# czi-ai/variantformer

Measured on AMD Instinct MI355X. Metric: genes/sec/node (54-tissue expr) at 1 Mb cis-window, higher is better.
Workload: dtype bf16; 1 GPU; BASELINE configs[1]: full 1.2B-architecture network (25 modulator layers, width 1536, 32 heads; seq2reg width 512, 8 heads, 6 layers, assumed), random-init weights, 1 Mb cis-window, 54 tissues, 1 donor; one step = 32 such genes per GPU; n_cre_windows=1024, gene_chunks=200, tissues=54, parallelism=gene-shard x1, streams=CRE layers on a side stream (default)

## Files before the change

variantformer_amd/_lib.py:

```python
from __future__ import annotations

import ctypes as C
import os

_HERE = os.path.dirname(os.path.abspath(__file__))
LIB_PATH = os.path.join(_HERE, "csrc", "libvf_hip.so")

VF_F32, VF_BF16, VF_F16 = 0, 1, 2
EPI_BF16, EPI_F32, EPI_RES_F32, EPI_GEGLU_BF16, EPI_GELU_F32, EPI_GELU_BF16 = 0, 1, 2, 3, 4, 5
ABI_VERSION = 13

_p, _i, _l, _f = C.c_void_p, C.c_int, C.c_int64, C.c_float

SIGNATURES = {
    "vf_version": [],
    "vf_last_error": [],
    "vf_last_kernel": [_i],
    "vf_gemm_bf16": [_p, _l, _p, _p, _p, _l, _p, _l, _i, _i, _i, _i, _p],
    "vf_gemm_bf16_ex": [_p, _l, _p, _p, _p, _l, _p, _l, _i, _i, _i, _i, _i, _p],
    "vf_gemm_f16": [_p, _l, _p, _p, _p, _l, _p, _l, _i, _i, _i, _i, _p],
    "vf_gemm_f16_ex": [_p, _l, _p, _p, _p, _l, _p, _l, _i, _i, _i, _i, _i, _p],
    "vf_gemm_ln_bf16": [_p, _l, _p, _p, _p, _l, _p, _l, _i, _i, _i, _i, _p, _p, _p, _l, _p, _p],
    "vf_gemm_ln_t16": [_p, _l, _p, _p, _p, _l, _f, _p, _l, _i, _i, _i, _i, _p, _l, _p, _f, _p, _l, _f, _p],
    "vf_gemm_ln": [_p, _l, _p, _p, _p, _l, _i, _p, _l, _i, _i, _i, _i, _i, _p, _p, _p, _l, _p, _f, _f, _p],
    "vf_ln_finalize": [_p, _l, _i, _i, _f, _p, _p],
    "vf_ln_finalize2": [_p, _l, _i, _i, _f, _f, _f, _f, _p, _p, _p],
    "vf_row_stats_cast2": [_p, _l, _i, _f, _p, _i, _f, _f, _f, _p, _p, _p],
    "vf_row_stats_cast": [_p, _l, _i, _f, _p, _i, _p, _p],
    "vf_pack_geglu_rows": [_p, _p, _p, _p, _i, _i, _p],
    "vf_attn_varlen_fwd": [_p, _p, _p, _p, _l, _l, _l, _l, _p, _p, _i, _i, _i, _i, _i, _p, _f, _p],
    "vf_attn_varlen_fwd_qstart": [_p, _p, _p, _p, _l, _l, _l, _l, _p, _p, _i, _i, _i, _i, _i, _p, _f, _p],
    "vf_attn_varlen_fwd_f16": [_p, _p, _p, _p, _l, _l, _l, _l, _p, _p, _i, _i, _i, _i, _i, _p, _f, _p],
    "vf_attn_varlen_fwd_qstart_f16": [_p, _p, _p, _p, _l, _l, _l, _l, _p, _p, _i, _i, _i, _i, _i, _p, _f, _p],
    "vf_attn_varlen_fwd_v2": [_p, _p, _p, _p, _l, _l, _l, _l, _p, _p, _i, _i, _i, _i, _i, _p, _f, _i, _i, _p],
    "vf_attn_varlen_fwd_v3": [_p, _p, _p, _p, _l, _l, _l, _l, _p, _p, _i, _i, _i, _i, _i, _p, _f, _i, _i, _p],
    "vf_attn_rows_supported": [_i, _i, _i, _i, _i, _i, _i],
    "vf_attn_counted_keys": [_p, _l, _p, _l, _p, _p, _i, _i, _i, _i, _i, _p, _l, _i, _p],
    "vf_attn_probs": [_p, _l, _p, _l, _p, _p, _p, _i, _i, _i, _i, _i, _f, _i, _i, _i, _p, _p, _l, _p],
    "vf_attn_probs_v2": [_p, _l, _p, _l, _p, _p, _p, _i, _i, _i, _i, _i, _f, _i, _i, _i, _p, _p, _l, _p, _p, _p, _p],
    "vf_softmax_counted": [_p, _l, _p, _p, _i, _i, _i, _i, _i, _p, _l, _i, _p],
    "vf_attn_varlen_fwd_rows": [_p, _p, _p, _p, _l, _l, _l, _l, _p, _p, _i, _i, _i, _i, _i, _p, _f, _i, _i, _p, _p, _p],
    "vf_layernorm": [_p, _p, _p, _p, _l, _i, _f, _i, _i, _p],
    "vf_embed_stream": [_p, _p, _p, _p, _p, _p, _p, _i, _f, _p, _f, _p, _f, _f, _f, _p, _i, _i, _i, _i, _p],
    "vf_embed_pack": [_p, _p, _p, _p, _p, _p, _i, _i, _i, _i, _p],
    "vf_mask_to_cu_seqlens": [_p, _p, _i, _i, _p],
    "vf_segment_mean": [_p, _p, _p, _i, _i, _i, _p],
    "vf_segment_mean16": [_p, _l, _i, _p, _f, _p, _p, _i, _i, _p],
    "vf_token_keys": [_p, _p, _p, _p, _i, _i, _i, _i, _p],
    "vf_gather_rows_f32": [_p, _p, _p, _p, _l, _i, _i, _p],
    "vf_gather_rows_bf16": [_p, _l, _p, _p, _l, _l, _i, _p],
    "vf_rowdot_softplus": [_p, _p, _p, _p, _l, _i, _i, _p],
    "vf_cast_f32_bf16": [_p, _p, _l, _p],
    "vf_cast_f32_f16": [_p, _p, _l, _p],
    "vf_segment_max": [_p, _p, _p, _i, _i, _p],
    "vf_segment_linear": [_p, _p, _p, _p, _p, _p, _i, _i, _i, _i, _p],
    "vf_affine_rows_f32": [_p, _p, _p, _p, _p, _l, _i, _p],
    "vf_add_rows_f32": [_p, _p, _p, _p, _p, _l, _i, _p],
    "vf_bpe_create": [_p, _i, _p, _i],
    "vf_bpe_destroy": [_p],
    "vf_bpe_encode": [_p, C.c_char_p, _l, _p, _p, _l],
    "vf_bpe_encode_prefix": [_p, C.c_char_p, _l, _l, _p, _p, _l],
    "vf_vcf_open": [C.c_char_p, C.c_char_p],
    "vf_vcf_close": [_p],
    "vf_vcf_num_records": [_p, C.c_char_p],
    "vf_vcf_consensus": [_p, C.c_char_p, _l, C.c_char_p, _l, _i, _i, _p, _l, _p],
    "vf_build_windows": [_p, _p, C.c_char_p, _l, C.c_char_p, _l, _l, _p, _p, _i, _i, _i, _i, _l, _p, _p, _p],
    "vf_narrow_ids": [_p, _l, _p, _l, _l],
}
NEXT_SIGNATURES = {
    "vf_attn_contrib": [_p, _l, _p, _p, _l, _p, _p, _i, _i, _i, _i, _i, _i, _i, _p, _p, _l, _p],
}
_RESTYPES = {"vf_last_error": C.c_char_p, "vf_last_kernel": C.c_char_p, "vf_bpe_create": C.c_void_p, "vf_bpe_destroy": None, "vf_bpe_encode": C.c_int64, "vf_bpe_encode_prefix": C.c_int64,
             "vf_vcf_open": C.c_void_p, "vf_vcf_close": None, "vf_vcf_num_records": C.c_int64,
             "vf_vcf_consensus": C.c_int64, "vf_build_windows": C.c_int64}

_lib = None


class VFError(RuntimeError):
    pass


def load(path: str | None = None):
    global _lib
    if _lib is not None and path is None:
        return _lib
    path = path or LIB_PATH
    import torch
    if not os.path.exists(path):
        raise VFError(
            f"{path} not found: the HIP extension has not been built "
            "(run `python -m variantformer_amd.csrc.build` or __graft_entry__.build()). "
            "There is no CPU fallback for the product path.")
    lib = C.CDLL(path)
    for name, argtypes in list(SIGNATURES.items()) + list(NEXT_SIGNATURES.items()):
        try:
            fn = getattr(lib, name)
        except AttributeError as e:
            raise VFError(f"libvf_hip.so does not export {name}") from e
        fn.argtypes = argtypes
        fn.restype = _RESTYPES.get(name, C.c_int)
    v = lib.vf_version()
    if v != ABI_VERSION:
        raise VFError(f"libvf_hip.so ABI version {v} != expected {ABI_VERSION}")
    _lib = lib
    return lib


def check(rc: int, what: str):
    if rc != 0:
        msg = load().vf_last_error()
        raise VFError(f"{what} failed (code {rc}): {msg.decode() if msg else ''}")
```

variantformer_amd/csrc/build.py:

```python
from __future__ import annotations

import os
import shutil
import subprocess
import sys

HERE = os.path.dirname(os.path.abspath(__file__))
SOURCES = ["vf_gemm.hip", "vf_attn.hip", "vf_misc.hip", "vf_bpe.cpp", "vf_vcf.cpp", "vf_host.cpp"]
HEADERS = ["vf_common.h", os.path.join("..", "..", "include", "vf_hip.h"), os.path.join("..", "..", "include", "vf_hip_next.h")]
LIB = os.path.join(HERE, "libvf_hip.so")
ARCH = "gfx950"
EXTRA_FLAGS = {"vf_attn.hip": ["-fno-honor-nans"]}
NO_PACKED_FP32 = ["-Xclang", "-target-feature", "-Xclang", "-packed-fp32-ops"]


def _stale() -> bool:
    if not os.path.exists(LIB):
        return True
    t = os.path.getmtime(LIB)
    return any(os.path.getmtime(os.path.join(HERE, f)) > t for f in SOURCES + HEADERS + [os.path.basename(__file__)])


def build_lib(force: bool = False, verbose: bool = False) -> str:
    if not force and not _stale():
        return LIB
    hipcc = shutil.which("hipcc") or "/opt/rocm/bin/hipcc"
    if not os.path.exists(hipcc):
        raise RuntimeError("hipcc not found: cannot build libvf_hip.so")
    objs = []
    procs = []
    for src in SOURCES:
        obj = os.path.join(HERE, os.path.splitext(src)[0] + ".o")
        cmd = [hipcc, f"--offload-arch={ARCH}", "-O3", "-std=c++17", "-fPIC", "-Wno-unused-result",
               "-mllvm", "-amdgpu-mfma-vgpr-form=1"] + (NO_PACKED_FP32 if src.endswith(".hip") else []) + \
              EXTRA_FLAGS.get(src, []) + \
              ["-c", os.path.join(HERE, src), "-o", obj]
        if verbose:
            cmd.insert(1, "-Rpass-analysis=kernel-resource-usage")
        procs.append((src, subprocess.Popen(cmd, stdout=subprocess.PIPE, stderr=subprocess.STDOUT, text=True)))
        objs.append(obj)
    for src, p in procs:
        out, _ = p.communicate()
        if p.returncode != 0:
            raise RuntimeError(f"hipcc failed on {src}:\n{out}")
        if verbose and out:
            print(out)
    cmd = [hipcc, f"--offload-arch={ARCH}", "-shared", "-fPIC", "-o", LIB + ".tmp"] + objs + ["-lz"]
    r = subprocess.run(cmd, stdout=subprocess.PIPE, stderr=subprocess.STDOUT, text=True)
    if r.returncode != 0:
        raise RuntimeError(f"link failed:\n{r.stdout}")
    os.replace(LIB + ".tmp", LIB)
    return LIB


if __name__ == "__main__":
    print(build_lib(force="--force" in sys.argv, verbose="-v" in sys.argv))
```

variantformer_amd/csrc/vf_common.h:

```cpp
#pragma once
#include <hip/hip_runtime.h>
#include <stdint.h>
#include <stdio.h>
#include "../../include/vf_hip.h"
#include "../../include/vf_hip_next.h"

typedef __attribute__((ext_vector_type(8))) __bf16 bf16x8_t;
typedef __attribute__((ext_vector_type(4))) short s16x4_t;
typedef __attribute__((ext_vector_type(4))) float f32x4_t;
typedef __attribute__((ext_vector_type(16))) float f32x16_t;
typedef __attribute__((ext_vector_type(4))) unsigned int u32x4_t;
typedef __attribute__((ext_vector_type(2))) unsigned int u32x2_t;

#define VF_WAVE 64

void vf_set_error(const char* fmt, ...);
void vf_note_kernel(int which, const char* name);

#define VF_MAX_DEVICES 64
static inline int vf_current_device() {
    int d = -1;
    if (hipGetDevice(&d) != hipSuccess) { (void)hipGetLastError(); return -1; }
    return (d >= 0 && d < VF_MAX_DEVICES) ? d : -1;
}

#define VF_REQUIRE(cond, ...)                        \
    do {                                             \
        if (!(cond)) {                               \
            vf_set_error(__VA_ARGS__);               \
            return VF_ERR_INVALID_ARG;               \
        }                                            \
    } while (0)

#define VF_CHECK_LAUNCH(name)                                                          \
    do {                                                                               \
        hipError_t e_ = hipGetLastError();                                             \
        if (e_ != hipSuccess) {                                                        \
            vf_set_error("%s: launch failed: %s", name, hipGetErrorString(e_));        \
            return VF_ERR_LAUNCH;                                                      \
        }                                                                              \
    } while (0)

__device__ __forceinline__ unsigned short f2bf(float x) {
    __bf16 b = (__bf16)x;
    return *reinterpret_cast<unsigned short*>(&b);
}
typedef __attribute__((ext_vector_type(2))) float f32x2_t;
typedef __attribute__((ext_vector_type(2))) __bf16 bf16x2_t;
__device__ __forceinline__ unsigned int pack2bf(float lo, float hi) {
    const f32x2_t v = {lo, hi};
    const bf16x2_t b = __builtin_convertvector(v, bf16x2_t);
    return __builtin_bit_cast(unsigned int, b);
}
__device__ __forceinline__ float bf2f(unsigned short b) {
    return __uint_as_float(((unsigned int)b) << 16);
}
typedef __attribute__((ext_vector_type(8))) _Float16 f16x8_t;
typedef __attribute__((ext_vector_type(2))) _Float16 f16x2_t;
__device__ __forceinline__ unsigned int pack2h(float lo, float hi) {
    const f32x2_t v = {lo, hi};
    const f16x2_t h = __builtin_convertvector(v, f16x2_t);
    return __builtin_bit_cast(unsigned int, h);
}
__device__ __forceinline__ float h2f(unsigned short b) {
    return (float)__builtin_bit_cast(_Float16, b);
}

template <int DT> struct Op16;
template <> struct Op16<VF_BF16> {
    using frag = bf16x8_t;
    static __device__ __forceinline__ f32x4_t mfma(frag a, frag b, f32x4_t c) {
        return __builtin_amdgcn_mfma_f32_16x16x32_bf16(a, b, c, 0, 0, 0);
    }
    static __device__ __forceinline__ f32x16_t mfma32(frag a, frag b, f32x16_t c) {
        return __builtin_amdgcn_mfma_f32_32x32x16_bf16(a, b, c, 0, 0, 0);
    }
    static __device__ __forceinline__ unsigned int pack2(float lo, float hi) { return pack2bf(lo, hi); }
    static __device__ __forceinline__ float to_f32(unsigned short b) { return bf2f(b); }
    static constexpr unsigned int ONE = 0x3F80u, NEG_BIG = 0xC700u;
};
template <> struct Op16<VF_F16> {
    using frag = f16x8_t;
    static __device__ __forceinline__ f32x4_t mfma(frag a, frag b, f32x4_t c) {
        return __builtin_amdgcn_mfma_f32_16x16x32_f16(a, b, c, 0, 0, 0);
    }
    static __device__ __forceinline__ f32x16_t mfma32(frag a, frag b, f32x16_t c) {
        return __builtin_amdgcn_mfma_f32_32x32x16_f16(a, b, c, 0, 0, 0);
    }
    static __device__ __forceinline__ unsigned int pack2(float lo, float hi) { return pack2h(lo, hi); }
    static __device__ __forceinline__ float to_f32(unsigned short b) { return h2f(b); }
    static constexpr unsigned int ONE = 0x3C00u, NEG_BIG = 0xF800u;
};

__device__ __forceinline__ f32x4_t gelu_erf4(f32x4_t x) {
    f32x4_t ax, t, e;
#pragma unroll
    for (int i = 0; i < 4; ++i) ax[i] = __builtin_fabsf(x[i]);
    const f32x4_t d = ax * 0.23164190f + 1.0f;
#pragma unroll
    for (int i = 0; i < 4; ++i) t[i] = __builtin_amdgcn_rcpf(d[i]);
    f32x4_t p = t * 1.061405429f + -1.453152027f;
    p = p * t + 1.421413741f;
    p = p * t + -0.284496736f;
    p = p * t + 0.254829592f;
    const f32x4_t w = x * x * -0.72134752044448170368f;
#pragma unroll
    for (int i = 0; i < 4; ++i) e[i] = __builtin_amdgcn_exp2f(w[i]);
    const f32x4_t hq = p * t * e * 0.5f;
    f32x4_t r;
#pragma unroll
    for (int i = 0; i < 4; ++i) r[i] = x[i] * (x[i] >= 0.f ? 1.0f - hq[i] : hq[i]);
    return r;
}
__device__ __forceinline__ float gelu_erf(float x) {
    return gelu_erf4((f32x4_t){x, x, x, x})[0];
}
__device__ __forceinline__ float wave_sum(float v) {
#pragma unroll
    for (int o = 32; o > 0; o >>= 1) v += __shfl_xor(v, o);
    return v;
}
```

variantformer_amd/csrc/vf_gemm.hip:

```cpp
#include <type_traits>
#include "vf_common.h"

namespace {

template <int BK>
__device__ __forceinline__ int swz(int row) {
    if (BK == 64) return (row >> 1) & 7;
    return (0x78 >> (((row >> 2) & 3) * 2)) & 3;
}

__device__ __forceinline__ void glds16(const void* g, void* lds) {
    __builtin_amdgcn_global_load_lds((__attribute__((address_space(1))) void*)g,
                                     (__attribute__((address_space(3))) void*)lds, 16, 0, 0);
}

template <int N>
__device__ __forceinline__ void wait_vmcnt() {
    asm volatile("s_waitcnt vmcnt(%0)" ::"n"(N) : "memory");
}

struct LnArgs {
    const float* row_stats;
    const float* colsum;
    void* out16;
    float* part_stats;
    int64_t ld16;
    int64_t rows;
    float x16_scale;
    float res16_scale;
    const unsigned short* res16;
    int64_t ldr16;
    unsigned short* t16_out;
    int64_t ldt16;
    float t16_scale;
};
enum { VF_LN_NONE = 0, VF_LN_CONSUMER = 1, VF_LN_PRODUCER = 2, VF_LN_PRODUCER_R16 = 3, VF_LN_PRODUCER_T16 = 4 };
constexpr bool ln_is_producer(int ln) { return ln == VF_LN_PRODUCER || ln == VF_LN_PRODUCER_R16 || ln == VF_LN_PRODUCER_T16; }
constexpr bool ln_res_is_16(int ln) { return ln == VF_LN_PRODUCER_R16 || ln == VF_LN_PRODUCER_T16; }

template <int DT>
__device__ __forceinline__ f32x4_t cvt4_16(u32x2_t v) {
    if (DT == VF_BF16)
        return (f32x4_t){__uint_as_float(v[0] << 16), __uint_as_float(v[0] & 0xFFFF0000u), __uint_as_float(v[1] << 16),
                         __uint_as_float(v[1] & 0xFFFF0000u)};
    return (f32x4_t){Op16<DT>::to_f32((unsigned short)(v[0] & 0xFFFFu)), Op16<DT>::to_f32((unsigned short)(v[0] >> 16)),
                     Op16<DT>::to_f32((unsigned short)(v[1] & 0xFFFFu)), Op16<DT>::to_f32((unsigned short)(v[1] >> 16))};
}

template <int CTRL>
__device__ __forceinline__ float dpp_f32(float v) {
    return __builtin_bit_cast(float, __builtin_amdgcn_update_dpp(0, __builtin_bit_cast(int, v), CTRL, 0xF, 0xF, true));
}

template <int DT>
__device__ __forceinline__ void ln_emit(f32x4_t f, bool valid, unsigned short* p16, float* ppart, int lane,
                                        float x16_scale = 1.0f, unsigned short* pt16 = nullptr, float t16_scale = 1.0f) {
    float s1 = (f[0] + f[1]) + (f[2] + f[3]);
    s1 += dpp_f32<0xB1>(s1);
    s1 += dpp_f32<0x4E>(s1);
    s1 += dpp_f32<0x141>(s1);
    const float mp = s1 * (1.0f / 32.0f);
    const float d0 = f[0] - mp, d1 = f[1] - mp, d2 = f[2] - mp, d3 = f[3] - mp;
    float s2 = __builtin_fmaf(d3, d3, __builtin_fmaf(d2, d2, __builtin_fmaf(d1, d1, d0 * d0)));
    s2 += dpp_f32<0xB1>(s2);
    s2 += dpp_f32<0x4E>(s2);
    s2 += dpp_f32<0x141>(s2);
    if (valid) {
        u32x2_t pk;
        if (pt16) {
            const f32x4_t t = f * t16_scale;
            pk[0] = pack2h(t[0], t[1]);
            pk[1] = pack2h(t[2], t[3]);
            *reinterpret_cast<u32x2_t*>(pt16) = pk;
        }
        if (DT == VF_F16) f *= x16_scale;
        pk[0] = Op16<DT>::pack2(f[0], f[1]);
        pk[1] = Op16<DT>::pack2(f[2], f[3]);
        *reinterpret_cast<u32x2_t*>(p16) = pk;
        if ((lane & 7) == 0) *reinterpret_cast<f32x2_t*>(ppart) = (f32x2_t){s1, s2};
    }
}

template <int DT>
__device__ __forceinline__ void ln_emit8(f32x4_t fa, f32x4_t fb, bool valid, unsigned short* p16, float* ppart, int lane,
                                         float x16_scale, unsigned short* pt16, float t16_scale) {
    float s1 = ((fa[0] + fa[1]) + (fa[2] + fa[3])) + ((fb[0] + fb[1]) + (fb[2] + fb[3]));
    s1 += dpp_f32<0xB1>(s1);
    s1 += dpp_f32<0x4E>(s1);
    const float mp = s1 * (1.0f / 32.0f);
    const float a0 = fa[0] - mp, a1 = fa[1] - mp, a2 = fa[2] - mp, a3 = fa[3] - mp;
    const float b0 = fb[0] - mp, b1 = fb[1] - mp, b2 = fb[2] - mp, b3 = fb[3] - mp;
    float s2 = __builtin_fmaf(a3, a3, __builtin_fmaf(a2, a2, __builtin_fmaf(a1, a1, a0 * a0))) +
               __builtin_fmaf(b3, b3, __builtin_fmaf(b2, b2, __builtin_fmaf(b1, b1, b0 * b0)));
    s2 += dpp_f32<0xB1>(s2);
    s2 += dpp_f32<0x4E>(s2);
    if (valid) {
        u32x4_t pk;
        if (pt16) {
            const f32x4_t ta = fa * t16_scale, tb = fb * t16_scale;
            pk = (u32x4_t){pack2h(ta[0], ta[1]), pack2h(ta[2], ta[3]), pack2h(tb[0], tb[1]), pack2h(tb[2], tb[3])};
            *reinterpret_cast<u32x4_t*>(pt16) = pk;
        }
        if (DT == VF_F16) { fa *= x16_scale; fb *= x16_scale; }
        pk = (u32x4_t){Op16<DT>::pack2(fa[0], fa[1]), Op16<DT>::pack2(fa[2], fa[3]), Op16<DT>::pack2(fb[0], fb[1]),
                       Op16<DT>::pack2(fb[2], fb[3])};
        *reinterpret_cast<u32x4_t*>(p16) = pk;
        if ((lane & 3) == 0) *reinterpret_cast<f32x2_t*>(ppart) = (f32x2_t){s1, s2};
        else asm volatile("" :: "v"(s1), "v"(s2));
    }
}

template <int DT, int LN, class V>
__device__ __forceinline__ f32x4_t res_value(V v, const LnArgs& ln) {
    if constexpr (LN == VF_LN_PRODUCER_T16) return cvt4_16<VF_F16>(v) * ln.res16_scale;
    else if constexpr (ln_res_is_16(LN)) {
        if constexpr (DT == VF_F16) return cvt4_16<DT>(v) * ln.res16_scale;
        else return cvt4_16<DT>(v);
    }
    else return v;
}

template <int DT, int LN, int REGION>
__device__ __forceinline__ void producer16_epilogue_wide(f32x4_t (&acc)[4][8], char* region, const char* side, int side_n,
                                                         int64_t mw0, int nw0, bool has_bias, void* out, int64_t ldo, int M,
                                                         int N, const LnArgs& ln) {
    constexpr int TM = 8, TN = 4, WT_M = 128, PITCH = 64 * 4 + 16, RP = 32, IMP = RP / 16, NPASS = TM / IMP;
    constexpr int RI = 8, NI = RP / RI;
    constexpr bool T16 = LN == VF_LN_PRODUCER_T16;
    static_assert(REGION >= RP * PITCH, "wide producer epilogue: staging region too small");
    int lane_e;
    asm volatile("v_mbcnt_lo_u32_b32 %0, -1, 0\n\tv_mbcnt_hi_u32_b32 %0, -1, %0" : "=v"(lane_e));
    const int lane = lane_e, r = lane & 15, g = lane >> 4;
    const int ep_row = lane >> 3, ep_col = nw0 + (lane & 7) * 8;
    const int rows_left = (int)(M - mw0) - ep_row;
    const int64_t row0 = mw0 + ep_row;
    const int colc = ep_col < N ? ep_col : N - 8;
    const char* res_run = reinterpret_cast<const char*>(ln.res16) + (row0 * ln.ldr16 + colc) * 2;
    const char* const res_last = reinterpret_cast<const char*>(ln.res16) + ((int64_t)(M - 1) * ln.ldr16 + colc) * 2;
    const int64_t res_step = (int64_t)RI * ln.ldr16 * 2;
    char* out_run = reinterpret_cast<char*>(out) + (row0 * ldo + ep_col) * 4;
    const int64_t out_step = (int64_t)RI * ldo * 4;
    unsigned short* o16_run = reinterpret_cast<unsigned short*>(ln.out16) + row0 * ln.ld16 + ep_col;
    const int64_t o16_step = (int64_t)RI * ln.ld16;
    float* part_run = ln.part_stats + ((int64_t)(ep_col >> 5) * ln.rows + row0) * 2;
    unsigned short* t16_run = T16 ? ln.t16_out + row0 * ln.ldt16 + ep_col : nullptr;
    const int64_t t16_step = (int64_t)RI * ln.ldt16;
    u32x4_t rbuf[2][NI];
    auto load_res_pass = [&](int ps, u32x4_t (&dst)[NI]) {
#pragma unroll
        for (int k = 0; k < NI; ++k) {
            const int j = ps * NI + k;
            const char* rp = (j * RI < rows_left) ? res_run : res_last;
            res_run += res_step;
            dst[k] = *reinterpret_cast<const u32x4_t*>(rp);
        }
    };
    load_res_pass(0, rbuf[0]);
    f32x4_t bvec[TN];
#pragma unroll
    for (int in = 0; in < TN; ++in)
        bvec[in] = has_bias ? *reinterpret_cast<const f32x4_t*>(side + (side_n + in * 16 + 4 * g) * 4) : (f32x4_t){0.f, 0.f, 0.f, 0.f};
#pragma unroll
    for (int ps = 0; ps < NPASS; ++ps) {
        if (ps + 1 < NPASS) load_res_pass(ps + 1, rbuf[(ps + 1) & 1]);
#pragma unroll
        for (int iml = 0; iml < IMP; ++iml) {
            const int im = ps * IMP + iml;
            char* rowp = region + (iml * 16 + r) * PITCH;
#pragma unroll
            for (int in = 0; in < TN; ++in) *reinterpret_cast<f32x4_t*>(rowp + (in * 16 + 4 * g) * 4) = acc[in][im] + bvec[in];
        }
        u32x4_t da[NI], db[NI];
#pragma unroll
        for (int k = 0; k < NI; ++k) {
            const char* p = region + (k * RI + ep_row) * PITCH + (lane & 7) * 32;
            da[k] = *reinterpret_cast<const u32x4_t*>(p);
            db[k] = *reinterpret_cast<const u32x4_t*>(p + 16);
        }
#pragma unroll
        for (int k = 0; k < NI; ++k) {
            const int j = ps * NI + k;
            const u32x4_t rv = rbuf[ps & 1][k];
            const f32x4_t fa = __builtin_bit_cast(f32x4_t, da[k]) + res_value<DT, LN>((u32x2_t){rv[0], rv[1]}, ln);
            const f32x4_t fb = __builtin_bit_cast(f32x4_t, db[k]) + res_value<DT, LN>((u32x2_t){rv[2], rv[3]}, ln);
            const bool ok = j * RI + ep_row < WT_M && j * RI < rows_left && ep_col < N;
            ln_emit8<DT>(fa, fb, ok, o16_run, part_run, lane, ln.x16_scale, (T16 && ln.t16_out) ? t16_run : nullptr, ln.t16_scale);
            o16_run += o16_step;
            part_run += RI * 2;
            if (T16) t16_run += t16_step;
            if (ok && out != nullptr) {
                *reinterpret_cast<f32x4_t*>(out_run) = fa;
                *reinterpret_cast<f32x4_t*>(out_run + 16) = fb;
            }
            out_run += out_step;
        }
    }
}

template <int EPI, int DT = VF_BF16>
__device__ __forceinline__ void epilogue_store(f32x4_t v, f32x4_t gate, int64_t m, int n_bias, int n_bias_gate,
                                               int n_out, const float* __restrict__ bias,
                                               const float* __restrict__ res, int64_t ldr, void* out, int64_t ldo,
                                               const f32x4_t* res_pre = nullptr) {
    if (bias) {
        const f32x4_t b = *reinterpret_cast<const f32x4_t*>(bias + n_bias);
        v += b;
        if (EPI == VF_EPI_GEGLU_BF16) gate += *reinterpret_cast<const f32x4_t*>(bias + n_bias_gate);
    }
    if (EPI == VF_EPI_RES_F32) v += res_pre ? *res_pre : *reinterpret_cast<const f32x4_t*>(res + m * ldr + n_out);
    if (EPI == VF_EPI_GEGLU_BF16) {
        v = v * gelu_erf4(gate);
    }
    if (EPI == VF_EPI_GELU_F32 || EPI == VF_EPI_GELU_BF16) {
        v = gelu_erf4(v);
    }
    if (EPI == VF_EPI_F32 || EPI == VF_EPI_RES_F32 || EPI == VF_EPI_GELU_F32) {
        *reinterpret_cast<f32x4_t*>(reinterpret_cast<float*>(out) + m * ldo + n_out) = v;
    } else {
        u32x2_t p;
        p[0] = Op16<DT>::pack2(v[0], v[1]);
        p[1] = Op16<DT>::pack2(v[2], v[3]);
        *reinterpret_cast<u32x2_t*>(reinterpret_cast<unsigned short*>(out) + m * ldo + n_out) = p;
    }
}

template <int BM_, int BN_, int WM_, int WN_, int STAGES_, int BK_ = 64>
struct Cfg {
    static constexpr int BM = BM_, BN = BN_, WM = WM_, WN = WN_, STAGES = STAGES_, BK = BK_;
    static constexpr int NW = WM * WN, THREADS = NW * 64;
    static constexpr int TM = BM / WM / 16, TN = BN / WN / 16;
    static constexpr int ROW_BYTES = BK * 2, CPR = BK / 8, KS = BK / 32;
    static constexpr int ROWS_PER_PIECE = 1024 / ROW_BYTES;
    static constexpr int A_BYTES = BM * ROW_BYTES, W_BYTES = BN * ROW_BYTES, STAGE_BYTES = A_BYTES + W_BYTES;
    static constexpr int LDS_BYTES = STAGES * STAGE_BYTES;
    static constexpr int PA = A_BYTES / 1024 / NW, PW = W_BYTES / 1024 / NW;
    static constexpr int LPT = PA + PW;
    static_assert(BK == 64 || BK == 32, "BK");
    static_assert(A_BYTES % (1024 * NW) == 0 && W_BYTES % (1024 * NW) == 0, "pieces must divide over the waves");
    static_assert(STAGES >= 2 && STAGES <= 5 && (STAGES - 2) * LPT <= 48, "vmcnt range");
};

__device__ __forceinline__ void tile_origin(int t, int n_tiles, int tiles_n, int GROUP_M, int BM, int BN, int& m0, int& n0) {
    const int q8 = n_tiles >> 3, r8 = n_tiles & 7, xcd = t & 7, loc = t >> 3;
    const int wg = (xcd < r8 ? xcd * (q8 + 1) : r8 * (q8 + 1) + (xcd - r8) * q8) + loc;
    const int tiles_m = n_tiles / tiles_n;
    const int per_group = GROUP_M * tiles_n;
    const int grp = wg / per_group, in_grp = wg - grp * per_group;
    const int first_m = grp * GROUP_M;
    const int gsz = (tiles_m - first_m) < GROUP_M ? (tiles_m - first_m) : GROUP_M;
    m0 = (first_m + in_grp % gsz) * BM;
    n0 = (in_grp / gsz) * BN;
}

template <class C, int EPI, int DT = VF_BF16, int LN = VF_LN_NONE>
__global__ __launch_bounds__(C::THREADS, 2) void gemm_mfma_kernel(const unsigned short* __restrict__ A, int64_t lda,
                                                              const unsigned short* __restrict__ W,
                                                              const float* __restrict__ bias,
                                                              const float* __restrict__ res, int64_t ldr, void* out,
                                                              int64_t ldo, int M, int N, int K, int tiles_n, int n_blocks,
                                                              int GROUP_M, LnArgs ln) {
    extern __shared__ __attribute__((aligned(16))) char smem[];
    using frag_t = typename Op16<DT>::frag;
    constexpr int BM = C::BM, BN = C::BN, TM = C::TM, TN = C::TN, STAGES = C::STAGES, LPT = C::LPT;
    constexpr int BK = C::BK, ROW_BYTES = C::ROW_BYTES, CPR = C::CPR, RPP = C::ROWS_PER_PIECE;

    int m0, n0;
    tile_origin(blockIdx.x, n_blocks, tiles_n, GROUP_M, BM, BN, m0, n0);

    const int tid = threadIdx.x, lane = tid & 63;
    const int wave = __builtin_amdgcn_readfirstlane(tid >> 6);
    const int wm = wave / C::WN, wn = wave % C::WN;
    const int r = lane & 15, g = lane >> 4;

    const unsigned short* srcA[C::PA];
    const unsigned short* srcW[C::PW];
#pragma unroll
    for (int i = 0; i < C::PA; ++i) {
        const int row = RPP * (wave * C::PA + i) + lane / CPR;
        const int c = (lane % CPR) ^ swz<BK>(row);
        int gm = m0 + row; gm = gm < M ? gm : M - 1;
        srcA[i] = A + (int64_t)gm * lda + c * 8;
    }
#pragma unroll
    for (int i = 0; i < C::PW; ++i) {
        const int row = RPP * (wave * C::PW + i) + lane / CPR;
        const int c = (lane % CPR) ^ swz<BK>(row);
        int gn = n0 + row; gn = gn < N ? gn : N - 1;
        srcW[i] = W + (int64_t)gn * K + c * 8;
    }
    char* const ldsA_piece = smem + wave * C::PA * 1024;
    char* const ldsW_piece = smem + C::A_BYTES + wave * C::PW * 1024;

    auto issue = [&](int kt, int stage) {
#pragma unroll
        for (int i = 0; i < C::PA; ++i) glds16(srcA[i] + kt * BK, ldsA_piece + stage * C::STAGE_BYTES + i * 1024);
#pragma unroll
        for (int i = 0; i < C::PW; ++i) glds16(srcW[i] + kt * BK, ldsW_piece + stage * C::STAGE_BYTES + i * 1024);
    };

    f32x4_t acc[TN][TM];
#pragma unroll
    for (int i = 0; i < TN; ++i)
#pragma unroll
        for (int j = 0; j < TM; ++j) acc[i][j] = (f32x4_t){0.f, 0.f, 0.f, 0.f};

    const int sw = swz<BK>(r);
    const int offW = C::A_BYTES + (wn * (BN / C::WN) + r) * ROW_BYTES;
    const int offA = (wm * (BM / C::WM) + r) * ROW_BYTES;

    auto read_frags = [&](int stage, int ks, frag_t(&wf)[TN], frag_t(&af)[TM]) {
        const char* base = smem + stage * C::STAGE_BYTES + (((4 * ks + g) ^ sw) << 4);
#pragma unroll
        for (int i = 0; i < TN; ++i) wf[i] = *reinterpret_cast<const frag_t*>(base + offW + i * 16 * ROW_BYTES);
#pragma unroll
        for (int i = 0; i < TM; ++i) af[i] = *reinterpret_cast<const frag_t*>(base + offA + i * 16 * ROW_BYTES);
    };
    auto issue_piece = [&](int kt, int stage, int i) {
        if (i < C::PA) glds16(srcA[i] + kt * BK, ldsA_piece + stage * C::STAGE_BYTES + i * 1024);
        else glds16(srcW[i - C::PA] + kt * BK, ldsW_piece + stage * C::STAGE_BYTES + (i - C::PA) * 1024);
    };
    auto mma_spread = [&](const frag_t(&wf)[TN], const frag_t(&af)[TM], int kt_issue, int stage_issue, bool do_issue) {
        constexpr int EVERY = 3;
#pragma unroll
        for (int in = 0; in < TN; ++in)
#pragma unroll
            for (int im = 0; im < TM; ++im) {
                acc[in][im] = Op16<DT>::mfma(wf[in], af[im], acc[in][im]);
                const int idx = in * TM + im;
                if (idx % EVERY == EVERY - 1 && idx / EVERY < LPT) {
                    if (do_issue) issue_piece(kt_issue, stage_issue, idx / EVERY);
                    __builtin_amdgcn_sched_barrier(0);
                }
            }
    };
    auto mma = [&](const frag_t(&wf)[TN], const frag_t(&af)[TM]) {
#pragma unroll
        for (int in = 0; in < TN; ++in)
#pragma unroll
            for (int im = 0; im < TM; ++im)
                acc[in][im] = Op16<DT>::mfma(wf[in], af[im], acc[in][im]);
    };
    auto wait_tiles = [&](int ahead) {
        if (STAGES >= 5 && ahead >= 3) wait_vmcnt<3 * LPT>();
        else if (STAGES >= 4 && ahead == 2) wait_vmcnt<2 * LPT>();
        else if (STAGES >= 3 && ahead == 1) wait_vmcnt<LPT>();
        else wait_vmcnt<0>();
    };

    const int nkt = K / BK;
#pragma unroll
    for (int p = 0; p < STAGES; ++p)
        if (p < nkt) issue(p, p);
    wait_tiles((nkt - 1) < (STAGES - 1) ? (nkt - 1) : (STAGES - 1));
    __builtin_amdgcn_s_barrier();
    asm volatile("" ::: "memory");

    frag_t wf0[TN], af0[TM], wf1[TN], af1[TM];
    read_frags(0, 0, wf0, af0);
    int stage = 0;
    auto boundary = [&](int t) {
        asm volatile("s_waitcnt lgkmcnt(0)" ::: "memory");
        wait_tiles((nkt - 2 - t) < (STAGES - 2) ? (nkt - 2 - t) : (STAGES - 2));
        __builtin_amdgcn_s_barrier();
        asm volatile("" ::: "memory");
        if (t + STAGES < nkt) issue(t + STAGES, stage);
        stage = stage + 1 == STAGES ? 0 : stage + 1;
    };
    constexpr bool OUT_F32 = (EPI == VF_EPI_F32 || EPI == VF_EPI_RES_F32 || EPI == VF_EPI_GELU_F32);
    constexpr int ES = OUT_F32 ? 4 : 2;
    constexpr int WT_M = BM / C::WM, WT_N = BN / C::WN;
    constexpr int WT_NO = (EPI == VF_EPI_GEGLU_BF16) ? WT_N / 2 : WT_N;
    constexpr int PITCH = WT_NO * ES + 16;
    constexpr int REGION = C::LDS_BYTES / C::NW;
    constexpr int RP = (((REGION / PITCH) < WT_M ? (REGION / PITCH) : WT_M) / 16) * 16;
    constexpr int IMP = RP / 16, NPASS = (TM + IMP - 1) / IMP;
    constexpr int CR = WT_NO * ES / 16, RI = 64 / CR, NI = RP / RI;
    static_assert(RP >= 16 && CR >= 1 && CR <= 64 && 64 % CR == 0, "epilogue geometry");
    const int n_out_total = (EPI == VF_EPI_GEGLU_BF16) ? N / 2 : N;
    const int64_t mw0 = m0 + wm * WT_M;
    const int no0 = (EPI == VF_EPI_GEGLU_BF16) ? (n0 + wn * WT_N) / 2 : (n0 + wn * WT_N);
    const int ep_row = lane / CR, ep_col = no0 + (lane % CR) * (16 / ES);
    constexpr bool RES_PRE = (EPI == VF_EPI_RES_F32) && (TN * TM <= 16);
    constexpr bool R16 = ln_res_is_16(LN), T16 = LN == VF_LN_PRODUCER_T16;
    using res_t = typename std::conditional<R16, u32x2_t, f32x4_t>::type;
    auto res_load = [&](int64_t m, int col) -> res_t {
        if constexpr (R16) return *reinterpret_cast<const u32x2_t*>(ln.res16 + m * ln.ldr16 + col);
        else return *reinterpret_cast<const f32x4_t*>(res + m * ldr + col);
    };
    res_t resv[RES_PRE ? NPASS : 1][RES_PRE ? NI : 1];
    auto prefetch_residual = [&]() {
        if (RES_PRE) {
#pragma unroll
            for (int ps = 0; ps < NPASS; ++ps)
#pragma unroll
                for (int k = 0; k < NI; ++k) {
                    int64_t m = mw0 + ps * RP + k * RI + ep_row;
                    m = m < M ? m : M - 1;
                    const int col = ep_col < N ? ep_col : N - 4;
                    resv[RES_PRE ? ps : 0][RES_PRE ? k : 0] = res_load(m, col);
                }
        }
    };
    constexpr bool RES_PIPE = (EPI == VF_EPI_RES_F32) && !RES_PRE;
    res_t rbuf[2][RES_PIPE ? NI : 1];
    auto load_res_pass = [&](int ps, res_t (&dst)[RES_PIPE ? NI : 1]) {
        if (RES_PIPE) {
#pragma unroll
            for (int k = 0; k < NI; ++k) {
                int64_t m = mw0 + ps * RP + k * RI + ep_row;
                m = m < M ? m : M - 1;
                const int col = ep_col < N ? ep_col : N - 4;
                dst[RES_PIPE ? k : 0] = res_load(m, col);
            }
        }
    };
    constexpr bool SPREAD = C::KS == 2 && C::NW == 8 && STAGES == 2 && (TN * TM) >= 3 * LPT;
    if (SPREAD) {
        for (int kt = 0; kt < nkt; ++kt) {
            read_frags(stage, 1, wf1, af1);
            if (kt + 1 == nkt) prefetch_residual();
            mma(wf0, af0);
            int freed = stage;
            const bool more = kt + 1 < nkt;
            if (more) {
                asm volatile("s_waitcnt lgkmcnt(0)" ::: "memory");
                wait_tiles((nkt - 2 - kt) < (STAGES - 2) ? (nkt - 2 - kt) : (STAGES - 2));
                __builtin_amdgcn_s_barrier();
                asm volatile("" ::: "memory");
                stage = stage + 1 == STAGES ? 0 : stage + 1;
                read_frags(stage, 0, wf0, af0);
            }
            mma_spread(wf1, af1, kt + STAGES, freed, more && kt + STAGES < nkt);
        }
    } else if (C::KS == 2) {
        for (int kt = 0; kt < nkt; ++kt) {
            read_frags(stage, 1, wf1, af1);
            if (kt + 1 == nkt) prefetch_residual();
            mma(wf0, af0);
            if (kt + 1 < nkt) {
                boundary(kt);
                read_frags(stage, 0, wf0, af0);
            }
            mma(wf1, af1);
        }
    } else {
        for (int kt = 0; kt < nkt; kt += 2) {
            boundary(kt);
            read_frags(stage, 0, wf1, af1);
            mma(wf0, af0);
            if (kt + 2 < nkt) {
                boundary(kt + 1);
                read_frags(stage, 0, wf0, af0);
            } else {
                prefetch_residual();
            }
            mma(wf1, af1);
        }
    }

    const int nw0 = n0 + wn * WT_N;
    load_res_pass(0, rbuf[0]);
    __syncthreads();
    f32x4_t bvec[TN];
    if (bias) {
#pragma unroll
        for (int in = 0; in < TN; ++in) {
            int nb = (EPI == VF_EPI_GEGLU_BF16) ? nw0 + (in >> 1) * 32 + (in & 1) * 16 + 4 * g : nw0 + in * 16 + 4 * g;
            nb = nb < N ? nb : 0;
            bvec[in] = *reinterpret_cast<const f32x4_t*>(bias + nb);
        }
    } else {
#pragma unroll
        for (int in = 0; in < TN; ++in) bvec[in] = (f32x4_t){0.f, 0.f, 0.f, 0.f};
    }
    f32x4_t svec[LN == VF_LN_CONSUMER ? TN : 1];
    float ln_mu[LN == VF_LN_CONSUMER ? TM : 1], ln_rs[LN == VF_LN_CONSUMER ? TM : 1];
    if (LN == VF_LN_CONSUMER) {
#pragma unroll
        for (int in = 0; in < TN; ++in) {
            int nb = (EPI == VF_EPI_GEGLU_BF16) ? nw0 + (in >> 1) * 32 + (in & 1) * 16 + 4 * g : nw0 + in * 16 + 4 * g;
            nb = nb < N ? nb : 0;
            svec[LN == VF_LN_CONSUMER ? in : 0] = *reinterpret_cast<const f32x4_t*>(ln.colsum + nb);
        }
#pragma unroll
        for (int im = 0; im < TM; ++im) {
            int64_t m = mw0 + im * 16 + r;
            m = m < M ? m : M - 1;
            const f32x2_t st = *reinterpret_cast<const f32x2_t*>(ln.row_stats + 2 * m);
            ln_mu[LN == VF_LN_CONSUMER ? im : 0] = -st[0] * st[1];
            ln_rs[LN == VF_LN_CONSUMER ? im : 0] = st[1];
        }
    }
    auto lnv = [&](int in, int im) -> f32x4_t {
        if (LN == VF_LN_CONSUMER)
            return acc[in][im] * ln_rs[LN == VF_LN_CONSUMER ? im : 0] +
                   (ln_mu[LN == VF_LN_CONSUMER ? im : 0] * svec[LN == VF_LN_CONSUMER ? in : 0] + bvec[in]);
        return acc[in][im] + bvec[in];
    };
    char* const region = smem + wave * REGION;
#pragma unroll
    for (int ps = 0; ps < NPASS; ++ps) {
        if (ps + 1 < NPASS) load_res_pass(ps + 1, rbuf[(ps + 1) & 1]);
#pragma unroll
        for (int iml = 0; iml < IMP; ++iml) {
            const int im = ps * IMP + iml;
            if (im < TM) {
                char* rowp = region + (iml * 16 + r) * PITCH;
                if (EPI == VF_EPI_GEGLU_BF16) {
#pragma unroll
                    for (int ip = 0; ip < TN / 2; ++ip) {
                        const f32x4_t v = lnv(2 * ip, im), gt = lnv(2 * ip + 1, im);
                        u32x2_t pk;
                        const f32x4_t y = v * gelu_erf4(gt);
                        pk[0] = Op16<DT>::pack2(y[0], y[1]);
                        pk[1] = Op16<DT>::pack2(y[2], y[3]);
                        *reinterpret_cast<u32x2_t*>(rowp + (ip * 16 + 4 * g) * 2) = pk;
                    }
                } else {
#pragma unroll
                    for (int in = 0; in < TN; ++in) {
                        f32x4_t v = lnv(in, im);
                        if (EPI == VF_EPI_GELU_F32 || EPI == VF_EPI_GELU_BF16) {
                            v = gelu_erf4(v);
                        }
                        if (OUT_F32) {
                            *reinterpret_cast<f32x4_t*>(rowp + (in * 16 + 4 * g) * 4) = v;
                        } else {
                            u32x2_t pk;
                            pk[0] = Op16<DT>::pack2(v[0], v[1]);
                            pk[1] = Op16<DT>::pack2(v[2], v[3]);
                            *reinterpret_cast<u32x2_t*>(rowp + (in * 16 + 4 * g) * 2) = pk;
                        }
                    }
                }
            }
        }
        constexpr int KB = (EPI == VF_EPI_RES_F32) ? 4 : NI;
#pragma unroll
        for (int k0 = 0; k0 < NI; k0 += KB) {
            u32x4_t dd[KB];
#pragma unroll
            for (int k = 0; k < KB; ++k)
                if (k0 + k < NI)
                    dd[k] = *reinterpret_cast<const u32x4_t*>(region + ((k0 + k) * RI + ep_row) * PITCH + (lane % CR) * 16);
#pragma unroll
            for (int k = 0; k < KB; ++k) {
                if (k0 + k >= NI) continue;
                const int row = (k0 + k) * RI + ep_row;
                const int64_t m = mw0 + ps * RP + row;
                u32x4_t d = dd[k];
                if (EPI == VF_EPI_RES_F32) {
                    f32x4_t f = __builtin_bit_cast(f32x4_t, d);
                    f += res_value<DT, LN>(RES_PRE ? resv[RES_PRE ? ps : 0][RES_PRE ? k0 + k : 0] : rbuf[ps & 1][RES_PIPE ? k0 + k : 0], ln);
                    d = __builtin_bit_cast(u32x4_t, f);
                }
                const bool ok = ps * RP + row < WT_M && m < M && ep_col < n_out_total;
                if (ln_is_producer(LN) && OUT_F32)
                    ln_emit<DT>(__builtin_bit_cast(f32x4_t, d), ok,
                                reinterpret_cast<unsigned short*>(ln.out16) + m * ln.ld16 + ep_col,
// ... 43 lines not shown
                        Op16<DT>::mfma(WF[i][ks], af[j][ks], acc[IN0 + i][IM0 + j]); \
    } while (0)

template <int EPI, int DT = VF_BF16, int LN = VF_LN_NONE>
__global__ __launch_bounds__(512, 2) void gemm8_kernel(const unsigned short* __restrict__ A, int64_t lda,
                                                       const unsigned short* __restrict__ W,
                                                       const float* __restrict__ bias, const float* __restrict__ res,
                                                       int64_t ldr, void* out, int64_t ldo, int M, int N, int K,
                                                       int tiles_n, int n_blocks, int GROUP_M, LnArgs ln) {
    extern __shared__ __attribute__((aligned(16))) char smem[];
    using frag_t = typename Op16<DT>::frag;
    using C = Cfg8;
    constexpr int BM = C::BM, BN = C::BN, TM = C::TM, TN = C::TN, BK = C::BK;

    int m0, n0;
    tile_origin(blockIdx.x, n_blocks, tiles_n, GROUP_M, BM, BN, m0, n0);

    const int tid = threadIdx.x, lane = tid & 63;
    const int wave = __builtin_amdgcn_readfirstlane(tid >> 6);
    const int wm = wave >> 2, wn = wave & 3;
    const int r = lane & 15, g = lane >> 4;

    const unsigned short* src[4][2];
#pragma unroll
    for (int pi = 0; pi < 2; ++pi) {
        const int i = 16 * wave + 8 * pi + (lane >> 3);
        const int c = (lane & 7) ^ ((i >> 1) & 7);
        const int am = m0 + (i >> 6) * 128 + (i & 63);
        const int wn_row = n0 + (i >> 5) * 64 + (i & 31);
        int v;
        v = am;           v = v < M ? v : M - 1;  src[C::AL][pi] = A + (int64_t)v * lda + c * 8;
        v = am + 64;      v = v < M ? v : M - 1;  src[C::AH][pi] = A + (int64_t)v * lda + c * 8;
        v = wn_row;       v = v < N ? v : N - 1;  src[C::WL][pi] = W + (int64_t)v * K + c * 8;
        v = wn_row + 32;  v = v < N ? v : N - 1;  src[C::WH][pi] = W + (int64_t)v * K + c * 8;
    }
    char* const lds_piece = smem + wave * 2048;
    auto issue = [&](int kt, int type) {
        char* dst = lds_piece + (kt & 1) * C::TILE_BYTES + type * C::HALF_BYTES;
        glds16(src[type][0] + kt * BK, dst);
        glds16(src[type][1] + kt * BK, dst + 1024);
    };

    f32x4_t acc[TN][TM];
#pragma unroll
    for (int i = 0; i < TN; ++i)
#pragma unroll
        for (int j = 0; j < TM; ++j) acc[i][j] = (f32x4_t){0.f, 0.f, 0.f, 0.f};

    const int sw = (r >> 1) & 7;
    const int ck0 = ((g) ^ sw) << 4, ck1 = ((4 + g) ^ sw) << 4;
    const int offW = (wn * 32 + r) * 128;
    const int offA = (wm * 64 + r) * 128;
    frag_t wlo[2][2], whi[2][2], af[4][2];
    auto read_w = [&](const char* buf, int type, frag_t (&f)[2][2]) {
        const char* b = buf + type * C::HALF_BYTES + offW;
#pragma unroll
        for (int i = 0; i < 2; ++i) {
            f[i][0] = *reinterpret_cast<const frag_t*>(b + i * 2048 + ck0);
            f[i][1] = *reinterpret_cast<const frag_t*>(b + i * 2048 + ck1);
        }
    };
    auto read_a = [&](const char* buf, int type) {
        const char* b = buf + type * C::HALF_BYTES + offA;
#pragma unroll
        for (int i = 0; i < 4; ++i) {
            af[i][0] = *reinterpret_cast<const frag_t*>(b + i * 2048 + ck0);
            af[i][1] = *reinterpret_cast<const frag_t*>(b + i * 2048 + ck1);
        }
    };
    char* const side = smem + C::LDS_BYTES;
    if (bias && wave == 0) {
        int n = n0 + 4 * lane;
        n = n < N ? n : N - 4;
        glds16(bias + n, side);
    }
    if (LN == VF_LN_CONSUMER) {
        if (wave == 1) {
            int n = n0 + 4 * lane;
            n = n < N ? n : N - 4;
            glds16(ln.colsum + n, side + 1024);
        }
        int64_t m = m0 + 32 * wave + (lane >> 1);
        m = m < M ? m : M - 1;
        __builtin_amdgcn_global_load_lds((__attribute__((address_space(1))) void*)(ln.row_stats + 2 * m + (lane & 1)),
                                         (__attribute__((address_space(3))) void*)(side + 2048 + wave * 256), 4, 0, 0);
    }

    const int nkt = K / BK;
    issue(0, C::WL); issue(0, C::AL); issue(0, C::WH); issue(0, C::AH);
    if (nkt > 1) {
        issue(1, C::WL); issue(1, C::AL); issue(1, C::WH);
        wait_vmcnt<6>();
    } else {
        wait_vmcnt<0>();
    }
    __builtin_amdgcn_s_barrier();
    asm volatile("" ::: "memory");
    if (wm == 1) __builtin_amdgcn_s_barrier();

    for (int t = 0; t < nkt; ++t) {
        const char* buf = smem + (t & 1) * C::TILE_BYTES;
        const bool pre1 = t + 1 < nkt, pre2 = t + 2 < nkt;
        read_w(buf, C::WL, wlo);
        __builtin_amdgcn_sched_barrier(0);
        read_a(buf, C::AL);
        if (pre1) issue(t + 1, C::AH);
        asm volatile("s_waitcnt lgkmcnt(8)" ::: "memory");
        VF_G8_SYNC_IN();
        VF_G8_MMA(wlo, 0, 0);
        VF_G8_SYNC_OUT();
        read_w(buf, C::WH, whi);
        if (pre2) issue(t + 2, C::WL);
        VF_G8_SYNC_IN();
        VF_G8_MMA(whi, 2, 0);
        VF_G8_SYNC_OUT();
        read_a(buf, C::AH);
        if (pre2) issue(t + 2, C::AL);
        VF_G8_SYNC_IN();
        VF_G8_MMA(whi, 2, 4);
        VF_G8_SYNC_OUT();
        if (pre2) {
            issue(t + 2, C::WH);
            wait_vmcnt<6>();
        } else {
            wait_vmcnt<0>();
        }
        VF_G8_SYNC_IN();
        VF_G8_MMA(wlo, 0, 4);
        VF_G8_SYNC_OUT();
    }
    if (wm == 0) __builtin_amdgcn_s_barrier();
    asm volatile("" ::: "memory");

    constexpr bool OUT_F32 = (EPI == VF_EPI_F32 || EPI == VF_EPI_RES_F32 || EPI == VF_EPI_GELU_F32);
    constexpr int ES = OUT_F32 ? 4 : 2;
    constexpr int WT_M = 128, WT_N = 64;
    constexpr int WT_NO = (EPI == VF_EPI_GEGLU_BF16) ? WT_N / 2 : WT_N;
    constexpr int PITCH = WT_NO * ES + 16;
    constexpr int REGION = C::LDS_BYTES / C::NW;
    constexpr int RP_FIT = (((REGION / PITCH) < WT_M ? (REGION / PITCH) : WT_M) / 16) * 16;
    constexpr int RP = (ln_is_producer(LN) && EPI == VF_EPI_RES_F32 && RP_FIT > 32) ? 32 : RP_FIT;
    constexpr int IMP = RP / 16, NPASS = (TM + IMP - 1) / IMP;
    constexpr int CR = WT_NO * ES / 16, RI = 64 / CR, NI = RP / RI;
    static_assert(RP >= 16 && CR >= 1 && CR <= 64 && 64 % CR == 0, "epilogue geometry");
    constexpr bool RES = (EPI == VF_EPI_RES_F32);
    const int n_out_total = (EPI == VF_EPI_GEGLU_BF16) ? N / 2 : N;
    const int64_t mw0 = m0 + wm * WT_M;
    const int nw0 = n0 + wn * WT_N;
    const int no0 = (EPI == VF_EPI_GEGLU_BF16) ? nw0 / 2 : nw0;
    const int ep_row = lane / CR, ep_col = no0 + (lane % CR) * (16 / ES);
    const int rows_left = (int)(M - mw0) - ep_row;
    const int64_t row0 = mw0 + ep_row;
    const int colc = ep_col < N ? ep_col : N - 4;
    constexpr bool R16 = ln_res_is_16(LN), T16 = LN == VF_LN_PRODUCER_T16;
    using res_t = typename std::conditional<R16, u32x2_t, f32x4_t>::type;
    const char* const res_base = R16 ? reinterpret_cast<const char*>(ln.res16) : reinterpret_cast<const char*>(res);
    const int64_t res_ld = R16 ? ln.ldr16 : ldr;
    constexpr int RES_ES = R16 ? 2 : 4;
    const char* const res_p = RES ? res_base + (row0 * res_ld + colc) * RES_ES : nullptr;
    const char* const res_last = RES ? res_base + ((int64_t)(M - 1) * res_ld + colc) * RES_ES : nullptr;
    const int64_t res_step = (int64_t)RI * res_ld * RES_ES;
    char* const out_p = reinterpret_cast<char*>(out) + (row0 * ldo + ep_col) * ES;
    const int64_t out_step = (int64_t)RI * ldo * ES;
    unsigned short* const o16_p = ln_is_producer(LN) ? reinterpret_cast<unsigned short*>(ln.out16) + row0 * ln.ld16 + ep_col : nullptr;
    const int64_t o16_step = (int64_t)RI * ln.ld16;
    float* const part_p = ln_is_producer(LN) ? ln.part_stats + ((int64_t)(ep_col >> 5) * ln.rows + row0) * 2 : nullptr;
    const char* res_run = res_p;
    char* out_run = out_p;
    unsigned short* o16_run = o16_p;
    float* part_run = part_p;
    unsigned short* t16_run = T16 ? ln.t16_out + row0 * ln.ldt16 + ep_col : nullptr;
    const int64_t t16_step = (int64_t)RI * ln.ldt16;
    res_t rbuf[2][RES ? NI : 1];
    auto load_res_pass = [&](int ps, res_t (&dst)[RES ? NI : 1]) {
        if (RES) {
#pragma unroll
            for (int k = 0; k < NI; ++k) {
                const int j = ps * NI + k;
                const char* rp = (j * RI < rows_left) ? res_run : res_last;
                res_run += res_step;
                dst[RES ? k : 0] = *reinterpret_cast<const res_t*>(rp);
            }
        }
    };
    load_res_pass(0, rbuf[0]);
    f32x4_t bvec[TN];
    if (bias) {
#pragma unroll
        for (int in = 0; in < TN; ++in) {
            const int nl = wn * WT_N + ((EPI == VF_EPI_GEGLU_BF16) ? (in >> 1) * 32 + (in & 1) * 16 + 4 * g : in * 16 + 4 * g);
            bvec[in] = *reinterpret_cast<const f32x4_t*>(side + nl * 4);
        }
    } else {
#pragma unroll
        for (int in = 0; in < TN; ++in) bvec[in] = (f32x4_t){0.f, 0.f, 0.f, 0.f};
    }
    f32x4_t svec[LN == VF_LN_CONSUMER ? TN : 1];
    float ln_mu[LN == VF_LN_CONSUMER ? TM : 1], ln_rs[LN == VF_LN_CONSUMER ? TM : 1];
    if (LN == VF_LN_CONSUMER) {
#pragma unroll
        for (int in = 0; in < TN; ++in) {
            const int nl = wn * WT_N + ((EPI == VF_EPI_GEGLU_BF16) ? (in >> 1) * 32 + (in & 1) * 16 + 4 * g : in * 16 + 4 * g);
            svec[LN == VF_LN_CONSUMER ? in : 0] = *reinterpret_cast<const f32x4_t*>(side + 1024 + nl * 4);
        }
#pragma unroll
        for (int im = 0; im < TM; ++im) {
            const f32x2_t st = *reinterpret_cast<const f32x2_t*>(side + 2048 + (wm * WT_M + im * 16 + r) * 8);
            ln_mu[LN == VF_LN_CONSUMER ? im : 0] = -st[0] * st[1];
            ln_rs[LN == VF_LN_CONSUMER ? im : 0] = st[1];
        }
    }
    auto lnv = [&](int in, int im) -> f32x4_t {
        if (LN == VF_LN_CONSUMER)
            return acc[in][im] * ln_rs[LN == VF_LN_CONSUMER ? im : 0] +
                   (ln_mu[LN == VF_LN_CONSUMER ? im : 0] * svec[LN == VF_LN_CONSUMER ? in : 0] + bvec[in]);
        return acc[in][im] + bvec[in];
    };
    char* const region = smem + wave * REGION;
#pragma unroll
    for (int ps = 0; ps < NPASS; ++ps) {
        if (ps + 1 < NPASS) load_res_pass(ps + 1, rbuf[(ps + 1) & 1]);
#pragma unroll
        for (int iml = 0; iml < IMP; ++iml) {
            const int im = ps * IMP + iml;
            if (im < TM) {
                char* rowp = region + (iml * 16 + r) * PITCH;
                if (EPI == VF_EPI_GEGLU_BF16) {
#pragma unroll
                    for (int ip = 0; ip < TN / 2; ++ip) {
                        const f32x4_t v = lnv(2 * ip, im), gt = lnv(2 * ip + 1, im);
                        u32x2_t pk;
                        const f32x4_t y = v * gelu_erf4(gt);
                        pk[0] = Op16<DT>::pack2(y[0], y[1]);
                        pk[1] = Op16<DT>::pack2(y[2], y[3]);
                        *reinterpret_cast<u32x2_t*>(rowp + (ip * 16 + 4 * g) * 2) = pk;
                    }
                } else {
#pragma unroll
                    for (int in = 0; in < TN; ++in) {
                        f32x4_t v = lnv(in, im);
                        if (EPI == VF_EPI_GELU_F32 || EPI == VF_EPI_GELU_BF16) {
                            v = gelu_erf4(v);
                        }
                        if (OUT_F32) {
                            *reinterpret_cast<f32x4_t*>(rowp + (in * 16 + 4 * g) * 4) = v;
                        } else {
                            u32x2_t pk;
                            pk[0] = Op16<DT>::pack2(v[0], v[1]);
                            pk[1] = Op16<DT>::pack2(v[2], v[3]);
                            *reinterpret_cast<u32x2_t*>(rowp + (in * 16 + 4 * g) * 2) = pk;
                        }
                    }
                }
            }
        }
        constexpr int KB = RES ? 4 : NI;
#pragma unroll
        for (int k0 = 0; k0 < NI; k0 += KB) {
            u32x4_t dd[KB];
#pragma unroll
            for (int k = 0; k < KB; ++k)
                if (k0 + k < NI)
                    dd[k] = *reinterpret_cast<const u32x4_t*>(region + ((k0 + k) * RI + ep_row) * PITCH + (lane % CR) * 16);
#pragma unroll
            for (int k = 0; k < KB; ++k) {
                if (k0 + k >= NI) continue;
                const int j = ps * NI + k0 + k;
                u32x4_t d = dd[k];
                if (RES) {
                    f32x4_t f = __builtin_bit_cast(f32x4_t, d);
                    f += res_value<DT, LN>(rbuf[ps & 1][RES ? k0 + k : 0], ln);
                    d = __builtin_bit_cast(u32x4_t, f);
                }
                const bool ok = j * RI + ep_row < WT_M && j * RI < rows_left && ep_col < n_out_total;
                if (ln_is_producer(LN) && OUT_F32) {
                    ln_emit<DT>(__builtin_bit_cast(f32x4_t, d), ok, o16_run, part_run, lane, ln.x16_scale,
                                (T16 && ln.t16_out) ? t16_run : nullptr, ln.t16_scale);
                    o16_run += o16_step;
                    part_run += RI * 2;
                    if (T16) t16_run += t16_step;
                }
                if (ok && (!ln_is_producer(LN) || out != nullptr)) *reinterpret_cast<u32x4_t*>(out_run) = d;
                out_run += out_step;
            }
        }
    }
}

template <int EPI, int DT = VF_BF16, int LN = VF_LN_NONE>
__global__ __launch_bounds__(512, 2) void gemm8x_kernel(const unsigned short* __restrict__ A, int64_t lda,
                                                       const unsigned short* __restrict__ W,
                                                       const float* __restrict__ bias, const float* __restrict__ res,
                                                       int64_t ldr, void* out, int64_t ldo, int M, int N, int K,
                                                       int tiles_n, int n_tiles, int GROUP_M, LnArgs ln) {
    extern __shared__ __attribute__((aligned(16))) char smem[];
    using frag_t = typename Op16<DT>::frag;
    using C = Cfg8;
    constexpr int BM = C::BM, BN = C::BN, TM = C::TM, TN = C::TN, BK = C::BK;

    const int bid = blockIdx.x;
    const int grid = gridDim.x;
    const int my_tiles = (n_tiles - bid + grid - 1) / grid;
    auto origin = [&](int t, int& m0, int& n0) { tile_origin(t, n_tiles, tiles_n, GROUP_M, BM, BN, m0, n0); };

    const int tid = threadIdx.x, lane = tid & 63;
    const int wave = __builtin_amdgcn_readfirstlane(tid >> 6);
    const int wm = wave >> 2, wn = wave & 3;
    const int r = lane & 15, g = lane >> 4;

    const unsigned short* src[4][2];
    auto set_src = [&](int m0, int n0) {
#pragma unroll
        for (int pi = 0; pi < 2; ++pi) {
            const int i = 16 * wave + 8 * pi + (lane >> 3);
            const int c = (lane & 7) ^ ((i >> 1) & 7);
            const int am = m0 + (i >> 6) * 128 + (i & 63);
            const int wn_row = n0 + (i >> 5) * 64 + (i & 31);
            int v;
            v = am;           v = v < M ? v : M - 1;  src[C::AL][pi] = A + (int64_t)v * lda + c * 8;
            v = am + 64;      v = v < M ? v : M - 1;  src[C::AH][pi] = A + (int64_t)v * lda + c * 8;
            v = wn_row;       v = v < N ? v : N - 1;  src[C::WL][pi] = W + (int64_t)v * K + c * 8;
            v = wn_row + 32;  v = v < N ? v : N - 1;  src[C::WH][pi] = W + (int64_t)v * K + c * 8;
        }
    };
    char* const lds_piece = smem + wave * 2048;
    auto issue = [&](int gk, int kt, int type) {
        char* dst = lds_piece + (gk & 1) * C::TILE_BYTES + type * C::HALF_BYTES;
        glds16(src[type][0] + kt * BK, dst);
        glds16(src[type][1] + kt * BK, dst + 1024);
    };
    auto issue_side = [&](int m0, int n0, int seq) {
        char* const sd = smem + C::LDS_BYTES + C::SPARE_BYTES + (seq & 1) * C::SIDE_BYTES;
        int lane;
        asm volatile("v_mbcnt_lo_u32_b32 %0, -1, 0\n\tv_mbcnt_hi_u32_b32 %0, -1, %0" : "=v"(lane));
        if (bias && wave == 0) {
            int n = n0 + 4 * lane;
            n = n < N ? n : N - 4;
            glds16(bias + n, sd);
        }
        if (LN == VF_LN_CONSUMER) {
            if (wave == 1) {
                int n = n0 + 4 * lane;
                n = n < N ? n : N - 4;
                glds16(ln.colsum + n, sd + 1024);
            }
            int64_t m = m0 + 32 * wave + (lane >> 1);
            m = m < M ? m : M - 1;
            __builtin_amdgcn_global_load_lds((__attribute__((address_space(1))) void*)(ln.row_stats + 2 * m + (lane & 1)),
                                             (__attribute__((address_space(3))) void*)(sd + 2048 + wave * 256), 4, 0, 0);
        }
    };

    f32x4_t acc[TN][TM];

    const int sw = (r >> 1) & 7;
    const int ck0 = ((g) ^ sw) << 4, ck1 = ((4 + g) ^ sw) << 4;
    const int offW = (wn * 32 + r) * 128;
    const int offA = (wm * 64 + r) * 128;
    frag_t wlo[2][2], whi[2][2], af[4][2];
    auto read_w = [&](const char* buf, int type, frag_t (&f)[2][2]) {
        const char* b = buf + type * C::HALF_BYTES + offW;
#pragma unroll
        for (int i = 0; i < 2; ++i) {
            f[i][0] = *reinterpret_cast<const frag_t*>(b + i * 2048 + ck0);
            f[i][1] = *reinterpret_cast<const frag_t*>(b + i * 2048 + ck1);
        }
    };
    auto read_a = [&](const char* buf, int type) {
        const char* b = buf + type * C::HALF_BYTES + offA;
#pragma unroll
        for (int i = 0; i < 4; ++i) {
            af[i][0] = *reinterpret_cast<const frag_t*>(b + i * 2048 + ck0);
            af[i][1] = *reinterpret_cast<const frag_t*>(b + i * 2048 + ck1);
        }
    };
    const int nkt = K / BK;
    int m0, n0;
    origin(bid, m0, n0);
    set_src(m0, n0);
    issue_side(m0, n0, 0);
    issue(0, 0, C::WL); issue(0, 0, C::AL); issue(0, 0, C::WH); issue(0, 0, C::AH);

    int g0 = 0;
    for (int ti = 0; ti < my_tiles; ++ti) {
        const bool has_next = ti + 1 < my_tiles;
        origin(bid + ti * grid, m0, n0);
#pragma unroll
        for (int i = 0; i < TN; ++i)
#pragma unroll
            for (int j = 0; j < TM; ++j) acc[i][j] = (f32x4_t){0.f, 0.f, 0.f, 0.f};
        issue(g0 + 1, 1, C::WL); issue(g0 + 1, 1, C::AL); issue(g0 + 1, 1, C::WH);
        if (ti == 0) wait_vmcnt<6>();
        __builtin_amdgcn_s_barrier();
        asm volatile("" ::: "memory");
        if (wm == 1) __builtin_amdgcn_s_barrier();

        for (int t = 0; t < nkt; ++t) {
            const char* buf = smem + ((g0 + t) & 1) * C::TILE_BYTES;
            const bool pre1 = t + 1 < nkt || has_next;
            const bool pre2 = t + 2 < nkt || (t + 2 == nkt && has_next);
            const bool into_next = t + 2 >= nkt;
            read_w(buf, C::WL, wlo);
            __builtin_amdgcn_sched_barrier(0);
            read_a(buf, C::AL);
            if (pre1) issue(g0 + t + 1, t + 1 < nkt ? t + 1 : 0, C::AH);
            asm volatile("s_waitcnt lgkmcnt(8)" ::: "memory");
            VF_G8_SYNC_IN();
            VF_G8_MMA(wlo, 0, 0);
            VF_G8_SYNC_OUT();
            if (t + 2 == nkt && has_next) {
                int m1, n1;
                origin(bid + (ti + 1) * grid, m1, n1);
                set_src(m1, n1);
                issue_side(m1, n1, ti + 1);
            }
            read_w(buf, C::WH, whi);
            if (pre2) issue(g0 + t + 2, into_next ? 0 : t + 2, C::WL);
            VF_G8_SYNC_IN();
            VF_G8_MMA(whi, 2, 0);
            VF_G8_SYNC_OUT();
            read_a(buf, C::AH);
            if (pre2) issue(g0 + t + 2, into_next ? 0 : t + 2, C::AL);
            VF_G8_SYNC_IN();
            VF_G8_MMA(whi, 2, 4);
            VF_G8_SYNC_OUT();
            if (pre2) {
                issue(g0 + t + 2, into_next ? 0 : t + 2, C::WH);
                wait_vmcnt<6>();
            } else {
                wait_vmcnt<0>();
            }
            VF_G8_SYNC_IN();
            VF_G8_MMA(wlo, 0, 4);
            VF_G8_SYNC_OUT();
        }
        if (wm == 0) __builtin_amdgcn_s_barrier();
        asm volatile("" ::: "memory");
        char* const side = smem + C::LDS_BYTES + C::SPARE_BYTES + (ti & 1) * C::SIDE_BYTES;
        char* const stage_buf = smem + C::TILE_BYTES;
        int lane_e;
        asm volatile("v_mbcnt_lo_u32_b32 %0, -1, 0\n\tv_mbcnt_hi_u32_b32 %0, -1, %0" : "=v"(lane_e));
        const int lane = lane_e, r = lane & 15, g = lane >> 4;

        constexpr bool WIDE = ln_res_is_16(LN) && EPI == VF_EPI_RES_F32;
        if constexpr (WIDE) {
            producer16_epilogue_wide<DT, LN, (C::TILE_BYTES + C::SPARE_BYTES) / C::NW>(
                acc, stage_buf + wave * ((C::TILE_BYTES + C::SPARE_BYTES) / C::NW), side, wn * 64, (int64_t)m0 + wm * 128,
                n0 + wn * 64, bias != nullptr, out, ldo, M, N, ln);
        } else {
        constexpr bool OUT_F32 = (EPI == VF_EPI_F32 || EPI == VF_EPI_RES_F32 || EPI == VF_EPI_GELU_F32);
        constexpr int ES = OUT_F32 ? 4 : 2;
        constexpr int WT_M = 128, WT_N = 64;
        constexpr int WT_NO = (EPI == VF_EPI_GEGLU_BF16) ? WT_N / 2 : WT_N;
        constexpr int PITCH = WT_NO * ES + 16;
        constexpr int REGION = (C::TILE_BYTES + C::SPARE_BYTES) / C::NW;
        constexpr int RP_FIT = (((REGION / PITCH) < WT_M ? (REGION / PITCH) : WT_M) / 16) * 16;
        constexpr bool R16 = ln_res_is_16(LN), T16 = LN == VF_LN_PRODUCER_T16;
        constexpr int RP = (EPI == VF_EPI_RES_F32 && !R16 && RP_FIT > 16) ? 16 : RP_FIT;
        constexpr int IMP = RP / 16, NPASS = (TM + IMP - 1) / IMP;
        constexpr int CR = WT_NO * ES / 16, RI = 64 / CR, NI = RP / RI;
        static_assert(RP >= 16 && CR >= 1 && CR <= 64 && 64 % CR == 0, "epilogue geometry");
        constexpr bool RES = (EPI == VF_EPI_RES_F32);
        const int n_out_total = (EPI == VF_EPI_GEGLU_BF16) ? N / 2 : N;
        const int64_t mw0 = m0 + wm * WT_M;
        const int nw0 = n0 + wn * WT_N;
        const int no0 = (EPI == VF_EPI_GEGLU_BF16) ? nw0 / 2 : nw0;
        const int ep_row = lane / CR, ep_col = no0 + (lane % CR) * (16 / ES);
        const int rows_left = (int)(M - mw0) - ep_row;
        const int64_t row0 = mw0 + ep_row;
        const int colc = ep_col < N ? ep_col : N - 4;
        using res_t = typename std::conditional<R16, u32x2_t, f32x4_t>::type;
        const char* const res_base = R16 ? reinterpret_cast<const char*>(ln.res16) : reinterpret_cast<const char*>(res);
        const int64_t res_ld = R16 ? ln.ldr16 : ldr;
        constexpr int RES_ES = R16 ? 2 : 4;
        const char* const res_p = RES ? res_base + (row0 * res_ld + colc) * RES_ES : nullptr;
        const char* const res_last = RES ? res_base + ((int64_t)(M - 1) * res_ld + colc) * RES_ES : nullptr;
        const int64_t res_step = (int64_t)RI * res_ld * RES_ES;
        char* const out_p = reinterpret_cast<char*>(out) + (row0 * ldo + ep_col) * ES;
        const int64_t out_step = (int64_t)RI * ldo * ES;
        unsigned short* const o16_p = ln_is_producer(LN) ? reinterpret_cast<unsigned short*>(ln.out16) + row0 * ln.ld16 + ep_col : nullptr;
        const int64_t o16_step = (int64_t)RI * ln.ld16;
        float* const part_p = ln_is_producer(LN) ? ln.part_stats + ((int64_t)(ep_col >> 5) * ln.rows + row0) * 2 : nullptr;
        const char* res_run = res_p;
        char* out_run = out_p;
        unsigned short* o16_run = o16_p;
        float* part_run = part_p;
        unsigned short* t16_run = T16 ? ln.t16_out + row0 * ln.ldt16 + ep_col : nullptr;
        const int64_t t16_step = (int64_t)RI * ln.ldt16;
        res_t rbuf[2][RES ? NI : 1];
        auto load_res_pass = [&](int ps, res_t (&dst)[RES ? NI : 1]) {
            if (RES) {
#pragma unroll
                for (int k = 0; k < NI; ++k) {
                    const int j = ps * NI + k;
                    const char* rp = (j * RI < rows_left) ? res_run : res_last;
                    res_run += res_step;
                    dst[RES ? k : 0] = *reinterpret_cast<const res_t*>(rp);
                }
            }
        };
        load_res_pass(0, rbuf[0]);
        f32x4_t bvec[TN];
        if (bias) {
#pragma unroll
            for (int in = 0; in < TN; ++in) {
                const int nl = wn * WT_N + ((EPI == VF_EPI_GEGLU_BF16) ? (in >> 1) * 32 + (in & 1) * 16 + 4 * g : in * 16 + 4 * g);
                bvec[in] = *reinterpret_cast<const f32x4_t*>(side + nl * 4);
            }
        } else {
#pragma unroll
            for (int in = 0; in < TN; ++in) bvec[in] = (f32x4_t){0.f, 0.f, 0.f, 0.f};
        }
        f32x4_t svec[LN == VF_LN_CONSUMER ? TN : 1];
        if (LN == VF_LN_CONSUMER) {
#pragma unroll
            for (int in = 0; in < TN; ++in) {
                const int nl = wn * WT_N + ((EPI == VF_EPI_GEGLU_BF16) ? (in >> 1) * 32 + (in & 1) * 16 + 4 * g : in * 16 + 4 * g);
                svec[LN == VF_LN_CONSUMER ? in : 0] = *reinterpret_cast<const f32x4_t*>(side + 1024 + nl * 4);
            }
        }
        auto lnv = [&](int in, int im, f32x2_t st) -> f32x4_t {
            if (LN == VF_LN_CONSUMER) return acc[in][im] * st[1] + (st[0] * svec[LN == VF_LN_CONSUMER ? in : 0] + bvec[in]);
            return acc[in][im] + bvec[in];
        };
        char* const region = stage_buf + wave * REGION;
#pragma unroll
        for (int ps = 0; ps < NPASS; ++ps) {
            if (ps + 1 < NPASS) load_res_pass(ps + 1, rbuf[(ps + 1) & 1]);
#pragma unroll
            for (int iml = 0; iml < IMP; ++iml) {
                const int im = ps * IMP + iml;
                if (im < TM) {
                    char* rowp = region + (iml * 16 + r) * PITCH;
                    f32x2_t st = {0.f, 1.f};
                    if (LN == VF_LN_CONSUMER) {
                        st = *reinterpret_cast<const f32x2_t*>(side + 2048 + (wm * WT_M + im * 16 + r) * 8);
                        st[0] = -st[0] * st[1];
                    }
                    if (EPI == VF_EPI_GEGLU_BF16) {
#pragma unroll
                        for (int ip = 0; ip < TN / 2; ++ip) {
                            const f32x4_t v = lnv(2 * ip, im, st), gt = lnv(2 * ip + 1, im, st);
                            u32x2_t pk;
                            const f32x4_t y = v * gelu_erf4(gt);
                            pk[0] = Op16<DT>::pack2(y[0], y[1]);
                            pk[1] = Op16<DT>::pack2(y[2], y[3]);
                            *reinterpret_cast<u32x2_t*>(rowp + (ip * 16 + 4 * g) * 2) = pk;
                        }
                    } else {
#pragma unroll
                        for (int in = 0; in < TN; ++in) {
                            f32x4_t v = lnv(in, im, st);
                            if (EPI == VF_EPI_GELU_F32 || EPI == VF_EPI_GELU_BF16) {
                                v = gelu_erf4(v);
                            }
                            if (OUT_F32) {
                                *reinterpret_cast<f32x4_t*>(rowp + (in * 16 + 4 * g) * 4) = v;
                            } else {
                                u32x2_t pk;
                                pk[0] = Op16<DT>::pack2(v[0], v[1]);
                                pk[1] = Op16<DT>::pack2(v[2], v[3]);
                                *reinterpret_cast<u32x2_t*>(rowp + (in * 16 + 4 * g) * 2) = pk;
                            }
                        }
                    }
                }
            }
            constexpr int KB = RES ? 4 : NI;
#pragma unroll
            for (int k0 = 0; k0 < NI; k0 += KB) {
                u32x4_t dd[KB];
#pragma unroll
                for (int k = 0; k < KB; ++k)
                    if (k0 + k < NI)
                        dd[k] = *reinterpret_cast<const u32x4_t*>(region + ((k0 + k) * RI + ep_row) * PITCH + (lane % CR) * 16);
#pragma unroll
                for (int k = 0; k < KB; ++k) {
                    if (k0 + k >= NI) continue;
                    const int j = ps * NI + k0 + k;
                    u32x4_t d = dd[k];
                    if (RES) {
                        f32x4_t f = __builtin_bit_cast(f32x4_t, d);
                        f += res_value<DT, LN>(rbuf[ps & 1][RES ? k0 + k : 0], ln);
                        d = __builtin_bit_cast(u32x4_t, f);
                    }
                    const bool ok = j * RI + ep_row < WT_M && j * RI < rows_left && ep_col < n_out_total;
                    if (ln_is_producer(LN) && OUT_F32) {
                        ln_emit<DT>(__builtin_bit_cast(f32x4_t, d), ok, o16_run, part_run, lane, ln.x16_scale,
                                    (T16 && ln.t16_out) ? t16_run : nullptr, ln.t16_scale);
                        o16_run += o16_step;
                        part_run += RI * 2;
                        if (T16) t16_run += t16_step;
                    }
                    if (ok && (!ln_is_producer(LN) || out != nullptr)) *reinterpret_cast<u32x4_t*>(out_run) = d;
                    out_run += out_step;
                }
            }
        }

        }

        __builtin_amdgcn_s_barrier();
        asm volatile("" ::: "memory");
        g0 += nkt;
    }
#undef VF_G8_SYNC_IN
#undef VF_G8_SYNC_OUT
#undef VF_G8_MMA
}

// ... 64 lines not shown
        }
        if (dev >= 0) attr_set[dev] = true;
    }
    vf_note_kernel(0, name);
    hipLaunchKernelGGL(KERN, dim3(grid), dim3(threads), LDS, st, args...);
    VF_CHECK_LAUNCH("vf_gemm_bf16");
    return VF_OK;
}

template <class C, int EPI, int DT = VF_BF16, int LN = VF_LN_NONE>
int launch_cfg(const void* A, int64_t lda, const void* W, const float* bias, const float* res, int64_t ldr, void* out,
               int64_t ldo, int M, int N, int K, hipStream_t st, LnArgs ln = LnArgs{}) {
    const int tiles_m = (M + C::BM - 1) / C::BM, tiles_n = (N + C::BN - 1) / C::BN;
    const int n_blocks = tiles_m * tiles_n;
    const int group_m = 8;
    return launch_with_lds<gemm_mfma_kernel<C, EPI, DT, LN>, C::LDS_BYTES>(
        vf_current_device(), C::BM == 128 ? "gemm_mfma_kernel<128x128>" : C::BM == 64 ? "gemm_mfma_kernel<64x64>" : "gemm_mfma_kernel<other>",
        n_blocks, C::THREADS, st, (const unsigned short*)A, lda, (const unsigned short*)W, bias, res, ldr, out, ldo, M, N, K,
        tiles_n, n_blocks, group_m, ln);
}

template <int EPI, int DT = VF_BF16, int LN = VF_LN_NONE>
int launch_gemm8(const void* A, int64_t lda, const void* W, const float* bias, const float* res, int64_t ldr, void* out,
                 int64_t ldo, int M, int N, int K, hipStream_t st, LnArgs ln = LnArgs{}) {
    const int tiles_m = (M + 255) / 256, tiles_n = (N + 255) / 256;
    const int n_blocks = tiles_m * tiles_n;
    const int group_m = 8;
    return launch_with_lds<gemm8_kernel<EPI, DT, LN>, Cfg8::LDS_BYTES + Cfg8::SIDE_BYTES>(
        vf_current_device(), "gemm8_kernel", n_blocks, 512, st, (const unsigned short*)A, lda, (const unsigned short*)W, bias, res,
        ldr, out, ldo, M, N, K, tiles_n, n_blocks, group_m, ln);
}

template <int EPI, int DT = VF_BF16, int LN = VF_LN_NONE>
int launch_gemm8x(const void* A, int64_t lda, const void* W, const float* bias, const float* res, int64_t ldr, void* out,
                  int64_t ldo, int M, int N, int K, hipStream_t st, LnArgs ln = LnArgs{}) {
    constexpr int LDS = Cfg8::LDS_BYTES + Cfg8::SPARE_BYTES + 2 * Cfg8::SIDE_BYTES;
    static int n_cu[VF_MAX_DEVICES] = {};
    const int dev = vf_current_device();
    int cus = 256;
    if (dev >= 0) {
        if (n_cu[dev] == 0) {
            int v = 0;
            if (hipDeviceGetAttribute(&v, hipDeviceAttributeMultiprocessorCount, dev) != hipSuccess || v <= 0) v = 256;
            n_cu[dev] = v;
        }
        cus = n_cu[dev];
    }
    const int tiles_m = (M + 255) / 256, tiles_n = (N + 255) / 256;
    const int n_tiles = tiles_m * tiles_n;
    const int grid = n_tiles < cus ? n_tiles : cus;
    const int group_m = 8;
    return launch_with_lds<gemm8x_kernel<EPI, DT, LN>, LDS>(dev, "gemm8x_kernel", grid, 512, st, (const unsigned short*)A, lda,
                                                            (const unsigned short*)W, bias, res, ldr, out, ldo, M, N, K, tiles_n,
                                                            n_tiles, group_m, ln);
}

int pick_variant(int M, int N, int K, int epilogue) {
    const long t128 = (long)((M + 127) / 128) * ((N + 127) / 128);
    const long t256 = (long)((M + 255) / 256) * ((N + 255) / 256);
    if (t128 < 256) return 5;
    (void)K;
    const long waves_small = (t128 + 511) / 512, waves_big = (t256 + 255) / 256;
    const double gain = epilogue == VF_EPI_RES_F32 ? 1.14 : 1.2;
    if (!((double)waves_big * 2.0 / gain < (double)waves_small)) return 1;
    const bool out16 = epilogue == VF_EPI_BF16 || epilogue == VF_EPI_GEGLU_BF16 || epilogue == VF_EPI_GELU_BF16;
    return (out16 && K % 128 == 0) ? 22 : 20;
}

template <int EPI, int DT>
int launch_gemm(const void* A, int64_t lda, const void* W, const float* bias, const float* res, int64_t ldr, void* out,
                int64_t ldo, int M, int N, int K, int variant, hipStream_t st) {
    if (K % 64 != 0) {
        static int max_grid_y[VF_MAX_DEVICES] = {};
        const int dev = vf_current_device();
        int limit = 65535;
        if (dev >= 0) {
            if (max_grid_y[dev] == 0) {
                int v = 0;
                if (hipDeviceGetAttribute(&v, hipDeviceAttributeMaxGridDimY, dev) != hipSuccess || v <= 0) {
                    (void)hipGetLastError();
                    v = 65535;
                }
                max_grid_y[dev] = v;
            }
            limit = max_grid_y[dev];
        }
        VF_REQUIRE(((long)M + 63) / 64 <= limit,
                   "vf_gemm: K=%d is not a multiple of 64, and the generic kernel puts ceil(M / 64) = %d row blocks on "
                   "grid.y, above the device's limit of %d (hipDeviceAttributeMaxGridDimY): split M", K, (int)(((long)M + 63) / 64), limit);
        dim3 grid((N + 63) / 64, (M + 63) / 64);
        vf_note_kernel(0, "gemm_generic_kernel");
        hipLaunchKernelGGL((gemm_generic_kernel<EPI, DT>), grid, dim3(256), 0, st, (const unsigned short*)A, lda,
                           (const unsigned short*)W, bias, res, ldr, out, ldo, M, N, K);
        VF_CHECK_LAUNCH("vf_gemm_bf16");
        return VF_OK;
    }
    if (variant == 0) variant = pick_variant(M, N, K, EPI);
    switch (variant) {
        case 1: return launch_cfg<CfgA, EPI, DT>(A, lda, W, bias, res, ldr, out, ldo, M, N, K, st);
        case 5: return launch_cfg<CfgE, EPI, DT>(A, lda, W, bias, res, ldr, out, ldo, M, N, K, st);
        case 20: return launch_gemm8<EPI, DT>(A, lda, W, bias, res, ldr, out, ldo, M, N, K, st);
        case 22: if (K % 128 == 0) return launch_gemm8x<EPI, DT>(A, lda, W, bias, res, ldr, out, ldo, M, N, K, st);
                 return launch_gemm8<EPI, DT>(A, lda, W, bias, res, ldr, out, ldo, M, N, K, st);
        default: break;
    }
    vf_set_error("vf_gemm_bf16_ex: unknown variant %d", variant);
    return VF_ERR_INVALID_ARG;
}

__global__ void pack_geglu_rows_kernel(const unsigned short* __restrict__ W, const float* __restrict__ bias,
                                       unsigned short* __restrict__ Wo, float* __restrict__ bo, int two_f, int K) {
    const int row_out = blockIdx.x;
    const int F = two_f / 2;
    const int b = row_out >> 5, t = row_out & 31;
    const int row_in = t < 16 ? 16 * b + t : F + 16 * b + (t - 16);
    for (int k = threadIdx.x; k < K; k += blockDim.x) Wo[(int64_t)row_out * K + k] = W[(int64_t)row_in * K + k];
    if (bias && threadIdx.x == 0) bo[row_out] = bias[row_in];
}

}

template <int DT>
static int gemm_dispatch(const void* A, int64_t lda, const void* W, const float* bias, const float* residual,
                         int64_t ldr, void* out, int64_t ldo, int M, int N, int K, int epilogue, int variant, void* stream) {
    VF_REQUIRE(A && W && out, "vf_gemm: null pointer");
    VF_REQUIRE(M >= 0 && N > 0 && K > 0, "vf_gemm: bad shape M=%d N=%d K=%d", M, N, K);
    VF_REQUIRE(K % 8 == 0 && N % 8 == 0, "vf_gemm: K and N must be multiples of 8 (K=%d N=%d)", K, N);
    VF_REQUIRE(lda % 8 == 0 && lda >= K, "vf_gemm: lda=%lld must be >= K and a multiple of 8", (long long)lda);
    VF_REQUIRE(ldo % 8 == 0 || (ldo % 4 == 0 && (epilogue == VF_EPI_F32 || epilogue == VF_EPI_RES_F32 || epilogue == VF_EPI_GELU_F32)),
               "vf_gemm: ldo=%lld must keep rows 16-byte aligned (multiple of 8 for 16-bit, 4 for fp32 outputs)", (long long)ldo);
    VF_REQUIRE(((uintptr_t)A % 16 == 0) && ((uintptr_t)W % 16 == 0) && ((uintptr_t)out % 16 == 0),
               "vf_gemm: pointers must be 16-byte aligned");
    VF_REQUIRE(variant >= 0 && variant <= 999, "vf_gemm_ex: variant %d out of range", variant);
    if (M == 0) return VF_OK;
    hipStream_t st = (hipStream_t)stream;
    switch (epilogue) {
        case VF_EPI_BF16: return launch_gemm<VF_EPI_BF16, DT>(A, lda, W, bias, residual, ldr, out, ldo, M, N, K, variant, st);
        case VF_EPI_F32: return launch_gemm<VF_EPI_F32, DT>(A, lda, W, bias, residual, ldr, out, ldo, M, N, K, variant, st);
        case VF_EPI_RES_F32:
            VF_REQUIRE(residual && ldr % 4 == 0 && ((uintptr_t)residual % 16 == 0), "vf_gemm: residual epilogue needs an aligned residual");
            return launch_gemm<VF_EPI_RES_F32, DT>(A, lda, W, bias, residual, ldr, out, ldo, M, N, K, variant, st);
        case VF_EPI_GEGLU_BF16:
            VF_REQUIRE(N % 32 == 0, "vf_gemm: GEGLU epilogue needs N %% 32 == 0 (N=%d)", N);
            return launch_gemm<VF_EPI_GEGLU_BF16, DT>(A, lda, W, bias, residual, ldr, out, ldo, M, N, K, variant, st);
        case VF_EPI_GELU_F32: return launch_gemm<VF_EPI_GELU_F32, DT>(A, lda, W, bias, residual, ldr, out, ldo, M, N, K, variant, st);
        case VF_EPI_GELU_BF16: return launch_gemm<VF_EPI_GELU_BF16, DT>(A, lda, W, bias, residual, ldr, out, ldo, M, N, K, variant, st);
        default: VF_REQUIRE(false, "vf_gemm: unknown epilogue %d", epilogue);
    }
    return VF_OK;
}

template <int EPI, int DT, int LN>
static int launch_gemm_ln(const void* A, int64_t lda, const void* W, const float* bias, const float* residual, int64_t ldr,
                          void* out, int64_t ldo, int M, int N, int K, const LnArgs& ln, hipStream_t st) {
    int variant = pick_variant(M, N, K, EPI);
    if constexpr (ln_res_is_16(LN)) {
        if (variant == 20 && K % 128 == 0 && out == nullptr) variant = 22;
    }
    switch (variant) {
        case 1: return launch_cfg<CfgA, EPI, DT, LN>(A, lda, W, bias, residual, ldr, out, ldo, M, N, K, st, ln);
        case 5: return launch_cfg<CfgE, EPI, DT, LN>(A, lda, W, bias, residual, ldr, out, ldo, M, N, K, st, ln);
        case 22: return launch_gemm8x<EPI, DT, LN>(A, lda, W, bias, residual, ldr, out, ldo, M, N, K, st, ln);
        default: return launch_gemm8<EPI, DT, LN>(A, lda, W, bias, residual, ldr, out, ldo, M, N, K, st, ln);
    }
}

template <int DT>
static int gemm_ln_dispatch(const void* A, int64_t lda, const void* W, const float* bias, const void* residual, int64_t ldr,
                            int residual_dtype, void* out, int64_t ldo, int M, int N, int K, int epilogue,
                            const float* row_stats, const float* colsum, void* out16, int64_t ld16, float* part_stats,
                            float x16_scale, float res16_scale, void* stream, bool trunk = false, void* t16_out = nullptr,
                            int64_t ldt16 = 0, float t16_scale = 1.0f) {
    VF_REQUIRE(A && W && (out || (out16 && part_stats)), "vf_gemm_ln: null pointer");
    VF_REQUIRE(M >= 0 && N > 0 && K > 0 && K % 64 == 0 && N % 8 == 0, "vf_gemm_ln: needs K %% 64 == 0, N %% 8 == 0 (N=%d K=%d)", N, K);
    VF_REQUIRE(lda % 8 == 0 && lda >= K, "vf_gemm_ln: lda=%lld must be >= K and a multiple of 8", (long long)lda);
    VF_REQUIRE(((uintptr_t)A % 16 == 0) && ((uintptr_t)W % 16 == 0) && ((uintptr_t)out % 16 == 0),
               "vf_gemm_ln: pointers must be 16-byte aligned");
    const bool consumer = row_stats && colsum, producer = out16 && part_stats;
    VF_REQUIRE(consumer != producer, "vf_gemm_ln: give (row_stats, colsum) OR (out16, part_stats)");
    if (M == 0) return VF_OK;
    LnArgs ln{};
    ln.x16_scale = 1.0f;
    ln.res16_scale = 1.0f;
    hipStream_t st = (hipStream_t)stream;
    if (consumer) {
        VF_REQUIRE(out, "vf_gemm_ln: the consumer needs an output");
        VF_REQUIRE(((uintptr_t)row_stats % 8 == 0) && ((uintptr_t)colsum % 16 == 0), "vf_gemm_ln: misaligned statistics");
        VF_REQUIRE(ldo % 8 == 0, "vf_gemm_ln: ldo=%lld must be a multiple of 8", (long long)ldo);
        ln.row_stats = row_stats;
        ln.colsum = colsum;
        if (epilogue == VF_EPI_BF16)
            return launch_gemm_ln<VF_EPI_BF16, DT, VF_LN_CONSUMER>(A, lda, W, bias, nullptr, 0, out, ldo, M, N, K, ln, st);
        if (epilogue == VF_EPI_F32)
            return launch_gemm_ln<VF_EPI_F32, DT, VF_LN_CONSUMER>(A, lda, W, bias, nullptr, 0, out, ldo, M, N, K, ln, st);
        VF_REQUIRE(epilogue == VF_EPI_GEGLU_BF16 && N % 32 == 0, "vf_gemm_ln: consumer epilogues are BF16, F32 and GEGLU_BF16");
        return launch_gemm_ln<VF_EPI_GEGLU_BF16, DT, VF_LN_CONSUMER>(A, lda, W, bias, nullptr, 0, out, ldo, M, N, K, ln, st);
    }
    VF_REQUIRE(ld16 % 4 == 0 && ld16 >= N && ((uintptr_t)out16 % 8 == 0) && ((uintptr_t)part_stats % 8 == 0) && ldo % 4 == 0,
               "vf_gemm_ln: producer outputs must keep 8-byte alignment (ld16=%lld)", (long long)ld16);
    VF_REQUIRE(N % 32 == 0, "vf_gemm_ln: a producer needs N %% 32 == 0 (whole 32-column parts; N=%d)", N);
    VF_REQUIRE(x16_scale > 0.f && (DT == VF_F16 || x16_scale == 1.0f), "vf_gemm_ln: x16_scale must be > 0 (and 1 for bf16 streams)");
    ln.out16 = out16;
    ln.part_stats = part_stats;
    ln.ld16 = ld16;
    ln.rows = M;
    ln.x16_scale = x16_scale;
    if (epilogue == VF_EPI_F32)
        return launch_gemm_ln<VF_EPI_F32, DT, VF_LN_PRODUCER>(A, lda, W, bias, nullptr, 0, out, ldo, M, N, K, ln, st);
    VF_REQUIRE(epilogue == VF_EPI_RES_F32 && residual, "vf_gemm_ln: producer epilogues are F32 and RES_F32 (with a residual)");
    if (residual_dtype == VF_F32) {
        VF_REQUIRE(ldr % 4 == 0 && ((uintptr_t)residual % 16 == 0), "vf_gemm_ln: misaligned fp32 residual");
        return launch_gemm_ln<VF_EPI_RES_F32, DT, VF_LN_PRODUCER>(A, lda, W, bias, (const float*)residual, ldr, out, ldo, M, N, K, ln, st);
    }
    if (trunk) {
        VF_REQUIRE(residual_dtype == VF_F16, "vf_gemm_ln_t16: the trunk residual is fp16");
        VF_REQUIRE(ldr % 4 == 0 && ((uintptr_t)residual % 8 == 0) && res16_scale > 0.f, "vf_gemm_ln_t16: misaligned fp16 residual");
        VF_REQUIRE(!t16_out || (ldt16 % 4 == 0 && ldt16 >= N && ((uintptr_t)t16_out % 8 == 0) && t16_scale > 0.f),
                   "vf_gemm_ln_t16: the fp16 trunk output must keep 8-byte alignment (ldt16=%lld)", (long long)ldt16);
        ln.res16 = (const unsigned short*)residual;
        ln.ldr16 = ldr;
        ln.res16_scale = res16_scale;
        ln.t16_out = (unsigned short*)t16_out;
        ln.ldt16 = ldt16;
        ln.t16_scale = t16_scale;
        return launch_gemm_ln<VF_EPI_RES_F32, DT, VF_LN_PRODUCER_T16>(A, lda, W, bias, (const float*)residual, ldr, out, ldo, M, N, K, ln, st);
    }
    VF_REQUIRE(residual_dtype == DT, "vf_gemm_ln: a 16-bit residual must have the operand type");
    VF_REQUIRE(ldr % 4 == 0 && ((uintptr_t)residual % 8 == 0) && res16_scale > 0.f, "vf_gemm_ln: misaligned 16-bit residual");
    VF_REQUIRE(DT == VF_F16 || res16_scale == 1.0f, "vf_gemm_ln: res16_scale must be 1 for bf16 streams");
    ln.res16 = (const unsigned short*)residual;
    ln.ldr16 = ldr;
    ln.res16_scale = res16_scale;
    return launch_gemm_ln<VF_EPI_RES_F32, DT, VF_LN_PRODUCER_R16>(A, lda, W, bias, (const float*)residual, ldr, out, ldo, M, N, K, ln, st);
}

extern "C" int vf_gemm_ln(const void* A, int64_t lda, const void* W, const float* bias, const void* residual, int64_t ldr,
                          int residual_dtype, void* out, int64_t ldo, int M, int N, int K, int epilogue, int operand_dtype,
                          const float* row_stats, const float* colsum, void* out16, int64_t ld16, float* part_stats,
                          float x16_scale, float res16_scale, void* stream) {
    if (operand_dtype == VF_BF16)
        return gemm_ln_dispatch<VF_BF16>(A, lda, W, bias, residual, ldr, residual_dtype, out, ldo, M, N, K, epilogue, row_stats,
                                         colsum, out16, ld16, part_stats, x16_scale, res16_scale, stream);
    VF_REQUIRE(operand_dtype == VF_F16, "vf_gemm_ln: operand_dtype must be VF_BF16 or VF_F16");
    return gemm_ln_dispatch<VF_F16>(A, lda, W, bias, residual, ldr, residual_dtype, out, ldo, M, N, K, epilogue, row_stats,
                                    colsum, out16, ld16, part_stats, x16_scale, res16_scale, stream);
}

extern "C" int vf_gemm_ln_t16(const void* A, int64_t lda, const void* W, const float* bias, const void* residual_f16,
                              int64_t ldr, float res_scale, void* out, int64_t ldo, int M, int N, int K, int operand_dtype,
                              void* out16, int64_t ld16, float* part_stats, float x16_scale, void* t16_out, int64_t ldt16,
                              float t16_scale, void* stream) {
    VF_REQUIRE(residual_f16, "vf_gemm_ln_t16: null residual");
    if (operand_dtype == VF_BF16)
        return gemm_ln_dispatch<VF_BF16>(A, lda, W, bias, residual_f16, ldr, VF_F16, out, ldo, M, N, K, VF_EPI_RES_F32, nullptr,
                                         nullptr, out16, ld16, part_stats, x16_scale, res_scale, stream, true, t16_out, ldt16,
                                         t16_scale);
    VF_REQUIRE(operand_dtype == VF_F16, "vf_gemm_ln_t16: operand_dtype must be VF_BF16 or VF_F16");
    return gemm_ln_dispatch<VF_F16>(A, lda, W, bias, residual_f16, ldr, VF_F16, out, ldo, M, N, K, VF_EPI_RES_F32, nullptr, nullptr,
                                    out16, ld16, part_stats, x16_scale, res_scale, stream, true, t16_out, ldt16, t16_scale);
}

extern "C" int vf_gemm_ln_bf16(const void* A, int64_t lda, const void* W, const float* bias, const float* residual,
                               int64_t ldr, void* out, int64_t ldo, int M, int N, int K, int epilogue,
                               const float* row_stats, const float* colsum, void* out16, int64_t ld16,
                               float* part_stats, void* stream) {
    return gemm_ln_dispatch<VF_BF16>(A, lda, W, bias, residual, ldr, VF_F32, out, ldo, M, N, K, epilogue, row_stats, colsum,
                                     out16, ld16, part_stats, 1.0f, 1.0f, stream);
}

extern "C" int vf_gemm_bf16(const void* A, int64_t lda, const void* W, const float* bias, const float* residual,
                            int64_t ldr, void* out, int64_t ldo, int M, int N, int K, int epilogue, void* stream) {
    return gemm_dispatch<VF_BF16>(A, lda, W, bias, residual, ldr, out, ldo, M, N, K, epilogue, 0, stream);
}

extern "C" int vf_gemm_bf16_ex(const void* A, int64_t lda, const void* W, const float* bias, const float* residual,
                               int64_t ldr, void* out, int64_t ldo, int M, int N, int K, int epilogue, int variant,
                               void* stream) {
    return gemm_dispatch<VF_BF16>(A, lda, W, bias, residual, ldr, out, ldo, M, N, K, epilogue, variant, stream);
}

extern "C" int vf_gemm_f16(const void* A, int64_t lda, const void* W, const float* bias, const float* residual,
                           int64_t ldr, void* out, int64_t ldo, int M, int N, int K, int epilogue, void* stream) {
    return gemm_dispatch<VF_F16>(A, lda, W, bias, residual, ldr, out, ldo, M, N, K, epilogue, 0, stream);
}

extern "C" int vf_gemm_f16_ex(const void* A, int64_t lda, const void* W, const float* bias, const float* residual,
                              int64_t ldr, void* out, int64_t ldo, int M, int N, int K, int epilogue, int variant,
                              void* stream) {
    return gemm_dispatch<VF_F16>(A, lda, W, bias, residual, ldr, out, ldo, M, N, K, epilogue, variant, stream);
}

extern "C" int vf_pack_geglu_rows(const void* W, const float* bias, void* W_out, float* bias_out, int two_f, int K,
                                  void* stream) {
    VF_REQUIRE(W && W_out && two_f > 0 && two_f % 32 == 0 && K > 0, "vf_pack_geglu_rows: need 2F %% 32 == 0 (2F=%d)", two_f);
    VF_REQUIRE(!bias || bias_out, "vf_pack_geglu_rows: bias given without bias_out");
    hipLaunchKernelGGL(pack_geglu_rows_kernel, dim3(two_f), dim3(256), 0, (hipStream_t)stream, (const unsigned short*)W,
                       bias, (unsigned short*)W_out, bias_out, two_f, K);
    VF_CHECK_LAUNCH("vf_pack_geglu_rows");
    return VF_OK;
}
```

variantformer_amd/ops.py:

```python
from __future__ import annotations

import contextlib
import contextvars
import math

import torch

from . import _lib, runtime
from ._lib import (EPI_BF16, EPI_F32, EPI_GEGLU_BF16, EPI_GELU_BF16, EPI_GELU_F32, EPI_RES_F32, VF_BF16,
                   VF_F16, VF_F32, check)

_CDT: contextvars.ContextVar = contextvars.ContextVar("vf_compute_dtype", default=torch.bfloat16)


@contextlib.contextmanager
def compute_dtype(dtype):
    assert dtype in (torch.bfloat16, torch.float16), dtype
    token = _CDT.set(dtype)
    try:
        yield
    finally:
        _CDT.reset(token)


def cdt():
    return _CDT.get()


def _is16(dtype) -> bool:
    return dtype in (torch.bfloat16, torch.float16)


def _stream() -> int:
    return torch.cuda.current_stream().cuda_stream


class KernelTimer:

    def __init__(self, detail: bool = False):
        self.records = {}
        self.detail = detail
        self.order = []

    def time(self, name: str, flops, nbytes: float, launch, geometry: str = "", family: str = ""):
        a, b = torch.cuda.Event(enable_timing=True), torch.cuda.Event(enable_timing=True)
        a.record()
        out = launch()
        b.record()
        rec = [a, b, flops, nbytes]
        self.records.setdefault(name, []).append(rec)
        if self.detail:
            self.order.append((name, geometry, family, None if callable(flops) else float(flops), float(nbytes)))
        if family:
            self.records.setdefault(f"{name}:{family}", []).append(rec)
        if self.detail and geometry:
            self.records.setdefault(f"{name}[{geometry}]", []).append(rec)
        return out

    def summary(self) -> dict:
        torch.cuda.synchronize()
        out = {}
        for name, recs in self.records.items():
            for r in recs:
                if callable(r[2]):
                    r[2] = float(r[2]())
            ms = sum(a.elapsed_time(b) for a, b, _, _ in recs)
            out[name] = {"launches": len(recs), "total_ms": ms, "flops": sum(r[2] for r in recs),
                         "bytes": sum(r[3] for r in recs)}
        return out


TIMER: KernelTimer | None = None
_SCOPE = ""


class scope:

    def __init__(self, name: str):
        self.name = name

    def __enter__(self):
        global _SCOPE
        self.prev, _SCOPE = _SCOPE, self.name

    def __exit__(self, *exc):
        global _SCOPE
        _SCOPE = self.prev
        return False


def _run(launch, record) -> None:
    if TIMER is not None:
        name, flops, nbytes, geometry, family = record()
        TIMER.time(name, flops, nbytes, launch, geometry, family)
    else:
        launch()


def _dev(*ts):
    cur = None
    for t in ts:
        if t is None:
            continue
        if not t.is_cuda:
            raise _lib.VFError("variantformer_amd ops need tensors on the GPU (no CPU fallback)")
        if cur is None:
            cur = torch.cuda.current_device()
        if t.device.index != cur:
            raise _lib.VFError(f"tensor on cuda:{t.device.index} but the current device is cuda:{cur}: "
                               "libvf_hip launches on the current device's stream (wrap the call in torch.cuda.device)")


def _ptr(t):
    return 0 if t is None else t.data_ptr()


def _dt(dtype) -> int:
    if dtype == torch.float32:
        return VF_F32
    if dtype == torch.bfloat16:
        return VF_BF16
    if dtype == torch.float16:
        return VF_F16
    raise _lib.VFError(f"unsupported dtype {dtype}")


def gemm(a: torch.Tensor, w: torch.Tensor, bias: torch.Tensor | None, epilogue: int,
         residual: torch.Tensor | None = None, out: torch.Tensor | None = None, variant: int = 0,
         family: str = "") -> torch.Tensor:
    _dev(a, w, bias, residual, out)
    assert _is16(a.dtype) and w.dtype == a.dtype and a.dim() == 2 and w.dim() == 2
    assert a.stride(1) == 1 and w.is_contiguous() and a.shape[1] == w.shape[1]
    M, K = a.shape
    N = w.shape[0]
    n_out = N // 2 if epilogue == EPI_GEGLU_BF16 else N
    odt = torch.float32 if epilogue in (EPI_F32, EPI_RES_F32, EPI_GELU_F32) else a.dtype
    if out is None:
        out = torch.empty((M, n_out), dtype=odt, device=a.device)
    assert out.dtype == odt and out.shape == (M, n_out) and out.stride(1) == 1
    ldr = 0
    if residual is not None:
        assert residual.dtype == torch.float32 and residual.shape == (M, N) and residual.stride(1) == 1
        ldr = residual.stride(0)
    if bias is not None:
        assert bias.dtype == torch.float32 and bias.numel() == N and bias.is_contiguous()
    lib = _lib.load()

    def launch():
        lda = a.stride(0) if M > 1 else max(a.stride(0), K)
        ldo = out.stride(0) if M > 1 else max(out.stride(0), n_out)
        f16 = a.dtype == torch.float16
        if variant:
            fn = lib.vf_gemm_f16_ex if f16 else lib.vf_gemm_bf16_ex
            check(fn(a.data_ptr(), lda, w.data_ptr(), _ptr(bias), _ptr(residual), ldr, out.data_ptr(),
                     ldo, M, N, K, epilogue, variant, _stream()), "vf_gemm_ex")
        else:
            fn = lib.vf_gemm_f16 if f16 else lib.vf_gemm_bf16
            check(fn(a.data_ptr(), lda, w.data_ptr(), _ptr(bias), _ptr(residual), ldr, out.data_ptr(),
                     ldo, M, N, K, epilogue, _stream()), "vf_gemm")
    _run(launch, lambda: ("gemm", 2.0 * M * N * K,
                          2.0 * (M * K + N * K) + out.numel() * out.element_size() + (0 if residual is None else 4.0 * M * N),
                          f"M={M} N={N} K={K} epi={epilogue}", family or _SCOPE))
    return out


class LnStream:
    __slots__ = ("x", "x16", "stats", "scale", "t16")

    def __init__(self, x, x16, stats, scale: float = 1.0, t16=None):
        self.x, self.x16, self.stats, self.scale = x, x16, stats, float(scale)
        self.t16 = t16

    def operand16(self):
        return self.x16 if self.scale == 1.0 else cast16(self.x, self.x16.dtype)


def x16_scale_for(dtype) -> float:
    return 1.0 if dtype != torch.float16 else 2.0 ** -4


LN_FOLD_RATIO_LIMIT = 8.0
_ALERT: dict = {}


def _alert_flag(device) -> torch.Tensor:
    sid = torch.cuda.current_stream(device).cuda_stream if device.type == "cuda" else 0
    key = (device.type, device.index, sid)
    if key not in _ALERT:
        _ALERT[key] = torch.zeros(1, dtype=torch.int32, device=device)
    return _ALERT[key]


def ln_fold_alert_clear(device) -> None:
    if device.type == "cuda":
        _alert_flag(device).zero_()


def ln_fold_alert_take(device):
    if device.type != "cuda":
        return None
    flag = _alert_flag(device)
    bits = flag.clone()
    flag.zero_()
    return bits


def ln_fold_abs_limit() -> float:
    scales = []
    if cdt() == torch.float16:
        scales.append(x16_scale_for(torch.float16))
    if runtime.env().trunk16 == "f16":
        scales.append(T16_SCALE)
    return 60000.0 / max(scales) if scales else 0.0


def ln_fold_alert(device, reset: bool = True) -> int:
    if device.type != "cuda":
        return 0
    sid = torch.cuda.current_stream(device).cuda_stream
    key = (device.type, device.index, sid)
    if key not in _ALERT:
        return 0
    hit = int(_ALERT[key].item())
    if hit and reset:
        _ALERT[key].zero_()
    return hit


def ln_stream(x: torch.Tensor, eps: float = 1e-5, raise_alert: bool = True) -> LnStream:
    _dev(x)
    assert x.dtype == torch.float32 and x.is_contiguous() and x.dim() == 2
    M, D = x.shape
    x16 = torch.empty((M, D), dtype=cdt(), device=x.device)
    stats = torch.empty((M, 2), dtype=torch.float32, device=x.device)
    scale = x16_scale_for(x16.dtype)
    alert_ptr = _alert_flag(x.device).data_ptr() if raise_alert else 0

    def launch():
        check(_lib.load().vf_row_stats_cast2(x.data_ptr(), M, D, eps, x16.data_ptr(), _dt(x16.dtype), scale, LN_FOLD_RATIO_LIMIT,
                                             ln_fold_abs_limit(), alert_ptr, stats.data_ptr(), _stream()),
              "vf_row_stats_cast")
    _run(launch, lambda: ("layernorm", 0.0, float(M) * D * 6, f"stats_cast D={D}", _SCOPE))
    return LnStream(x, x16, stats, scale)


def ln_stream_rows(s: LnStream, rows: torch.Tensor) -> LnStream:
    return LnStream(None if s.x is None else gather_rows_f32(s.x, None, rows), gather_rows_bf16(s.x16, rows),
                    gather_rows_f32(s.stats, None, rows), s.scale,
                    None if s.t16 is None else gather_rows_bf16(s.t16, rows))


T16_SCALE = 2.0 ** -4


def trunk16_of(x: torch.Tensor, raise_alert: bool = True) -> torch.Tensor:
    _dev(x)
    assert x.dtype == torch.float32 and x.is_contiguous() and x.dim() == 2
    M, D = x.shape
    t16 = torch.empty((M, D), dtype=torch.float16, device=x.device)
    stats = torch.empty((M, 2), dtype=torch.float32, device=x.device)

    alert_ptr = _alert_flag(x.device).data_ptr() if raise_alert else 0

    def launch():
        check(_lib.load().vf_row_stats_cast2(x.data_ptr(), M, D, 1e-5, t16.data_ptr(), VF_F16, T16_SCALE, 1e30,
                                             60000.0 / T16_SCALE, alert_ptr, stats.data_ptr(), _stream()),
              "vf_row_stats_cast")
    _run(launch, lambda: ("layernorm", 0.0, float(M) * D * 6, f"trunk16_of D={D}", _SCOPE))
    return t16


def gemm_ln_consumer(s: LnStream, w: torch.Tensor, bias: torch.Tensor, colsum: torch.Tensor, epilogue: int,
                     family: str = "") -> torch.Tensor:
    a = s.x16
    _dev(a, w, bias, colsum, s.stats)
    assert _is16(a.dtype) and w.dtype == a.dtype and a.shape[1] == w.shape[1] and a.stride(1) == 1
    assert epilogue in (EPI_BF16, EPI_GEGLU_BF16, EPI_F32)
    M, K = a.shape
    N = w.shape[0]
    n_out = N // 2 if epilogue == EPI_GEGLU_BF16 else N
    out = torch.empty((M, n_out), dtype=torch.float32 if epilogue == EPI_F32 else a.dtype, device=a.device)
    lib = _lib.load()

    def launch():
        check(lib.vf_gemm_ln(a.data_ptr(), a.stride(0) if M > 1 else max(a.stride(0), K), w.data_ptr(), bias.data_ptr(),
                             0, 0, VF_F32, out.data_ptr(), n_out, M, N, K, epilogue, _dt(a.dtype), s.stats.data_ptr(),
                             colsum.data_ptr(), 0, 0, 0, 1.0, 1.0, _stream()), "vf_gemm_ln")
    _run(launch, lambda: ("gemm", 2.0 * M * N * K, 2.0 * (M * K + N * K) + out.numel() * out.element_size() + 8.0 * M,
                          f"M={M} N={N} K={K} epi={epilogue} ln=consumer", family or _SCOPE))
    return out


def gemm_ln_producer(a: torch.Tensor, w: torch.Tensor, bias: torch.Tensor | None, residual,
                     eps: float = 1e-5, family: str = "", need_x: bool = True, trunk16: torch.Tensor | None = None,
                     need_t16: bool = False) -> LnStream:
    assert residual is None if trunk16 is not None else not need_t16
    res16 = residual if isinstance(residual, LnStream) else None
    res32 = None if res16 is not None else residual
    _dev(a, w, bias, res32, None if res16 is None else res16.x16, trunk16)
    assert _is16(a.dtype) and w.dtype == a.dtype and a.shape[1] == w.shape[1] and a.stride(1) == 1
    M, K = a.shape
    N = w.shape[0]
    out = torch.empty((M, N), dtype=torch.float32, device=a.device) if need_x else None
    t_out = torch.empty((M, N), dtype=torch.float16, device=a.device) if need_t16 else None
    x16 = torch.empty((M, N), dtype=a.dtype, device=a.device)
    n_parts = (N + 31) // 32
    part = torch.empty((n_parts, M, 2), dtype=torch.float32, device=a.device)
    stats = torch.empty((M, 2), dtype=torch.float32, device=a.device)
    scale = x16_scale_for(a.dtype)
    alert = _alert_flag(a.device)
    lib = _lib.load()
    lda = a.stride(0) if M > 1 else max(a.stride(0), K)
    if trunk16 is not None:
        assert trunk16.dtype == torch.float16 and trunk16.shape == (M, N) and trunk16.stride(1) == 1
        epi, res_bytes = EPI_RES_F32, (2.0 + (2.0 if need_t16 else 0.0)) * M * N
        tag = "-t16" + ("" if need_t16 else "-in")

        def launch():
            check(lib.vf_gemm_ln_t16(a.data_ptr(), lda, w.data_ptr(), _ptr(bias), trunk16.data_ptr(), trunk16.stride(0),
                                     1.0 / T16_SCALE, _ptr(out), N, M, N, K, _dt(a.dtype), x16.data_ptr(), N, part.data_ptr(),
                                     scale, _ptr(t_out), N, T16_SCALE, _stream()), "vf_gemm_ln_t16")
    else:
        epi = EPI_F32 if residual is None else EPI_RES_F32
        if res32 is not None:
            assert res32.dtype == torch.float32 and res32.shape == (M, N) and res32.stride(1) == 1
            r_ptr, r_ld, r_dt, r_scale, res_bytes, tag = res32.data_ptr(), res32.stride(0), VF_F32, 1.0, 4.0 * M * N, ""
        elif res16 is not None:
            r = res16.x16
            assert r.dtype == a.dtype and r.shape == (M, N) and r.stride(1) == 1
            r_ptr, r_ld, r_dt, r_scale, res_bytes, tag = r.data_ptr(), r.stride(0), _dt(r.dtype), 1.0 / res16.scale, 2.0 * M * N, "-r16"
        else:
            r_ptr, r_ld, r_dt, r_scale, res_bytes, tag = 0, 0, VF_F32, 1.0, 0.0, ""

        def launch():
            check(lib.vf_gemm_ln(a.data_ptr(), lda, w.data_ptr(), _ptr(bias), r_ptr, r_ld, r_dt, _ptr(out), N, M, N, K, epi,
                                 _dt(a.dtype), 0, 0, x16.data_ptr(), N, part.data_ptr(), scale, r_scale, _stream()), "vf_gemm_ln")

    def finalize():
        check(lib.vf_ln_finalize2(part.data_ptr(), M, n_parts, N, eps, scale, LN_FOLD_RATIO_LIMIT, ln_fold_abs_limit(),
                                  alert.data_ptr(), stats.data_ptr(), _stream()), "vf_ln_finalize")
    _run(launch, lambda: ("gemm", 2.0 * M * N * K,
                          2.0 * (M * K + N * K) + M * N * ((4.0 if need_x else 0.0) + 2.0) + res_bytes + 8.0 * M * n_parts,
                          f"M={M} N={N} K={K} epi={epi} ln=producer{'' if need_x else '-nox'}{tag}", family or _SCOPE))
    _run(finalize, lambda: ("layernorm", 0.0, 8.0 * M * (n_parts + 1), f"finalize D={N}", _SCOPE))
    return LnStream(out, x16, stats, scale, t_out)


def pack_geglu_rows(w: torch.Tensor, bias: torch.Tensor | None):
    _dev(w, bias)
    assert _is16(w.dtype) and w.is_contiguous()
    wo = torch.empty_like(w)
    bo = torch.empty_like(bias) if bias is not None else None
    check(_lib.load().vf_pack_geglu_rows(w.data_ptr(), _ptr(bias), wo.data_ptr(), _ptr(bo), w.shape[0], w.shape[1],
                                         _stream()), "vf_pack_geglu_rows")
    return wo, bo


ATTN_Q_AT_START, ATTN_Q_LOG2 = 1, 2


def attn_counted_keys(q: torch.Tensor, kv_table: torch.Tensor, log2_count: torch.Tensor, cu_q: torch.Tensor, max_q: int,
                      n_heads: int, head_dim: int, family: str = "") -> torch.Tensor:
    _dev(q, kv_table, log2_count, cu_q)
    assert _is16(q.dtype) and kv_table.dtype == q.dtype and q.stride(1) == 1 and kv_table.stride(1) == 1
    assert log2_count.dtype == torch.float32 and log2_count.is_contiguous() and cu_q.dtype == torch.int32
    D = n_heads * head_dim
    n_seq, C = cu_q.numel() - 1, kv_table.shape[0]
    assert log2_count.shape == (n_seq, C) and kv_table.shape[1] >= 2 * D
    out = torch.empty((q.shape[0], D), dtype=q.dtype, device=q.device)

    def launch():
        check(_lib.load().vf_attn_counted_keys(q.data_ptr(), q.stride(0), kv_table.data_ptr(), kv_table.stride(0),
                                               log2_count.data_ptr(), cu_q.data_ptr(), n_seq, int(max_q), C, n_heads, head_dim,
                                               out.data_ptr(), out.stride(0), _dt(q.dtype), _stream()), "vf_attn_counted_keys")
    _run(launch, lambda: ("attn", 4.0 * q.shape[0] * C * D, 2.0 * D * 2 * q.shape[0],
                          f"H={n_heads} dh={head_dim} max_q={int(max_q)} counted_keys={C}", family or _SCOPE))
    return out


def softmax_counted(scores: torch.Tensor, log2_count: torch.Tensor, cu_q: torch.Tensor, max_q: int, n_heads: int, slots: int,
                    out_dtype=None, family: str = "") -> torch.Tensor:
    _dev(scores, log2_count, cu_q)
    assert scores.dtype == torch.float32 and scores.stride(1) == 1 and log2_count.dtype == torch.float32 and log2_count.is_contiguous()
    T, n_seq, C = scores.shape[0], cu_q.numel() - 1, log2_count.shape[1]
    assert scores.shape[1] >= n_heads * slots and log2_count.shape[0] == n_seq
    dt = cdt() if out_dtype is None else out_dtype
    out = torch.empty((T, n_heads * slots), dtype=dt, device=scores.device)

    def launch():
        check(_lib.load().vf_softmax_counted(scores.data_ptr(), scores.stride(0), log2_count.data_ptr(), cu_q.data_ptr(), n_seq,
                                             int(max_q), n_heads, slots, C, out.data_ptr(), out.stride(0), _dt(dt), _stream()),
              "vf_softmax_counted")
    _run(launch, lambda: ("attn", 0.0, float(T) * n_heads * slots * 6, f"softmax_counted H={n_heads} C={C}", family or _SCOPE))
    return out


def attn_rows_supported(head_dim: int, alibi: bool, n_seq: int, n_heads: int, max_q: int, max_k: int, q_log2: bool) -> bool:
    return bool(_lib.load().vf_attn_rows_supported(int(head_dim), int(bool(alibi)), int(n_seq), int(n_heads), int(max_q),
                                                   int(max_k), ATTN_Q_LOG2 if q_log2 else 0))


ATTN_CLASS_DIMS = (32, 48, 64, 96, 128)


def attn_varlen(q: torch.Tensor, k: torch.Tensor, v: torch.Tensor, cu_q: torch.Tensor, cu_k: torch.Tensor | None,
                max_q: int, max_k: int, n_heads: int, head_dim: int, slopes: torch.Tensor | None = None,
                scale: float | None = None, out: torch.Tensor | None = None, q_at_start: bool = False,
                family: str = "", q_log2: bool = False, rows: torch.Tensor | None = None) -> torch.Tensor:
    _dev(q, k, v, cu_q, cu_k, slopes, out, rows)
    for t in (q, k, v):
        assert _is16(t.dtype) and t.dtype == q.dtype and t.dim() == 2 and t.stride(1) == 1
    assert cu_q.dtype == torch.int32 and (cu_k is None or cu_k.dtype == torch.int32)
    D = n_heads * head_dim
    tq = q.shape[0] if rows is None else rows.numel()
    tk = k.shape[0] if rows is None else rows.numel()
    if rows is not None:
        assert rows.dtype == torch.int64 and rows.is_contiguous() and cu_k is None
    if out is None:
        out = torch.empty((tq, D), dtype=q.dtype, device=q.device)
    if scale is None:
        scale = 1.0 / math.sqrt(head_dim)
    if slopes is not None:
        assert slopes.dtype == torch.float32 and slopes.numel() == n_heads
    def launch():
        lib = _lib.load()
        flags = (ATTN_Q_AT_START if q_at_start else 0) | (ATTN_Q_LOG2 if q_log2 else 0)
        if rows is not None:
            check(lib.vf_attn_varlen_fwd_rows(q.data_ptr(), k.data_ptr(), v.data_ptr(), out.data_ptr(), q.stride(0), k.stride(0),
                                              v.stride(0), out.stride(0), cu_q.data_ptr(), None, cu_q.numel() - 1, int(max_q),
                                              int(max_k), n_heads, head_dim, _ptr(slopes), float(scale), _dt(q.dtype), flags,
                                              rows.data_ptr(), rows.data_ptr(), _stream()), "vf_attn_varlen_fwd_rows")
            return
        fwd = lib.vf_attn_varlen_fwd_v2 if head_dim in ATTN_CLASS_DIMS else lib.vf_attn_varlen_fwd_v3
        check(fwd(q.data_ptr(), k.data_ptr(), v.data_ptr(), out.data_ptr(), q.stride(0), k.stride(0),
                  v.stride(0), out.stride(0), cu_q.data_ptr(), _ptr(cu_k), cu_q.numel() - 1, int(max_q),
                  int(max_k), n_heads, head_dim, _ptr(slopes), float(scale), _dt(q.dtype), flags,
                  _stream()), "vf_attn_varlen_fwd")

    def flops():
        lq = (cu_q[1:] - cu_q[:-1]).double()
        lk = lq if cu_k is None else (cu_k[1:] - cu_k[:-1]).double()
        return 4.0 * float((lq * lk).sum().item()) * D
    _run(launch, lambda: ("attn", flops, 2.0 * D * (2 * tq + 2 * tk),
                          f"H={n_heads} dh={head_dim} max_q={int(max_q)} max_k={int(max_k)}" + (" rows" if rows is not None else ""),
                          family or _SCOPE))
    return out


def attn_probs(q: torch.Tensor, k: torch.Tensor, cu_rows: torch.Tensor, cu_k: torch.Tensor, max_rows: int, max_k: int,
               n_heads: int, head_dim: int, q_rows: torch.Tensor | None = None, q_log2: bool = True, per_head: bool = False,
               scale: float | None = None, out: torch.Tensor | None = None, family: str = "",
               slopes: torch.Tensor | None = None, q_pos: torch.Tensor | None = None, k_rows: torch.Tensor | None = None):
    _dev(q, k, cu_rows, cu_k, q_rows, out, slopes, q_pos, k_rows)
    for t in (q, k):
        assert _is16(t.dtype) and t.dtype == q.dtype and t.dim() == 2 and t.stride(1) == 1
    assert cu_rows.dtype == torch.int32 and cu_k.dtype == torch.int32 and cu_rows.numel() == cu_k.numel()
    D = n_heads * head_dim
    if q_rows is not None:
        assert q_rows.dtype == torch.int64 and q_rows.is_contiguous()
    R = q.shape[0] if q_rows is None else q_rows.numel()
    n_out = R * n_heads if per_head else R
    if out is None:
        out = torch.empty((n_out, int(max_k)), dtype=torch.float32, device=q.device)
    assert out.dtype == torch.float32 and out.dim() == 2 and out.shape[0] == n_out and out.shape[1] >= max_k and out.stride(1) == 1
    stats = torch.empty((R, n_heads, 2), dtype=torch.float32, device=q.device)
    if scale is None:
        scale = 1.0 / math.sqrt(head_dim)
    if slopes is not None:
        assert slopes.dtype == torch.float32 and slopes.is_contiguous() and slopes.numel() == n_heads
    if q_pos is not None:
        assert q_pos.dtype == torch.int32 and q_pos.is_contiguous() and q_pos.numel() == R
    if k_rows is not None:
        assert k_rows.dtype == torch.int64 and k_rows.is_contiguous()
    tk = k.shape[0] if k_rows is None else k_rows.numel()
    idx_bytes = 2.0 * ((8.0 * tk if k_rows is not None else 0.0) + (4.0 * R if slopes is not None and q_pos is not None else 0.0)
                       + (4.0 * n_heads if slopes is not None else 0.0) + (8.0 * R if q_rows is not None else 0.0))

    def launch():
        if R == 0:
            return
        check(_lib.load().vf_attn_probs_v2(q.data_ptr(), q.stride(0), k.data_ptr(), k.stride(0), _ptr(q_rows), cu_rows.data_ptr(),
                                        cu_k.data_ptr(), cu_rows.numel() - 1, int(max_rows), int(max_k), n_heads, head_dim,
                                        float(scale), _dt(q.dtype), ATTN_Q_LOG2 if q_log2 else 0, int(bool(per_head)),
                                           stats.data_ptr(), out.data_ptr(), out.stride(0), _ptr(slopes),
                                           _ptr(q_pos), _ptr(k_rows), _stream()),
              "vf_attn_probs_v2")

# ... 250 lines not shown
```

variantformer_amd/runtime.py:

```python
from __future__ import annotations

import contextvars
import os
from dataclasses import dataclass, replace


@dataclass(frozen=True)
class Switches:
    rows_in_attention: bool = True
    counted_context_keys: bool = True
    lowrank_context: bool = True
    layer0_qkv_table: bool = True
    pool_before_down_projection: bool = True
    overlap_cre_stream: bool = True


_SW: contextvars.ContextVar = contextvars.ContextVar("vf_switches", default=Switches())


def switches() -> Switches:
    return _SW.get()


class override:

    def __init__(self, **kw):
        self.kw = kw

    def __enter__(self):
        self.token = _SW.set(replace(_SW.get(), **self.kw))
        return _SW.get()

    def __exit__(self, *exc):
        _SW.reset(self.token)
        return False


def set_for_this_context(**kw) -> Switches:
    _SW.set(replace(_SW.get(), **kw))
    return _SW.get()


TRUNK16_MODES = ("f16", "0")


@dataclass(frozen=True)
class Env:
    ln_fold: bool
    trunk16: str


def read_env() -> Env:
    mode = os.environ.get("VF_TRUNK16", "f16")
    if mode not in TRUNK16_MODES:
        raise ValueError(f"VF_TRUNK16={mode!r}: the supported values are 'f16' (default) and '0' (fp32 trunk)")
    return Env(ln_fold=os.environ.get("VF_LN_FOLD", "1") != "0", trunk16=mode)


_ENV: contextvars.ContextVar = contextvars.ContextVar("vf_env", default=None)


def env() -> Env:
    e = _ENV.get()
    return e if e is not None else read_env()


class forward_env:

    def __init__(self, fold_off: bool = False):
        self.fold_off = bool(fold_off)

    def __enter__(self):
        cur = _ENV.get()
        e = cur if cur is not None else read_env()
        if self.fold_off and e.ln_fold:
            e = replace(e, ln_fold=False)
        self.token = _ENV.set(e)
        return e

    def __exit__(self, *exc):
        _ENV.reset(self.token)
        return False
```

variantformer_amd/seq2gene/modules/layers.py:

```python
from __future__ import annotations

import math
import threading
from typing import Optional

import torch
import torch.nn as nn

from ... import attn_maps, ops, runtime, weights


def get_alibi_slopes(n: int) -> torch.Tensor:
    def pow2(n):
        start = 2 ** (-(2 ** -(math.log2(n) - 3)))
        return [start * start ** i for i in range(n)]

    def slopes(n):
        if math.log2(n).is_integer():
            return pow2(n)
        c = 2 ** math.floor(math.log2(n))
        return pow2(c) + slopes(2 * c)[0::2][: n - c]
    return torch.tensor(slopes(n))


def _pack(lin: nn.Linear, norm, geglu: bool, wscale: float, bscale: float, qrows: int):
    wf = lin.weight.detach().float()
    def rows(scale):
        v = torch.full((wf.shape[0], 1), float(scale), dtype=torch.float32, device=wf.device)
        if qrows:
            v[qrows:] = 1.0
        return v
    w = wf if norm is None else wf * norm.weight.detach().float()[None, :]
    wb = ops.cast16((w if wscale == 1.0 else w * rows(wscale)).contiguous())
    b = None if norm is None else wf @ norm.bias.detach().float()
    if lin.bias is not None:
        b = lin.bias.detach().float() if b is None else b + lin.bias.detach().float()
    if b is not None:
        b = (b if bscale == 1.0 else b * rows(bscale)[:, 0]).contiguous()
    if geglu:
        wb, b = ops.pack_geglu_rows(wb, b)
    return (wb, b) if norm is None else (wb, b, wb.float().sum(dim=1).contiguous())


def packed_linear(lin: nn.Linear, geglu: bool = False, wscale: float = 1.0, bscale: float = 1.0, qrows: int = 0):
    return weights.derived(lin, "_vf_packed", (lin.weight, lin.bias), lambda: _pack(lin, None, geglu, wscale, bscale, qrows),
                           "plain", geglu, wscale, bscale, qrows)


def packed_linear_ln(lin: nn.Linear, norm: nn.LayerNorm, geglu: bool = False, wscale: float = 1.0, qrows: int = 0):
    return weights.derived(lin, "_vf_packed", (lin.weight, lin.bias, norm.weight, norm.bias),
                           lambda: _pack(lin, norm, geglu, wscale, wscale, qrows), "ln", geglu, wscale, qrows)


_LN_FOLD_TLS = threading.local()
_LN_FOLD_DISABLED = False


class ln_fold_forced_off:

    def __enter__(self):
        _LN_FOLD_TLS.off = getattr(_LN_FOLD_TLS, "off", 0) + 1
        return self

    def __exit__(self, *exc):
        _LN_FOLD_TLS.off -= 1
        return False


def ln_fold_disable():
    global _LN_FOLD_DISABLED
    _LN_FOLD_DISABLED = True


def ln_fold_reenable():
    global _LN_FOLD_DISABLED
    _LN_FOLD_DISABLED = False


def ln_fold_enabled(*widths: int) -> bool:
    return (not _LN_FOLD_DISABLED and getattr(_LN_FOLD_TLS, "off", 0) == 0 and all(int(w) % 64 == 0 for w in widths)
            and runtime.env().ln_fold)


def trunk16_enabled() -> bool:
    return trunk16_mode() == "f16"


def trunk16_mode() -> str:
    return runtime.env().trunk16


def trunk_f16_active() -> bool:
    return trunk16_mode() == "f16" and ops.cdt() == torch.bfloat16


def _as_stream(x):
    return x if isinstance(x, ops.LnStream) else ops.ln_stream(x)


def _as_tensor(x):
    return x.x if isinstance(x, ops.LnStream) else x


def layer_streams(layer, src, context=None):
    if ln_fold_enabled(layer.norm1.weight.numel(), layer.linear_geglu_2.in_features):
        return _as_stream(src), context
    return _as_tensor(src), _as_tensor(context)


def normalise(x, norm: nn.LayerNorm):
    return x if isinstance(x, ops.LnStream) else ops.layernorm(x, norm.weight, norm.bias)


def ln_linear(x, norm, lin: nn.Linear, epilogue: int = ops.EPI_BF16, geglu: bool = False, wscale: float = 1.0, qrows: int = 0,
              out_rows: slice | None = None, family: str = "") -> torch.Tensor:
    cut = (lambda t: t) if out_rows is None else (lambda t: None if t is None else t[out_rows])
    if isinstance(x, ops.LnStream):
        w, b, c = packed_linear_ln(lin, norm, geglu=geglu, wscale=wscale, qrows=qrows)
        return ops.gemm_ln_consumer(x, cut(w), cut(b), cut(c), epilogue, family=family)
    h = normalise(x, norm) if x.dtype == torch.float32 else x
    w, b = packed_linear(lin, geglu=geglu, wscale=wscale, bscale=wscale, qrows=qrows)
    return ops.gemm(h, cut(w), cut(b), epilogue, family=family)


def out_residual(a, w, b, x):
    if isinstance(x, ops.LnStream):
        return ops.gemm_ln_producer(a, w, b, x, need_x=False)
    return ops.gemm(a, w, b, ops.EPI_RES_F32, residual=x)


def down_projection(hg, lin: nn.Linear, s, keep_x: bool = True, rows32: bool = False, pooled=None):
    w2, b2 = packed_linear(lin)
    folded = isinstance(s, ops.LnStream)
    t16 = None
    if folded and trunk_f16_active():
        t16 = s.t16 if s.t16 is not None else ops.trunk16_of(s.x)
    x32 = s.x if folded else s
    if pooled is not None:
        if t16 is not None:
            return pooled(hg, w2, b2, res16=t16, res16_scale=1.0 / ops.T16_SCALE)
        return pooled(hg, w2, b2, res_f32=x32) if x32 is not None else pooled(hg, w2, b2, res16=s.x16, res16_scale=1.0 / s.scale)
    if t16 is None and x32 is not None and (rows32 or not folded):
        return ops.gemm(hg, w2, b2, ops.EPI_RES_F32, residual=x32)
    need_x = keep_x or rows32
    if t16 is not None:
        out = ops.gemm_ln_producer(hg, w2, b2, None, need_x=need_x, trunk16=t16, need_t16=not need_x)
    else:
        out = ops.gemm_ln_producer(hg, w2, b2, s if x32 is None else x32, need_x=need_x)
    return out.x if rows32 else out


def feed_forward(x, norm, layer, s, **how):
    hg = ln_linear(x, norm, layer.linear_geglu_1, ops.EPI_GEGLU_BF16, geglu=True)
    return down_projection(hg, layer.linear_geglu_2, s, **how)


def _cu_from_padded(batch: int, seqlen: int, device) -> torch.Tensor:
    return torch.arange(0, batch + 1, dtype=torch.int32, device=device) * seqlen


def unpad_input(hidden: torch.Tensor, keep_mask: torch.Tensor):
    seqlens = keep_mask.sum(dim=-1, dtype=torch.int32)
    indices = torch.nonzero(keep_mask.flatten(), as_tuple=False).flatten()
    cu = torch.nn.functional.pad(torch.cumsum(seqlens, 0, dtype=torch.int32), (1, 0))
    flat = hidden.reshape(-1, hidden.shape[-1]).float().contiguous()
    packed = ops.gather_rows_f32(flat, None, indices)
    return packed, indices, cu, int(seqlens.max().item()), seqlens


def pad_input(packed: torch.Tensor, indices: torch.Tensor, batch: int, seqlen: int) -> torch.Tensor:
    inv = torch.full((batch * seqlen,), -1, dtype=torch.int64, device=packed.device)
    inv[indices] = torch.arange(indices.numel(), device=packed.device)
    zero = torch.zeros((1, packed.shape[-1]), dtype=torch.float32, device=packed.device)
    out = ops.gather_rows_f32(packed.float().contiguous(), zero, inv)
    return out.view(batch, seqlen, packed.shape[-1])


class MHA(nn.Module):

    def __init__(self, embed_dim, num_heads, dropout=0.0, use_flash_attn=True, use_alibi=False, cross_attn=False, **kw):
        super().__init__()
        assert embed_dim % num_heads == 0
        self.embed_dim, self.num_heads, self.cross_attn = embed_dim, num_heads, cross_attn
        self.head_dim = embed_dim // num_heads
        self.q_log2_scale = math.log2(math.e) / math.sqrt(self.head_dim)
        self.use_alibi = use_alibi
        if cross_attn:
            self.Wq = nn.Linear(embed_dim, embed_dim)
            self.Wkv = nn.Linear(embed_dim, 2 * embed_dim)
        else:
            self.Wqkv = nn.Linear(embed_dim, 3 * embed_dim)
        self.out_proj = nn.Linear(embed_dim, embed_dim)
        self.family = "cross" if cross_attn else "self"
        if use_alibi:
            self.register_buffer("alibi_slopes", get_alibi_slopes(num_heads).float(), persistent=False)
        else:
            self.alibi_slopes = None

    def project_qkv(self, x, norm, out_rows: slice | None = None, family: str = "") -> torch.Tensor:
        return ln_linear(x, norm, self.Wqkv, wscale=self.q_log2_scale, qrows=self.embed_dim, out_rows=out_rows, family=family)

    def project_q(self, x, norm) -> torch.Tensor:
        return ln_linear(x, norm, self.Wq, wscale=self.q_log2_scale)

    def project_kv(self, x_kv_bf16: torch.Tensor) -> torch.Tensor:
        w, b = packed_linear(self.Wkv)
        return ops.gemm(x_kv_bf16, w, b, ops.EPI_BF16)

    def project_kv_of(self, ctx) -> torch.Tensor:
        if not isinstance(ctx, ops.LnStream):
            return self.project_kv(ops.cast16(ctx) if ctx.dtype == torch.float32 else ctx)
        if ctx.scale == 1.0:
            return self.project_kv(ctx.x16)
        w, b = packed_linear(self.Wkv, wscale=1.0 / ctx.scale)
        return ops.gemm(ctx.x16, w, b, ops.EPI_BF16)

    def attend(self, x, norm, kv_bf16, cu_q, max_q, cu_k=None, max_k=None) -> torch.Tensor:
        D = self.embed_dim
        if self.cross_attn:
            q = self.project_q(x, norm)
            cap = attn_maps.running()
            if cap is not None:
                if self.alibi_slopes is not None:
                    raise NotImplementedError("attention maps: cross_alibi (a positional bias in the gene -> cCRE cross "
                                              "attention) runs in the per-(gene, tissue) evaluation order, which is not captured")
                if cap.contributions:
                    cap.record(q, kv_bf16[:, :D], self.num_heads, self.head_dim, family=self.family, v=kv_bf16[:, D:],
                               s_gram=self.contrib_gram())
                else:
                    cap.record(q, kv_bf16[:, :D], self.num_heads, self.head_dim, family=self.family)
            return ops.attn_varlen(q, kv_bf16[:, :D], kv_bf16[:, D:], cu_q, cu_k, max_q, max_k,
                                   self.num_heads, self.head_dim, self.alibi_slopes, family=self.family, q_log2=True)
        return self.attend_qkv(self.project_qkv(x, norm), cu_q, max_q)

    def contrib_gram(self) -> torch.Tensor:
        H, dh = self.num_heads, self.head_dim

        def build():
            w = packed_linear(self.out_proj)[0].double()
            return (w.t() @ w).view(H, dh, H, dh).permute(0, 2, 1, 3).float().contiguous()
        return weights.derived(self, "_vf_contrib_gram", (self.out_proj.weight,), build)

    def lowrank_tables(self, norm, table: torch.Tensor):
        assert self.cross_attn
        C, D, H, dh = table.shape[0], self.embed_dim, self.num_heads, self.head_dim
        Cp = next((c for c in range(C + (C & 1), 17, 2) if (H * c) % 64 == 0), None)
        if Cp is None:
            return None
        prm = [table, self.Wq.weight, self.Wq.bias, self.Wkv.weight, self.Wkv.bias, self.out_proj.weight, self.out_proj.bias,
               None if norm is None else norm.weight, None if norm is None else norm.bias]
        def build():
            kv = table.detach().float() @ self.Wkv.weight.detach().float().t() + self.Wkv.bias.detach().float()
            k, v = kv[:, :D].view(C, H, dh), kv[:, D:].view(C, H, dh)
            wq = self.Wq.weight.detach().float().view(H, dh, D)
            z = torch.zeros((H, Cp, D), dtype=torch.float32, device=table.device)
            z[:, :C] = torch.einsum("chd,hdk->hck", k, wq) * self.q_log2_scale
            zb = torch.zeros((H, Cp), dtype=torch.float32, device=table.device)
            zb[:, :C] = torch.einsum("chd,hd->hc", k, self.Wq.bias.detach().float().view(H, dh)) * self.q_log2_scale
            z, zb = z.view(H * Cp, D), zb.view(H * Cp)
            u = torch.zeros((D, H, Cp), dtype=torch.float32, device=table.device)
            u[:, :, :C] = torch.einsum("nhd,chd->nhc", self.out_proj.weight.detach().float().view(D, H, dh), v)
            u16 = ops.cast16(u.view(D, H * Cp).contiguous())
            bo = self.out_proj.bias.detach().float().contiguous()
            if norm is not None:
                wz = ops.cast16((z * norm.weight.detach().float()[None, :]).contiguous())
                bz = (z @ norm.bias.detach().float() + zb).contiguous()
                cs = wz.float().sum(dim=1).contiguous()
            else:
                wz, bz, cs = ops.cast16(z.contiguous()), zb.contiguous(), None
            return wz, bz, cs, u16, bo, Cp
        return weights.derived(self, "_vf_lowrank_ln" if norm is not None else "_vf_lowrank", prm, build)

    def cross_lowrank(self, h, tables, log2_count, cu_q, max_q, x):
        wz, bz, cs, u16, bo, Cp = tables
        if isinstance(h, ops.LnStream):
            sc = ops.gemm_ln_consumer(h, wz, bz, cs, ops.EPI_F32)
        else:
            sc = ops.gemm(h, wz, bz, ops.EPI_F32)
        w16 = ops.softmax_counted(sc, log2_count, cu_q, max_q, self.num_heads, Cp, family=self.family)
        return out_residual(w16, u16, bo, x)

    def attend_counted(self, x, norm, counted, cu_q, max_q) -> torch.Tensor:
        assert self.cross_attn and self.alibi_slopes is None
        return ops.attn_counted_keys(self.project_q(x, norm), counted[0], counted[1], cu_q, max_q, self.num_heads, self.head_dim,
                                     family=self.family)

    def attend_qkv(self, qkv, cu_q, max_q, rows=None) -> torch.Tensor:
        D = self.embed_dim
        if rows is not None and not (runtime.switches().rows_in_attention and ops.attn_rows_supported(
                self.head_dim, self.alibi_slopes is not None, cu_q.numel() - 1, self.num_heads, max_q, max_q, True)):
            qkv, rows = ops.gather_rows_bf16(qkv, rows), None
        cap = attn_maps.running_self()
        if cap is not None:
            cap.record_self(qkv[:, :D], qkv[:, D:2 * D], self.num_heads, self.head_dim, self.alibi_slopes, rows=rows,
                            family=self.family)
        return ops.attn_varlen(qkv[:, :D], qkv[:, D:2 * D], qkv[:, 2 * D:], cu_q, None, max_q, max_q,
                               self.num_heads, self.head_dim, self.alibi_slopes, family=self.family,
                               q_log2=True, rows=rows)

    def out_proj_residual(self, a, x):
        w, b = packed_linear(self.out_proj)
        return out_residual(a, w, b, x)

    def self_block(self, x, norm, cu, max_len, qkv=None):
        a = self.attend(x, norm, None, cu, max_len) if qkv is None else self.attend_qkv(qkv[0], cu, max_len, rows=qkv[1])
        return self.out_proj_residual(a, x)

    def cross_block(self, x, norm, cu_q, max_q, context=None, cu_k=None, max_k=None, context_kv=None, context_counted=None):
        h = normalise(x, norm)
        lr = None
        if context_counted is not None and runtime.switches().lowrank_context and len(context_counted) > 2:
            lr = self.lowrank_tables(norm if isinstance(x, ops.LnStream) else None, context_counted[2])
        if lr is not None:
            return self.cross_lowrank(h, lr, context_counted[1], cu_q, max_q, x)
        if context_counted is not None:
            a = self.attend_counted(h, norm, context_counted, cu_q, max_q)
        else:
            if context_kv is None:
                context_kv = self.project_kv_of(context)
            a = self.attend(h, norm, context_kv, cu_q, max_q, cu_k, max_k)
        return self.out_proj_residual(a, x)

    def forward(self, x, x_kv=None, cu_seqlens=None, max_seqlen=None, cu_seqlens_k=None, max_seqlen_k=None, **kw):
        in_dtype, in_shape = x.dtype, x.shape
        if cu_seqlens is None:
            B, S = x.shape[:2]
            cu_seqlens, max_seqlen = _cu_from_padded(B, S, x.device), S
            x = x.reshape(B * S, -1)
            if x_kv is not None:
                Sk = x_kv.shape[1]
                cu_seqlens_k, max_seqlen_k = _cu_from_padded(B, Sk, x.device), Sk
                x_kv = x_kv.reshape(B * Sk, -1)
        cd = x.dtype if x.dtype in (torch.bfloat16, torch.float16) else ops.cdt()
        with ops.compute_dtype(cd):
            return self._forward_cd(x, x_kv, cu_seqlens, max_seqlen, cu_seqlens_k, max_seqlen_k, in_dtype, in_shape, cd)

    def _forward_cd(self, x, x_kv, cu_seqlens, max_seqlen, cu_seqlens_k, max_seqlen_k, in_dtype, in_shape, cd):
        xb = x if x.dtype == cd else ops.cast16(x.float().contiguous())
        kv = None
        if self.cross_attn:
            src = x_kv if x_kv is not None else x
            kv = self.project_kv(src if src.dtype == cd else ops.cast16(src.float().contiguous()))
            if cu_seqlens_k is None:
                cu_seqlens_k, max_seqlen_k = cu_seqlens, max_seqlen
        a = self.attend(xb, None, kv, cu_seqlens, max_seqlen, cu_seqlens_k, max_seqlen_k)
        w, b = packed_linear(self.out_proj)
        out = ops.gemm(a, w, b, ops.EPI_F32 if in_dtype == torch.float32 else ops.EPI_BF16)
        return out.to(in_dtype).view(in_shape)


class FlashAttLayer(nn.Module):

    def __init__(self, d_model, nhead, hidden_dim=2048, dropout=0.1, use_alibi=False, cross_attn=False,
                 flash_attn_3=False):
        super().__init__()
        self.cross_attn = cross_attn
        if cross_attn and flash_attn_3:
            raise NotImplementedError("flash-attention-3 is not supported at this time")
        self.MHA = MHA(d_model, nhead, dropout=dropout, use_flash_attn=True, use_alibi=use_alibi, cross_attn=cross_attn)

    def forward(self, src, cntx=None, src_key_padding_mask=None, context_key_padding_mask=None,
                precision=torch.float32, unpad_info=None, context_unpad_info=None):
        if unpad_info is not None:
            kw = {"cu_seqlens": unpad_info["cu_seqlens"], "max_seqlen": unpad_info["max_seqlen"]}
            if self.cross_attn:
                assert cntx is not None
                if context_unpad_info is not None:
                    kw.update(cu_seqlens_k=context_unpad_info["cu_seqlens"], max_seqlen_k=context_unpad_info["max_seqlen"])
                return self.MHA(src, cntx, **kw)
            return self.MHA(src, **kw)
        if src_key_padding_mask is not None:
            batch, seqlen = src.shape[:2]
            xs, idx, cu, mx, _ = unpad_input(src, ~src_key_padding_mask)
            kw = {"cu_seqlens": cu, "max_seqlen": mx}
            if self.cross_attn:
                assert cntx is not None and context_key_padding_mask is not None, \
                    "context_key_padding_mask must be provided if src_key_padding_mask is provided"
                cs, _, cuk, mxk, _ = unpad_input(cntx, ~context_key_padding_mask)
                out = self.MHA(xs, cs, cu_seqlens_k=cuk, max_seqlen_k=mxk, **kw)
            else:
                out = self.MHA(xs, **kw)
            return pad_input(out, idx, batch, seqlen).to(src.dtype)
        return self.MHA(src, cntx) if self.cross_attn else self.MHA(src)


class ContextFlashAttentionEncoderLayer(nn.Module):

    def __init__(self, d_model, nhead, hidden_dim=2048, dropout=0.1, batch_first=True, use_alibi=False,
                 make_data_kv=False, mlp_dout=0.0, cross_alibi=False, flash_attn_3=False):
        super().__init__()
        self.mixer = FlashAttLayer(d_model, nhead, dropout=dropout, use_alibi=use_alibi, cross_attn=False)
        self.crossMHA = FlashAttLayer(d_model, nhead, dropout=dropout, use_alibi=cross_alibi, cross_attn=True,
                                      flash_attn_3=flash_attn_3)
        self.norm1 = nn.LayerNorm(d_model)
        self.norm2 = nn.LayerNorm(d_model)
        self.norm3 = nn.LayerNorm(d_model)
        self.linear_geglu_1 = nn.Linear(d_model, hidden_dim)
        self.dropout = nn.Dropout(mlp_dout)
        self.linear_geglu_2 = nn.Linear(hidden_dim // 2, d_model)
        self.use_alibi = use_alibi
        self.num_heads = nhead
        self.make_data_kv = make_data_kv
        self.activation = nn.GELU()
        if use_alibi:
            self.register_buffer("m", get_alibi_slopes(self.num_heads))

    def self_qkv_of_unique_rows(self, rows_a, rows_b, idx, rows_b_used=None, with_stream: bool = False):
        if not ln_fold_enabled(self.norm1.weight.numel(), self.linear_geglu_2.in_features):
            return None
        sa = ops.ln_stream(rows_a.float().contiguous())
        qa = self.mixer.MHA.project_qkv(sa, self.norm1)
        tab_b = rows_b.float().contiguous()
        if rows_b_used is not None:
            ops.ln_stream(tab_b[rows_b_used].contiguous())
        sb = ops.ln_stream(tab_b, raise_alert=rows_b_used is None)
        qb = self.mixer.MHA.project_qkv(sb, self.norm1)
        both = torch.cat([qa, qb], dim=0)
        idx2 = torch.where(idx >= 0, idx, rows_a.shape[0] - idx - 1)
        qkv = (both, idx2)
        if not with_stream:
            return qkv
        stream = None
        if trunk_f16_active():
            x16 = ops.gather_rows_bf16(torch.cat([sa.x16, sb.x16], dim=0), idx2)
            t16 = ops.gather_rows_bf16(torch.cat([ops.trunk16_of(sa.x), ops.trunk16_of(sb.x, raise_alert=rows_b_used is None)],
                                                 dim=0), idx2)
            stream = ops.LnStream(None, x16, None, sa.scale, t16)
        return qkv, stream

    def forward_packed(self, src, cu_src, max_src, context=None, cu_ctx=None, max_ctx=None, context_kv=None,
                       cu_cross_q=None, max_cross_q=None, self_qkv=None, keep_x=True, context_counted=None):
        if self.make_data_kv:
            return self._forward_packed_data_kv(src, cu_src, max_src, context, cu_ctx, max_ctx)
        s, context = layer_streams(self, src, context)
        x1 = self.mixer.MHA.self_block(s, self.norm1, cu_src, max_src, qkv=self_qkv)
        x2 = self.crossMHA.MHA.cross_block(x1, self.norm2, cu_src if cu_cross_q is None else cu_cross_q,
                                           max_src if max_cross_q is None else max_cross_q, context, cu_ctx, max_ctx,
                                           context_kv, context_counted)
        return feed_forward(x2, self.norm3, self, s, keep_x=keep_x)

    def _forward_packed_data_kv(self, src, cu_src, max_src, context, cu_ctx, max_ctx):
        src, context = _as_tensor(src), _as_tensor(context)
        if src is None or context is None:
            raise RuntimeError("make_data_kv layers need the fp32 rows of their input streams (run them with VF_LN_FOLD=0 "
                               "when they sit inside a LayerNorm-folded stack)")
        assert context.shape == src.shape and (cu_ctx is None or cu_ctx is cu_src or torch.equal(cu_ctx, cu_src)), \
            "make_data_kv: src and context must have the same shape (reference seq2reg/modules.py:79)"
        cross = self.crossMHA.MHA
        x1 = self.mixer.MHA.self_block(src, self.norm1, cu_src, max_src)
        kv = cross.project_kv(normalise(x1, self.norm2))
        a = cross.attend(ops.cast16(context), None, kv, cu_src, max_src, cu_src, max_src)
        x2 = cross.out_proj_residual(a, x1)
        return feed_forward(x2, self.norm3, self, src)

    def forward_packed_rows(self, src, cu_src, max_src, rows, cu_rows, context, cu_ctx, max_ctx, cu_cross_rows,
                            max_cross_rows):
        if self.make_data_kv:
            raise NotImplementedError("make_data_kv: the cross attention's rows are context rows; no registry-only form")
        mha, D = self.mixer.MHA, self.mixer.MHA.embed_dim
        s, ctx = layer_streams(self, src, context)
        folded = isinstance(s, ops.LnStream)
        if isinstance(context, ops.LnStream) and not folded:
            ctx = context.operand16()
        h = normalise(s, self.norm1)
        kv = mha.project_qkv(h, self.norm1, out_rows=slice(D, None))
        hr = ops.ln_stream_rows(h, rows) if folded else ops.gather_rows_bf16(h, rows)
        q = mha.project_qkv(hr, self.norm1, out_rows=slice(0, D))
        cap = attn_maps.running_self()
        if cap is not None:
            cap.record_self(q, kv[:, :D], mha.num_heads, mha.head_dim, mha.alibi_slopes, family=mha.family + "_registry_rows")
        a = ops.attn_varlen(q, kv[:, :D], kv[:, D:], cu_rows, cu_src, 1, max_src, mha.num_heads, mha.head_dim,
                            mha.alibi_slopes, q_at_start=True, family=mha.family + "_registry_rows",
                            q_log2=True)
        sr = hr if folded else ops.gather_rows_f32(s, None, rows)
        x1 = mha.out_proj_residual(a, sr)
        x2 = self.crossMHA.MHA.cross_block(x1, self.norm2, cu_cross_rows, max_cross_rows, ctx, cu_ctx, max_ctx)
        return feed_forward(x2, self.norm3, self, sr, rows32=True)

    def forward(self, src, context, src_key_padding_mask=None, context_padding_mask=None, precision=torch.float32,
                unpad_info=None, context_unpad_info=None, gene_unpad_info=None):
        cd = {torch.float16: torch.float16, torch.float32: torch.float16, torch.bfloat16: torch.bfloat16}.get(precision, ops.cdt())
        with ops.compute_dtype(cd):
            return self._forward_ref(src, context, src_key_padding_mask, context_padding_mask, unpad_info,
                                     context_unpad_info, gene_unpad_info)

    def _forward_ref(self, src, context, src_key_padding_mask, context_padding_mask, unpad_info, context_unpad_info,
                     gene_unpad_info):
        if context_padding_mask is None and src_key_padding_mask is not None:
            context_padding_mask = src_key_padding_mask.clone()
        info = gene_unpad_info if gene_unpad_info is not None else unpad_info
        if info is not None:
            cinfo = context_unpad_info if context_unpad_info is not None else info
            return _as_tensor(self.forward_packed(src.float().contiguous(), info["cu_seqlens"], info["max_seqlen"],
                                                  context.float().contiguous(), cinfo["cu_seqlens"], cinfo["max_seqlen"])).to(src.dtype)
        batch, seqlen = src.shape[:2]
        if src_key_padding_mask is None:
            xs, cu, mx, idx = src.reshape(batch * seqlen, -1).float().contiguous(), _cu_from_padded(batch, seqlen, src.device), seqlen, None
            cs, cuk, mxk = context.reshape(-1, context.shape[-1]).float().contiguous(), _cu_from_padded(batch, context.shape[1], src.device), context.shape[1]
        else:
            xs, idx, cu, mx, _ = unpad_input(src, ~src_key_padding_mask)
            cs, _, cuk, mxk, _ = unpad_input(context, ~context_padding_mask)
        out = _as_tensor(self.forward_packed(xs, cu, mx, cs, cuk, mxk))
        if idx is None:
            return out.view(batch, seqlen, -1).to(src.dtype)
        return pad_input(out, idx, batch, seqlen).to(src.dtype)


class FlashAttentionEncoderLayer(nn.Module):

    def __init__(self, d_model, nhead, hidden_dim=2048, dropout=0.1, batch_first=True, use_alibi=False,
                 make_data_kv=False, mlp_dout=0.0):
        super().__init__()
        self.mixer = FlashAttLayer(d_model, nhead, dropout=dropout, use_alibi=use_alibi, cross_attn=False)
        self.norm1 = nn.LayerNorm(d_model)
        self.norm2 = nn.LayerNorm(d_model)
        self.norm3 = nn.LayerNorm(d_model)
        self.linear_geglu_1 = nn.Linear(d_model, hidden_dim)
        self.dropout = nn.Dropout(mlp_dout)
        self.linear_geglu_2 = nn.Linear(hidden_dim // 2, d_model)
        self.use_alibi, self.num_heads, self.make_data_kv = use_alibi, nhead, make_data_kv
        self.activation = nn.GELU()
        if use_alibi:
            self.register_buffer("m", get_alibi_slopes(self.num_heads))

    def forward_packed(self, src, cu_src, max_src, keep_x=True, **_):
        s = layer_streams(self, src)[0]
        x1 = self.mixer.MHA.self_block(s, self.norm1, cu_src, max_src)
        return feed_forward(x1, self.norm2, self, s, keep_x=keep_x)


class ContextFlashCrossAttentionEncoderLayer(nn.Module):

    def __init__(self, d_model, nhead, hidden_dim=2048, dropout=0.1, batch_first=True, use_alibi=False,
                 make_data_kv=False, mlp_dout=0.0, cross_alibi=False, flash_attn_3=False):
        super().__init__()
        self.crossMHA = FlashAttLayer(d_model, nhead, dropout=dropout, use_alibi=cross_alibi, cross_attn=True,
                                      flash_attn_3=flash_attn_3)
        self.norm1 = nn.LayerNorm(d_model)
        self.norm2 = nn.LayerNorm(d_model)
        self.linear_geglu_1 = nn.Linear(d_model, hidden_dim)
        self.dropout = nn.Dropout(mlp_dout)
        self.linear_geglu_2 = nn.Linear(hidden_dim // 2, d_model)
        self.use_alibi, self.num_heads, self.make_data_kv = use_alibi, nhead, make_data_kv
        self.activation = nn.GELU()
        if use_alibi:
            self.register_buffer("m", get_alibi_slopes(self.num_heads))

    def forward_packed(self, src, cu_src, max_src, context=None, cu_ctx=None, max_ctx=None, context_kv=None,
                       cu_cross_q=None, max_cross_q=None, keep_x=True):
        cross = self.crossMHA.MHA
        if self.make_data_kv:
            src, context = _as_tensor(src), _as_tensor(context)
            assert src is not None and context is not None and context.shape == src.shape, \
                "make_data_kv: src and context must have the same shape"
            kv = cross.project_kv(normalise(src, self.norm1))
            a = cross.attend(ops.cast16(context), None, kv, cu_src, max_src, cu_src, max_src)
            return feed_forward(cross.out_proj_residual(a, src), self.norm2, self, src)
        s, context = layer_streams(self, src, context)
        x1 = cross.cross_block(s, self.norm1, cu_src if cu_cross_q is None else cu_cross_q,
                               max_src if max_cross_q is None else max_cross_q, context, cu_ctx, max_ctx, context_kv)
        return feed_forward(x1, self.norm2, self, s, keep_x=keep_x)


class StartToken(nn.Module):

    def __init__(self, emb_dim):
        super().__init__()
        self.start_token = nn.Parameter(torch.randn(1, 1, emb_dim))

    def forward(self, x):
        return torch.ones(x.size(0), 1, x.size(2), device=x.device) * self.start_token


class AddContext(nn.Module):

    def __init__(self, num_tissues, emb_dim):
        super().__init__()
        self.num_registry_tokens = num_tissues
        self.registry_tokens = nn.Embedding(num_tissues, emb_dim)

# ... 74 lines not shown
```

variantformer_amd/seq2reg/model.py:

```python
from __future__ import annotations

import math
import types

import torch
import torch.nn as nn

from .. import ops, runtime, weights
from ..seq2gene.modules.layers import ContextFlashAttentionEncoderLayer, ln_fold_enabled, trunk16_enabled, trunk_f16_active
from ..utils.constants import REF_CREs
from .modules import FlashTransformerLayer


LAYER0_QKV_TABLE_MAX_BYTES = 1 << 30
_LAYER0_SLOTS = {torch.bfloat16: "_vf_layer0_qkv_bf16", torch.float16: "_vf_layer0_qkv_fp16"}


def positionalencoding1d(d_model: int, length: int) -> torch.Tensor:
    if d_model % 2 != 0:
        raise ValueError("Cannot use sin/cos positional encoding with odd dim (got dim={:d})".format(d_model))
    pe = torch.zeros(length, d_model)
    position = torch.arange(0, length).unsqueeze(1)
    div_term = torch.exp(torch.arange(0, d_model, 2, dtype=torch.float) * -(math.log(10000.0) / d_model))
    pe[:, 0::2] = torch.sin(position.float() * div_term)
    pe[:, 1::2] = torch.cos(position.float() * div_term)
    return pe


class Seq2RegPredictor(nn.Module):
    def __init__(self, vocab_size: int, embedding_dim: int, num_heads: int, num_layers: int, num_tissues: int,
                 num_classes: int, learning_rate: float = 1e-4, loss_fn=("cross_entropy", "0"), seq_pool: str = "mean",
                 cre_type: str = "multi", token_length: int = None, use_context: bool = False,
                 positional_encoding: str = "sinusoidal", use_flash: bool = False, majority_weight: float = None,
                 weight_decay: float = 0.0, lr_scale: float = 1.0, strand_agg: str = "mean",
                 expand_context: bool = False, mlp_dout: float = 0.1, tissues: list = None, **kwargs):
        super().__init__()
        hp = dict(vocab_size=vocab_size, embedding_dim=embedding_dim, num_heads=num_heads, num_layers=num_layers,
                  num_tissues=num_tissues, num_classes=num_classes, learning_rate=learning_rate, loss_fn=loss_fn,
                  seq_pool=seq_pool, cre_type=cre_type, token_length=token_length, use_context=use_context,
                  positional_encoding=positional_encoding, use_flash=use_flash, majority_weight=majority_weight,
                  weight_decay=weight_decay, lr_scale=lr_scale, strand_agg=strand_agg, expand_context=expand_context,
                  mlp_dout=mlp_dout, tissues=tissues)
        hp.update(kwargs)
        self.hparams = types.SimpleNamespace(**hp)
        assert use_flash, "Only Flash is supported"
        assert positional_encoding in ["sinusoidal", "alibi"], "Position encoding must be either 'sinusoidal' or 'alibi'"
        assert seq_pool in ["mean", "max", "linear"]
        self.token_embedding = nn.Embedding(vocab_size, embedding_dim)
        self.pos_encoding_type = positional_encoding
        self.seq_pool = seq_pool
        self.use_context = use_context
        self.expand_context_type = expand_context
        self.strand_agg = strand_agg
        self.num_classes = num_classes
        self.tissues = tissues
        use_alibi = positional_encoding == "alibi"
        if use_context:
            self.context_embedding = nn.Embedding(len(REF_CREs), embedding_dim)
            if expand_context:
                self.expand_context = nn.Linear(1, token_length)
        if not use_alibi:
            self.position_encoding = positionalencoding1d(embedding_dim, token_length)
        self._pe_dev = None
        if use_context:
            self.transformer_encoder = nn.ModuleList(
                [ContextFlashAttentionEncoderLayer(d_model=embedding_dim, nhead=num_heads, batch_first=True,
                                                   use_alibi=use_alibi, mlp_dout=mlp_dout) for _ in range(num_layers)])
            for l in self.transformer_encoder:
                l.mixer.MHA.family, l.crossMHA.MHA.family = "seq2reg_self", "seq2reg_ctx_cross"
        else:
            self.transformer_encoder = nn.ModuleList(
                [FlashTransformerLayer(d_model=embedding_dim, nhead=num_heads, use_alibi=use_alibi) for _ in range(num_layers)])
        if seq_pool == "linear":
            self.linear = nn.Linear(token_length, 1)
        in_f = embedding_dim * 2 if strand_agg == "concat" else embedding_dim
        self.tissue_classifiers = nn.ModuleDict({str(t): nn.Linear(in_f, num_classes) for t in range(num_tissues)})

    def _pos_table(self, device):
        if self.pos_encoding_type != "sinusoidal":
            return None
        if self._pe_dev is None or self._pe_dev.device != device:
            self._pe_dev = self.position_encoding.to(device).contiguous()
        return self._pe_dev

    def _layer0_qkv_table(self, device):
        l0 = self.transformer_encoder[0]
        pos = self._pos_table(device)
        V = self.token_embedding.weight.shape[0]
        key_L = pos.shape[0] if pos is not None else 1
        prm = [self.token_embedding.weight, l0.norm1.weight, l0.norm1.bias, l0.MHA.Wqkv.weight, l0.MHA.Wqkv.bias, pos]
        def build():
            for slot in _LAYER0_SLOTS.values():
                if not weights.built_from(self, slot, prm, key_L):
                    self.__dict__.pop(slot, None)
            ids = torch.arange(V, device=device, dtype=torch.int64).view(V, 1).expand(V, key_L).contiguous()
            pad = torch.zeros((V, key_L), dtype=torch.uint8, device=device)
            cu = (torch.arange(V + 1, device=device, dtype=torch.int32) * key_L).contiguous()
            alert = ops._alert_flag(device)
            before = alert.clone()
            s = ops.embed_stream(ids, pad, cu, self.token_embedding.weight, pos, V * key_L, need_t16=False)
            alert.copy_(before)
            return l0.MHA.project_qkv(s, l0.norm1, family="seq2reg")
        return weights.derived(self, _LAYER0_SLOTS[ops.cdt()], prm, build, key_L), key_L

    def _layer0_qkv_table_bytes(self) -> int:
        key_L = self.position_encoding.shape[0] if self.pos_encoding_type == "sinusoidal" else 1
        V, d = self.token_embedding.weight.shape
        return int(V) * int(key_L) * 3 * int(d) * 2

    def embed_packed(self, ids: torch.Tensor, pad: torch.Tensor, n_tokens: int, out_dtype=None,
                     max_len: int = 0, context: torch.Tensor | None = None):
        with runtime.forward_env():
            return self._embed_packed(ids, pad, n_tokens, out_dtype, max_len, context)

    def _embed_packed(self, ids, pad, n_tokens, out_dtype, max_len, context):
        W, L = ids.shape
        Lmax = max_len if 0 < max_len < L else L
        with ops.scope("seq2reg"):
            cu = ops.mask_to_cu_seqlens(pad)
            l0 = self.transformer_encoder[0]
            if (trunk_f16_active() and ln_fold_enabled(l0.norm1.weight.numel(), l0.linear_geglu_2.in_features)
                    and self.token_embedding.weight.shape[1] <= 2048):
                x = ops.embed_stream(ids, pad, cu, self.token_embedding.weight, self._pos_table(ids.device), n_tokens)
            else:
                x = ops.embed_pack(ids, pad, cu, self.token_embedding.weight, self._pos_table(ids.device), n_tokens)
            if self.use_context:
                if context is None or torch.is_floating_point(context):
                    raise NotImplementedError(
                        "a use_context tokenizer needs integer cCRE labels as context; the gene branch of the reference "
                        "passes a float zero tensor (model_combined_modulator.py:575-577), which nn.Embedding rejects there too")
                ctx = self._context_rows(pad, cu, context.to(ids.device).long().reshape(-1), n_tokens)
                n_layers = len(self.transformer_encoder)
                for li, layer in enumerate(self.transformer_encoder):
                    x = layer.forward_packed(x, cu, Lmax, context=ctx, cu_ctx=cu, max_ctx=Lmax,
                                             keep_x=not trunk16_enabled() or li + 1 == n_layers)
            else:
                n_layers = len(self.transformer_encoder)
                lg2 = self.transformer_encoder[-1].linear_geglu_2
                pool_in_layer = (self.seq_pool == "mean" and runtime.switches().pool_before_down_projection and lg2.in_features % 8 == 0 and
                                 lg2.out_features % 8 == 0 and max(lg2.in_features, lg2.out_features) <= 2048)
                qkv0 = None
                V = self.token_embedding.weight.shape[0]
                if (runtime.switches().layer0_qkv_table and ln_fold_enabled(l0.norm1.weight.numel(), l0.linear_geglu_2.in_features) and
                        self.token_embedding.weight.shape[1] <= 2048 and
                        self._layer0_qkv_table_bytes() <= LAYER0_QKV_TABLE_MAX_BYTES):
                    tab, key_L = self._layer0_qkv_table(ids.device)
                    qkv0 = (tab, ops.token_keys(ids, pad, cu, n_tokens, V, key_L))
                for li, layer in enumerate(self.transformer_encoder):
                    x = layer.forward_packed(x, cu, Lmax, last=li + 1 == n_layers, keep_x=not trunk16_enabled(),
                                             pool_mean=pool_in_layer and li + 1 == n_layers, qkv=qkv0 if li == 0 else None)
                if pool_in_layer:
                    od = ops.cdt() if out_dtype is None else out_dtype
                    return x if od == torch.float32 else ops.cast16(x, od)
            if isinstance(x, ops.LnStream):
                x = x.x
            if self.seq_pool == "mean":
                return ops.segment_mean(x, cu, out_dtype)
            if self.seq_pool == "max":
                m = ops.segment_max(x, cu)
                od = ops.cdt() if out_dtype is None else out_dtype
                return m if od == torch.float32 else ops.cast16(m, od)
            return ops.segment_linear(x, cu, pad, self.linear.weight.reshape(-1).contiguous(), self.linear.bias, out_dtype)

    def _context_rows(self, pad, cu, labels, n_tokens):
        lens = (cu[1:] - cu[:-1]).long()
        tok_label = torch.repeat_interleave(labels, lens, output_size=n_tokens).contiguous()
        table = self.context_embedding.weight.float().contiguous()
        if not self.expand_context_type:
            return ops.gather_rows_f32(table, None, tok_label)
        pos = torch.nonzero(pad.view(torch.uint8) == 0)[:, 1]
        scale = self.expand_context.weight[:, 0].float()[pos].contiguous()
        shift = self.expand_context.bias.float()[pos].contiguous()
        return ops.affine_rows(table, tok_label, scale, shift)

    def forward(self, x, padding_mask, tissue_vector=None, context=None, only_embed=False, precision=torch.float32):
        if not only_embed:
            raise NotImplementedError("only the embedding path (only_embed=True) is part of the inference hot path")
        b, ns, L = x.size()
        dev = self.token_embedding.weight.device
        ids = x.reshape(b * ns, L).to(dev).long().contiguous()
        pad = padding_mask.reshape(b * ns, L).to(dev).contiguous()
        n_tokens = int((~pad.bool()).sum().item())
        ctx = None
        if self.use_context and context is not None:
            ctx = torch.as_tensor(context).to(dev).reshape(-1)
            ctx = ctx if torch.is_floating_point(ctx) else ctx.long().repeat_interleave(ns)
        return self.embed_packed(ids, pad, n_tokens, torch.float32, context=ctx).view(b, ns, -1)
```

Before: 57.56 genes/sec.

## Read producer GEMM residual through a row index instead of gathering rows

Measured after the change: 57.79 genes/sec, median of 6. About the same (+0.4%).

```diff
diff --git a/include/vf_hip_rows.h b/include/vf_hip_rows.h
--- /dev/null
+++ b/include/vf_hip_rows.h
@@ -0,0 +1,23 @@
+#ifndef VF_HIP_ROWS_H
+#define VF_HIP_ROWS_H
+
+#include "vf_hip.h"
+
+#ifdef __cplusplus
+extern "C" {
+#endif
+
+int vf_gemm_ln_v2(const void* A, int64_t lda, const void* W, const float* bias, const void* residual, int64_t ldr,
+                  int residual_dtype, void* out, int64_t ldo, int M, int N, int K, int epilogue, int operand_dtype,
+                  const float* row_stats, const float* colsum, void* out16, int64_t ld16, float* part_stats,
+                  float x16_scale, float res16_scale, const void* res_idx, int res_idx_bytes, int64_t res_rows, int variant,
+                  void* stream);
+int vf_gemm_ln_t16_v2(const void* A, int64_t lda, const void* W, const float* bias, const void* residual_f16, int64_t ldr,
+                      float res_scale, void* out, int64_t ldo, int M, int N, int K, int operand_dtype, void* out16,
+                      int64_t ld16, float* part_stats, float x16_scale, void* t16_out, int64_t ldt16, float t16_scale,
+                      const void* res_idx, int res_idx_bytes, int64_t res_rows, int variant, void* stream);
+
+#ifdef __cplusplus
+}
+#endif
+#endif
diff --git a/variantformer_amd/_lib.py b/variantformer_amd/_lib.py
--- a/variantformer_amd/_lib.py
+++ b/variantformer_amd/_lib.py
@@ -70,6 +70,10 @@
 NEXT_SIGNATURES = {
     "vf_attn_contrib": [_p, _l, _p, _p, _l, _p, _p, _i, _i, _i, _i, _i, _i, _i, _p, _p, _l, _p],
 }
+ROWS_SIGNATURES = {
+    "vf_gemm_ln_v2": [_p, _l, _p, _p, _p, _l, _i, _p, _l, _i, _i, _i, _i, _i, _p, _p, _p, _l, _p, _f, _f, _p, _i, _l, _i, _p],
+    "vf_gemm_ln_t16_v2": [_p, _l, _p, _p, _p, _l, _f, _p, _l, _i, _i, _i, _i, _p, _l, _p, _f, _p, _l, _f, _p, _i, _l, _i, _p],
+}
 _RESTYPES = {"vf_last_error": C.c_char_p, "vf_last_kernel": C.c_char_p, "vf_bpe_create": C.c_void_p, "vf_bpe_destroy": None, "vf_bpe_encode": C.c_int64, "vf_bpe_encode_prefix": C.c_int64,
              "vf_vcf_open": C.c_void_p, "vf_vcf_close": None, "vf_vcf_num_records": C.c_int64,
              "vf_vcf_consensus": C.c_int64, "vf_build_windows": C.c_int64}
@@ -93,7 +97,7 @@
             "(run `python -m variantformer_amd.csrc.build` or __graft_entry__.build()). "
             "There is no CPU fallback for the product path.")
     lib = C.CDLL(path)
-    for name, argtypes in list(SIGNATURES.items()) + list(NEXT_SIGNATURES.items()):
+    for name, argtypes in list(SIGNATURES.items()) + list(NEXT_SIGNATURES.items()) + list(ROWS_SIGNATURES.items()):
         try:
             fn = getattr(lib, name)
         except AttributeError as e:
diff --git a/variantformer_amd/csrc/build.py b/variantformer_amd/csrc/build.py
--- a/variantformer_amd/csrc/build.py
+++ b/variantformer_amd/csrc/build.py
@@ -7,7 +7,8 @@
 
 HERE = os.path.dirname(os.path.abspath(__file__))
 SOURCES = ["vf_gemm.hip", "vf_attn.hip", "vf_misc.hip", "vf_bpe.cpp", "vf_vcf.cpp", "vf_host.cpp"]
-HEADERS = ["vf_common.h", os.path.join("..", "..", "include", "vf_hip.h"), os.path.join("..", "..", "include", "vf_hip_next.h")]
+HEADERS = ["vf_common.h", os.path.join("..", "..", "include", "vf_hip.h"), os.path.join("..", "..", "include", "vf_hip_next.h"),
+           os.path.join("..", "..", "include", "vf_hip_rows.h")]
 LIB = os.path.join(HERE, "libvf_hip.so")
 ARCH = "gfx950"
 EXTRA_FLAGS = {"vf_attn.hip": ["-fno-honor-nans"]}
diff --git a/variantformer_amd/csrc/vf_common.h b/variantformer_amd/csrc/vf_common.h
--- a/variantformer_amd/csrc/vf_common.h
+++ b/variantformer_amd/csrc/vf_common.h
@@ -4,6 +4,7 @@
 #include <stdio.h>
 #include "../../include/vf_hip.h"
 #include "../../include/vf_hip_next.h"
+#include "../../include/vf_hip_rows.h"
 
 typedef __attribute__((ext_vector_type(8))) __bf16 bf16x8_t;
 typedef __attribute__((ext_vector_type(4))) short s16x4_t;
diff --git a/variantformer_amd/csrc/vf_gemm.hip b/variantformer_amd/csrc/vf_gemm.hip
--- a/variantformer_amd/csrc/vf_gemm.hip
+++ b/variantformer_amd/csrc/vf_gemm.hip
@@ -20,8 +20,14 @@
 }
 
 struct LnArgs {
-    const float* row_stats;
-    const float* colsum;
+    union {
+        const float* row_stats;
+        const void* res_idx;
+    };
+    union {
+        const float* colsum;
+        int64_t res_rows;
+    };
     void* out16;
     float* part_stats;
     int64_t ld16;
@@ -33,10 +39,15 @@
     unsigned short* t16_out;
     int64_t ldt16;
     float t16_scale;
+    int res_idx64;
 };
-enum { VF_LN_NONE = 0, VF_LN_CONSUMER = 1, VF_LN_PRODUCER = 2, VF_LN_PRODUCER_R16 = 3, VF_LN_PRODUCER_T16 = 4 };
-constexpr bool ln_is_producer(int ln) { return ln == VF_LN_PRODUCER || ln == VF_LN_PRODUCER_R16 || ln == VF_LN_PRODUCER_T16; }
-constexpr bool ln_res_is_16(int ln) { return ln == VF_LN_PRODUCER_R16 || ln == VF_LN_PRODUCER_T16; }
+static_assert(sizeof(LnArgs) == 96, "LnArgs is a kernel argument: its size and layout are part of every GEMM kernel's code");
+enum { VF_LN_NONE = 0, VF_LN_CONSUMER = 1, VF_LN_PRODUCER = 2, VF_LN_PRODUCER_R16 = 3, VF_LN_PRODUCER_T16 = 4,
+       VF_LN_PRODUCER_R16M = 5, VF_LN_PRODUCER_T16M = 6 };
+constexpr bool ln_is_producer(int ln) { return ln >= VF_LN_PRODUCER && ln <= VF_LN_PRODUCER_T16M; }
+constexpr bool ln_res_is_16(int ln) { return ln >= VF_LN_PRODUCER_R16 && ln <= VF_LN_PRODUCER_T16M; }
+constexpr bool ln_is_t16(int ln) { return ln == VF_LN_PRODUCER_T16 || ln == VF_LN_PRODUCER_T16M; }
+constexpr bool ln_res_mapped(int ln) { return ln == VF_LN_PRODUCER_R16M || ln == VF_LN_PRODUCER_T16M; }
 
 template <int DT>
 __device__ __forceinline__ f32x4_t cvt4_16(u32x2_t v) {
@@ -112,12 +123,40 @@
 
 template <int DT, int LN, class V>
 __device__ __forceinline__ f32x4_t res_value(V v, const LnArgs& ln) {
-    if constexpr (LN == VF_LN_PRODUCER_T16) return cvt4_16<VF_F16>(v) * ln.res16_scale;
+    if constexpr (ln_is_t16(LN)) return cvt4_16<VF_F16>(v) * ln.res16_scale;
     else if constexpr (ln_res_is_16(LN)) {
         if constexpr (DT == VF_F16) return cvt4_16<DT>(v) * ln.res16_scale;
         else return cvt4_16<DT>(v);
     }
     else return v;
+}
+
+template <int NI>
+__device__ __forceinline__ void load_res_rows(const LnArgs& ln, int row_first, int row_step, int M, int (&tr)[NI]) {
+    const int last = (int)ln.res_rows - 1;
+    if (ln.res_idx64) {
+        const int64_t* ix = reinterpret_cast<const int64_t*>(ln.res_idx);
+        int64_t v[NI];
+#pragma unroll
+        for (int k = 0; k < NI; ++k) {
+            int m = row_first + k * row_step;
+            m = m < M ? m : M - 1;
+            v[k] = ix[m];
+        }
+#pragma unroll
+        for (int k = 0; k < NI; ++k) tr[k] = v[k] < 0 ? 0 : (v[k] > (int64_t)last ? last : (int)v[k]);
+    } else {
+        const int* ix = reinterpret_cast<const int*>(ln.res_idx);
+        int v[NI];
+#pragma unroll
+        for (int k = 0; k < NI; ++k) {
+            int m = row_first + k * row_step;
+            m = m < M ? m : M - 1;
+            v[k] = ix[m];
+        }
+#pragma unroll
+        for (int k = 0; k < NI; ++k) tr[k] = v[k] < 0 ? 0 : (v[k] > last ? last : v[k]);
+    }
 }
 
 template <int DT, int LN, int REGION>
@@ -126,7 +165,7 @@
                                                          int N, const LnArgs& ln) {
     constexpr int TM = 8, TN = 4, WT_M = 128, PITCH = 64 * 4 + 16, RP = 32, IMP = RP / 16, NPASS = TM / IMP;
     constexpr int RI = 8, NI = RP / RI;
-    constexpr bool T16 = LN == VF_LN_PRODUCER_T16;
+    constexpr bool T16 = ln_is_t16(LN), RMAP = ln_res_mapped(LN);
     static_assert(REGION >= RP * PITCH, "wide producer epilogue: staging region too small");
     int lane_e;
     asm volatile("v_mbcnt_lo_u32_b32 %0, -1, 0\n\tv_mbcnt_hi_u32_b32 %0, -1, %0" : "=v"(lane_e));
@@ -147,12 +186,20 @@
     const int64_t t16_step = (int64_t)RI * ln.ldt16;
     u32x4_t rbuf[2][NI];
     auto load_res_pass = [&](int ps, u32x4_t (&dst)[NI]) {
+        if constexpr (RMAP) {
+            int tr[NI];
+            load_res_rows<NI>(ln, (int)row0 + ps * NI * RI, RI, M, tr);
+#pragma unroll
+            for (int k = 0; k < NI; ++k)
+                dst[k] = *reinterpret_cast<const u32x4_t*>(reinterpret_cast<const char*>(ln.res16) + ((int64_t)tr[k] * ln.ldr16 + colc) * 2);
+        } else {
 #pragma unroll
         for (int k = 0; k < NI; ++k) {
             const int j = ps * NI + k;
             const char* rp = (j * RI < rows_left) ? res_run : res_last;
             res_run += res_step;
             dst[k] = *reinterpret_cast<const u32x4_t*>(rp);
+        }
         }
     };
     load_res_pass(0, rbuf[0]);
@@ -381,15 +428,27 @@
     const int no0 = (EPI == VF_EPI_GEGLU_BF16) ? (n0 + wn * WT_N) / 2 : (n0 + wn * WT_N);
     const int ep_row = lane / CR, ep_col = no0 + (lane % CR) * (16 / ES);
     constexpr bool RES_PRE = (EPI == VF_EPI_RES_F32) && (TN * TM <= 16);
-    constexpr bool R16 = ln_res_is_16(LN), T16 = LN == VF_LN_PRODUCER_T16;
+    constexpr bool R16 = ln_res_is_16(LN), T16 = ln_is_t16(LN), RMAP = ln_res_mapped(LN);
     using res_t = typename std::conditional<R16, u32x2_t, f32x4_t>::type;
     auto res_load = [&](int64_t m, int col) -> res_t {
         if constexpr (R16) return *reinterpret_cast<const u32x2_t*>(ln.res16 + m * ln.ldr16 + col);
         else return *reinterpret_cast<const f32x4_t*>(res + m * ldr + col);
     };
     res_t resv[RES_PRE ? NPASS : 1][RES_PRE ? NI : 1];
+    auto res_load_rows = [&](int ps, res_t* dst) {
+        if constexpr (RMAP) {
+            int tr[NI];
+            load_res_rows<NI>(ln, (int)mw0 + ps * RP + ep_row, RI, M, tr);
+            const int col = ep_col < N ? ep_col : N - 4;
+#pragma unroll
+            for (int k = 0; k < NI; ++k) dst[k] = res_load(tr[k], col);
+        }
+    };
     auto prefetch_residual = [&]() {
-        if (RES_PRE) {
+        if constexpr (RES_PRE && RMAP) {
+#pragma unroll
+            for (int ps = 0; ps < NPASS; ++ps) res_load_rows(ps, resv[RES_PRE ? ps : 0]);
+        } else if (RES_PRE) {
 #pragma unroll
             for (int ps = 0; ps < NPASS; ++ps)
 #pragma unroll
@@ -404,7 +463,9 @@
     constexpr bool RES_PIPE = (EPI == VF_EPI_RES_F32) && !RES_PRE;
     res_t rbuf[2][RES_PIPE ? NI : 1];
     auto load_res_pass = [&](int ps, res_t (&dst)[RES_PIPE ? NI : 1]) {
-        if (RES_PIPE) {
+        if constexpr (RES_PIPE && RMAP) {
+            res_load_rows(ps, dst);
+        } else if (RES_PIPE) {
 #pragma unroll
             for (int k = 0; k < NI; ++k) {
                 int64_t m = mw0 + ps * RP + k * RI + ep_row;
@@ -754,7 +815,7 @@
     const int rows_left = (int)(M - mw0) - ep_row;
     const int64_t row0 = mw0 + ep_row;
     const int colc = ep_col < N ? ep_col : N - 4;
-    constexpr bool R16 = ln_res_is_16(LN), T16 = LN == VF_LN_PRODUCER_T16;
+    constexpr bool R16 = ln_res_is_16(LN), T16 = ln_is_t16(LN), RMAP = ln_res_mapped(LN);
     using res_t = typename std::conditional<R16, u32x2_t, f32x4_t>::type;
     const char* const res_base = R16 ? reinterpret_cast<const char*>(ln.res16) : reinterpret_cast<const char*>(res);
     const int64_t res_ld = R16 ? ln.ldr16 : ldr;
@@ -775,7 +836,13 @@
     const int64_t t16_step = (int64_t)RI * ln.ldt16;
     res_t rbuf[2][RES ? NI : 1];
     auto load_res_pass = [&](int ps, res_t (&dst)[RES ? NI : 1]) {
-        if (RES) {
+        if constexpr (RMAP) {
+            int tr[NI];
+            load_res_rows<NI>(ln, (int)row0 + ps * NI * RI, RI, M, tr);
+#pragma unroll
+            for (int k = 0; k < NI; ++k)
+                dst[RES ? k : 0] = *reinterpret_cast<const res_t*>(res_base + ((int64_t)tr[k] * res_ld + colc) * RES_ES);
+        } else if (RES) {
 #pragma unroll
             for (int k = 0; k < NI; ++k) {
                 const int j = ps * NI + k;
@@ -1057,7 +1124,7 @@
         constexpr int PITCH = WT_NO * ES + 16;
         constexpr int REGION = (C::TILE_BYTES + C::SPARE_BYTES) / C::NW;
         constexpr int RP_FIT = (((REGION / PITCH) < WT_M ? (REGION / PITCH) : WT_M) / 16) * 16;
-        constexpr bool R16 = ln_res_is_16(LN), T16 = LN == VF_LN_PRODUCER_T16;
+        constexpr bool R16 = ln_res_is_16(LN), T16 = ln_is_t16(LN);
         constexpr int RP = (EPI == VF_EPI_RES_F32 && !R16 && RP_FIT > 16) ? 16 : RP_FIT;
         constexpr int IMP = RP / 16, NPASS = (TM + IMP - 1) / IMP;
         constexpr int CR = WT_NO * ES / 16, RI = 64 / CR, NI = RP / RI;
@@ -1428,10 +1495,11 @@
 
 template <int EPI, int DT, int LN>
 static int launch_gemm_ln(const void* A, int64_t lda, const void* W, const float* bias, const float* residual, int64_t ldr,
-                          void* out, int64_t ldo, int M, int N, int K, const LnArgs& ln, hipStream_t st) {
-    int variant = pick_variant(M, N, K, EPI);
+                          void* out, int64_t ldo, int M, int N, int K, const LnArgs& ln, hipStream_t st, int forced = 0) {
+    int variant = forced ? forced : pick_variant(M, N, K, EPI);
+    if (forced == 22 && K % 128 != 0) variant = 20;
     if constexpr (ln_res_is_16(LN)) {
-        if (variant == 20 && K % 128 == 0 && out == nullptr) variant = 22;
+        if (!forced && variant == 20 && K % 128 == 0 && out == nullptr) variant = 22;
     }
     switch (variant) {
         case 1: return launch_cfg<CfgA, EPI, DT, LN>(A, lda, W, bias, residual, ldr, out, ldo, M, N, K, st, ln);
@@ -1446,7 +1514,8 @@
                             int residual_dtype, void* out, int64_t ldo, int M, int N, int K, int epilogue,
                             const float* row_stats, const float* colsum, void* out16, int64_t ld16, float* part_stats,
                             float x16_scale, float res16_scale, void* stream, bool trunk = false, void* t16_out = nullptr,
-                            int64_t ldt16 = 0, float t16_scale = 1.0f) {
+                            int64_t ldt16 = 0, float t16_scale = 1.0f, const void* res_idx = nullptr, int res_idx_bytes = 0,
+                            int64_t res_rows = 0, int variant = 0) {
     VF_REQUIRE(A && W && (out || (out16 && part_stats)), "vf_gemm_ln: null pointer");
     VF_REQUIRE(M >= 0 && N > 0 && K > 0 && K % 64 == 0 && N % 8 == 0, "vf_gemm_ln: needs K %% 64 == 0, N %% 8 == 0 (N=%d K=%d)", N, K);
     VF_REQUIRE(lda % 8 == 0 && lda >= K, "vf_gemm_ln: lda=%lld must be >= K and a multiple of 8", (long long)lda);
@@ -1454,8 +1523,21 @@
                "vf_gemm_ln: pointers must be 16-byte aligned");
     const bool consumer = row_stats && colsum, producer = out16 && part_stats;
     VF_REQUIRE(consumer != producer, "vf_gemm_ln: give (row_stats, colsum) OR (out16, part_stats)");
+    VF_REQUIRE(variant == 0 || variant == 1 || variant == 5 || variant == 20 || variant == 22, "vf_gemm_ln_v2: unknown variant %d", variant);
+    if (res_idx) {
+        VF_REQUIRE(producer && epilogue == VF_EPI_RES_F32 && residual && residual_dtype != VF_F32,
+                   "vf_gemm_ln_v2: res_idx goes with a 16-bit residual of a producer (residual_dtype=%d)", residual_dtype);
+        VF_REQUIRE(res_idx_bytes == 4 || res_idx_bytes == 8, "vf_gemm_ln_v2: res_idx_bytes=%d must be 4 (int32) or 8 (int64)", res_idx_bytes);
+        VF_REQUIRE(res_rows >= 1 && res_rows <= 0x7fffffffLL, "vf_gemm_ln_v2: res_rows=%lld must be in 1 .. 2^31 - 1", (long long)res_rows);
+        VF_REQUIRE((uintptr_t)res_idx % res_idx_bytes == 0, "vf_gemm_ln_v2: misaligned res_idx");
+    }
     if (M == 0) return VF_OK;
     LnArgs ln{};
+    if (res_idx) {
+        ln.res_idx = res_idx;
+        ln.res_idx64 = res_idx_bytes == 8;
+        ln.res_rows = res_rows;
+    }
     ln.x16_scale = 1.0f;
     ln.res16_scale = 1.0f;
     hipStream_t st = (hipStream_t)stream;
@@ -1466,11 +1548,11 @@
         ln.row_stats = row_stats;
         ln.colsum = colsum;
         if (epilogue == VF_EPI_BF16)
-            return launch_gemm_ln<VF_EPI_BF16, DT, VF_LN_CONSUMER>(A, lda, W, bias, nullptr, 0, out, ldo, M, N, K, ln, st);
+            return launch_gemm_ln<VF_EPI_BF16, DT, VF_LN_CONSUMER>(A, lda, W, bias, nullptr, 0, out, ldo, M, N, K, ln, st, variant);
         if (epilogue == VF_EPI_F32)
-            return launch_gemm_ln<VF_EPI_F32, DT, VF_LN_CONSUMER>(A, lda, W, bias, nullptr, 0, out, ldo, M, N, K, ln, st);
+            return launch_gemm_ln<VF_EPI_F32, DT, VF_LN_CONSUMER>(A, lda, W, bias, nullptr, 0, out, ldo, M, N, K, ln, st, variant);
         VF_REQUIRE(epilogue == VF_EPI_GEGLU_BF16 && N % 32 == 0, "vf_gemm_ln: consumer epilogues are BF16, F32 and GEGLU_BF16");
-        return launch_gemm_ln<VF_EPI_GEGLU_BF16, DT, VF_LN_CONSUMER>(A, lda, W, bias, nullptr, 0, out, ldo, M, N, K, ln, st);
+        return launch_gemm_ln<VF_EPI_GEGLU_BF16, DT, VF_LN_CONSUMER>(A, lda, W, bias, nullptr, 0, out, ldo, M, N, K, ln, st, variant);
     }
     VF_REQUIRE(ld16 % 4 == 0 && ld16 >= N && ((uintptr_t)out16 % 8 == 0) && ((uintptr_t)part_stats % 8 == 0) && ldo % 4 == 0,
                "vf_gemm_ln: producer outputs must keep 8-byte alignment (ld16=%lld)", (long long)ld16);
@@ -1482,11 +1564,11 @@
     ln.rows = M;
     ln.x16_scale = x16_scale;
     if (epilogue == VF_EPI_F32)
-        return launch_gemm_ln<VF_EPI_F32, DT, VF_LN_PRODUCER>(A, lda, W, bias, nullptr, 0, out, ldo, M, N, K, ln, st);
+        return launch_gemm_ln<VF_EPI_F32, DT, VF_LN_PRODUCER>(A, lda, W, bias, nullptr, 0, out, ldo, M, N, K, ln, st, variant);
     VF_REQUIRE(epilogue == VF_EPI_RES_F32 && residual, "vf_gemm_ln: producer epilogues are F32 and RES_F32 (with a residual)");
     if (residual_dtype == VF_F32) {
         VF_REQUIRE(ldr % 4 == 0 && ((uintptr_t)residual % 16 == 0), "vf_gemm_ln: misaligned fp32 residual");
-        return launch_gemm_ln<VF_EPI_RES_F32, DT, VF_LN_PRODUCER>(A, lda, W, bias, (const float*)residual, ldr, out, ldo, M, N, K, ln, st);
+        return launch_gemm_ln<VF_EPI_RES_F32, DT, VF_LN_PRODUCER>(A, lda, W, bias, (const float*)residual, ldr, out, ldo, M, N, K, ln, st, variant);
     }
     if (trunk) {
         VF_REQUIRE(residual_dtype == VF_F16, "vf_gemm_ln_t16: the trunk residual is fp16");
@@ -1499,7 +1581,9 @@
         ln.t16_out = (unsigned short*)t16_out;
         ln.ldt16 = ldt16;
         ln.t16_scale = t16_scale;
-        return launch_gemm_ln<VF_EPI_RES_F32, DT, VF_LN_PRODUCER_T16>(A, lda, W, bias, (const float*)residual, ldr, out, ldo, M, N, K, ln, st);
+        if (res_idx)
+            return launch_gemm_ln<VF_EPI_RES_F32, DT, VF_LN_PRODUCER_T16M>(A, lda, W, bias, (const float*)residual, ldr, out, ldo, M, N, K, ln, st, variant);
+        return launch_gemm_ln<VF_EPI_RES_F32, DT, VF_LN_PRODUCER_T16>(A, lda, W, bias, (const float*)residual, ldr, out, ldo, M, N, K, ln, st, variant);
     }
     VF_REQUIRE(residual_dtype == DT, "vf_gemm_ln: a 16-bit residual must have the operand type");
     VF_REQUIRE(ldr % 4 == 0 && ((uintptr_t)residual % 8 == 0) && res16_scale > 0.f, "vf_gemm_ln: misaligned 16-bit residual");
@@ -1507,7 +1591,9 @@
     ln.res16 = (const unsigned short*)residual;
     ln.ldr16 = ldr;
     ln.res16_scale = res16_scale;
-    return launch_gemm_ln<VF_EPI_RES_F32, DT, VF_LN_PRODUCER_R16>(A, lda, W, bias, (const float*)residual, ldr, out, ldo, M, N, K, ln, st);
+    if (res_idx)
+        return launch_gemm_ln<VF_EPI_RES_F32, DT, VF_LN_PRODUCER_R16M>(A, lda, W, bias, (const float*)residual, ldr, out, ldo, M, N, K, ln, st, variant);
+    return launch_gemm_ln<VF_EPI_RES_F32, DT, VF_LN_PRODUCER_R16>(A, lda, W, bias, (const float*)residual, ldr, out, ldo, M, N, K, ln, st, variant);
 }
 
 extern "C" int vf_gemm_ln(const void* A, int64_t lda, const void* W, const float* bias, const void* residual, int64_t ldr,
@@ -1536,6 +1622,37 @@
                                     out16, ld16, part_stats, x16_scale, res_scale, stream, true, t16_out, ldt16, t16_scale);
 }
 
+extern "C" int vf_gemm_ln_v2(const void* A, int64_t lda, const void* W, const float* bias, const void* residual, int64_t ldr,
+                             int residual_dtype, void* out, int64_t ldo, int M, int N, int K, int epilogue, int operand_dtype,
+                             const float* row_stats, const float* colsum, void* out16, int64_t ld16, float* part_stats,
+                             float x16_scale, float res16_scale, const void* res_idx, int res_idx_bytes, int64_t res_rows,
+                             int variant, void* stream) {
+    if (operand_dtype == VF_BF16)
+        return gemm_ln_dispatch<VF_BF16>(A, lda, W, bias, residual, ldr, residual_dtype, out, ldo, M, N, K, epilogue, row_stats,
+                                         colsum, out16, ld16, part_stats, x16_scale, res16_scale, stream, false, nullptr, 0, 1.0f,
+                                         res_idx, res_idx_bytes, res_rows, variant);
+    VF_REQUIRE(operand_dtype == VF_F16, "vf_gemm_ln_v2: operand_dtype must be VF_BF16 or VF_F16");
+    return gemm_ln_dispatch<VF_F16>(A, lda, W, bias, residual, ldr, residual_dtype, out, ldo, M, N, K, epilogue, row_stats,
+                                    colsum, out16, ld16, part_stats, x16_scale, res16_scale, stream, false, nullptr, 0, 1.0f,
+                                    res_idx, res_idx_bytes, res_rows, variant);
+}
+
+extern "C" int vf_gemm_ln_t16_v2(const void* A, int64_t lda, const void* W, const float* bias, const void* residual_f16,
+                                 int64_t ldr, float res_scale, void* out, int64_t ldo, int M, int N, int K, int operand_dtype,
+                                 void* out16, int64_t ld16, float* part_stats, float x16_scale, void* t16_out, int64_t ldt16,
+                                 float t16_scale, const void* res_idx, int res_idx_bytes, int64_t res_rows, int variant,
+                                 void* stream) {
+    VF_REQUIRE(residual_f16, "vf_gemm_ln_t16_v2: null residual");
+    if (operand_dtype == VF_BF16)
+        return gemm_ln_dispatch<VF_BF16>(A, lda, W, bias, residual_f16, ldr, VF_F16, out, ldo, M, N, K, VF_EPI_RES_F32, nullptr,
+                                         nullptr, out16, ld16, part_stats, x16_scale, res_scale, stream, true, t16_out, ldt16,
+                                         t16_scale, res_idx, res_idx_bytes, res_rows, variant);
+    VF_REQUIRE(operand_dtype == VF_F16, "vf_gemm_ln_t16_v2: operand_dtype must be VF_BF16 or VF_F16");
+    return gemm_ln_dispatch<VF_F16>(A, lda, W, bias, residual_f16, ldr, VF_F16, out, ldo, M, N, K, VF_EPI_RES_F32, nullptr, nullptr,
+                                    out16, ld16, part_stats, x16_scale, res_scale, stream, true, t16_out, ldt16, t16_scale,
+                                    res_idx, res_idx_bytes, res_rows, variant);
+}
+
 extern "C" int vf_gemm_ln_bf16(const void* A, int64_t lda, const void* W, const float* bias, const float* residual,
                                int64_t ldr, void* out, int64_t ldo, int M, int N, int K, int epilogue,
                                const float* row_stats, const float* colsum, void* out16, int64_t ld16,
diff --git a/variantformer_amd/ops.py b/variantformer_amd/ops.py
--- a/variantformer_amd/ops.py
+++ b/variantformer_amd/ops.py
@@ -165,14 +165,23 @@
 
 
 class LnStream:
-    __slots__ = ("x", "x16", "stats", "scale", "t16")
-
-    def __init__(self, x, x16, stats, scale: float = 1.0, t16=None):
+    __slots__ = ("x", "x16", "stats", "scale", "t16", "rows")
+
+    def __init__(self, x, x16, stats, scale: float = 1.0, t16=None, rows=None):
         self.x, self.x16, self.stats, self.scale = x, x16, stats, float(scale)
+        self.rows = rows
         self.t16 = t16
 
     def operand16(self):
+        assert self.rows is None
         return self.x16 if self.scale == 1.0 else cast16(self.x, self.x16.dtype)
+
+    def gathered(self):
+        if self.rows is None:
+            return self
+        idx = self.rows.long()
+        return LnStream(None, gather_rows_bf16(self.x16, idx), None, self.scale,
+                        None if self.t16 is None else gather_rows_bf16(self.t16, idx))
 
 
 def x16_scale_for(dtype) -> float:
@@ -293,11 +302,20 @@
 
 def gemm_ln_producer(a: torch.Tensor, w: torch.Tensor, bias: torch.Tensor | None, residual,
                      eps: float = 1e-5, family: str = "", need_x: bool = True, trunk16: torch.Tensor | None = None,
-                     need_t16: bool = False) -> LnStream:
+                     need_t16: bool = False, res_rows: torch.Tensor | None = None, variant: int = 0) -> LnStream:
     assert residual is None if trunk16 is not None else not need_t16
     res16 = residual if isinstance(residual, LnStream) else None
     res32 = None if res16 is not None else residual
-    _dev(a, w, bias, res32, None if res16 is None else res16.x16, trunk16)
+    if res16 is not None and res16.rows is not None:
+        assert res_rows is None
+        res_rows = res16.rows
+    _dev(a, w, bias, res32, None if res16 is None else res16.x16, trunk16, res_rows)
+    if res_rows is not None:
+        assert (res16 is not None or trunk16 is not None) and res_rows.dtype in (torch.int32, torch.int64)
+        assert res_rows.is_contiguous() and res_rows.numel() == a.shape[0]
+    v2 = res_rows is not None or variant != 0
+    i_ptr, i_sz = _ptr(res_rows), (0 if res_rows is None else res_rows.element_size())
+    n_res = 0
     assert _is16(a.dtype) and w.dtype == a.dtype and a.shape[1] == w.shape[1] and a.stride(1) == 1
     M, K = a.shape
     N = w.shape[0]
@@ -312,11 +330,18 @@
     lib = _lib.load()
     lda = a.stride(0) if M > 1 else max(a.stride(0), K)
     if trunk16 is not None:
-        assert trunk16.dtype == torch.float16 and trunk16.shape == (M, N) and trunk16.stride(1) == 1
+        n_res = trunk16.shape[0]
+        assert trunk16.dtype == torch.float16 and trunk16.shape == (M if res_rows is None else n_res, N) and trunk16.stride(1) == 1
         epi, res_bytes = EPI_RES_F32, (2.0 + (2.0 if need_t16 else 0.0)) * M * N
-        tag = "-t16" + ("" if need_t16 else "-in")
+        tag = "-t16" + ("" if need_t16 else "-in") + ("" if res_rows is None else "-rows")
 
         def launch():
+            if v2:
+                check(lib.vf_gemm_ln_t16_v2(a.data_ptr(), lda, w.data_ptr(), _ptr(bias), trunk16.data_ptr(), trunk16.stride(0),
+                                            1.0 / T16_SCALE, _ptr(out), N, M, N, K, _dt(a.dtype), x16.data_ptr(), N, part.data_ptr(),
+                                            scale, _ptr(t_out), N, T16_SCALE, i_ptr, i_sz, n_res, variant, _stream()),
+                      "vf_gemm_ln_t16_v2")
+                return
             check(lib.vf_gemm_ln_t16(a.data_ptr(), lda, w.data_ptr(), _ptr(bias), trunk16.data_ptr(), trunk16.stride(0),
                                      1.0 / T16_SCALE, _ptr(out), N, M, N, K, _dt(a.dtype), x16.data_ptr(), N, part.data_ptr(),
                                      scale, _ptr(t_out), N, T16_SCALE, _stream()), "vf_gemm_ln_t16")
@@ -327,12 +352,19 @@
             r_ptr, r_ld, r_dt, r_scale, res_bytes, tag = res32.data_ptr(), res32.stride(0), VF_F32, 1.0, 4.0 * M * N, ""
         elif res16 is not None:
             r = res16.x16
-            assert r.dtype == a.dtype and r.shape == (M, N) and r.stride(1) == 1
-            r_ptr, r_ld, r_dt, r_scale, res_bytes, tag = r.data_ptr(), r.stride(0), _dt(r.dtype), 1.0 / res16.scale, 2.0 * M * N, "-r16"
+            n_res = r.shape[0]
+            assert r.dtype == a.dtype and r.shape == (M if res_rows is None else n_res, N) and r.stride(1) == 1
+            r_ptr, r_ld, r_dt, r_scale, res_bytes = r.data_ptr(), r.stride(0), _dt(r.dtype), 1.0 / res16.scale, 2.0 * M * N
+            tag = "-r16" + ("" if res_rows is None else "-rows")
         else:
             r_ptr, r_ld, r_dt, r_scale, res_bytes, tag = 0, 0, VF_F32, 1.0, 0.0, ""
 
         def launch():
+            if v2:
+                check(lib.vf_gemm_ln_v2(a.data_ptr(), lda, w.data_ptr(), _ptr(bias), r_ptr, r_ld, r_dt, _ptr(out), N, M, N, K, epi,
+                                        _dt(a.dtype), 0, 0, x16.data_ptr(), N, part.data_ptr(), scale, r_scale, i_ptr, i_sz, n_res,
+                                        variant, _stream()), "vf_gemm_ln_v2")
+                return
             check(lib.vf_gemm_ln(a.data_ptr(), lda, w.data_ptr(), _ptr(bias), r_ptr, r_ld, r_dt, _ptr(out), N, M, N, K, epi,
                                  _dt(a.dtype), 0, 0, x16.data_ptr(), N, part.data_ptr(), scale, r_scale, _stream()), "vf_gemm_ln")
 
diff --git a/variantformer_amd/runtime.py b/variantformer_amd/runtime.py
--- a/variantformer_amd/runtime.py
+++ b/variantformer_amd/runtime.py
@@ -12,6 +12,7 @@
     lowrank_context: bool = True
     layer0_qkv_table: bool = True
     pool_before_down_projection: bool = True
+    residual_rows: bool = True
     overlap_cre_stream: bool = True
 
 
diff --git a/variantformer_amd/seq2gene/modules/layers.py b/variantformer_amd/seq2gene/modules/layers.py
--- a/variantformer_amd/seq2gene/modules/layers.py
+++ b/variantformer_amd/seq2gene/modules/layers.py
@@ -132,9 +132,13 @@
 def down_projection(hg, lin: nn.Linear, s, keep_x: bool = True, rows32: bool = False, pooled=None):
     w2, b2 = packed_linear(lin)
     folded = isinstance(s, ops.LnStream)
+    if folded and s.rows is not None and pooled is not None:
+        s = s.gathered()
+    rows = s.rows if folded else None
     t16 = None
     if folded and trunk_f16_active():
         t16 = s.t16 if s.t16 is not None else ops.trunk16_of(s.x)
+    assert rows is None or t16 is not None, "a row-mapped stream carries its fp16 trunk copy"
     x32 = s.x if folded else s
     if pooled is not None:
         if t16 is not None:
@@ -144,7 +148,7 @@
         return ops.gemm(hg, w2, b2, ops.EPI_RES_F32, residual=x32)
     need_x = keep_x or rows32
     if t16 is not None:
-        out = ops.gemm_ln_producer(hg, w2, b2, None, need_x=need_x, trunk16=t16, need_t16=not need_x)
+        out = ops.gemm_ln_producer(hg, w2, b2, None, need_x=need_x, trunk16=t16, need_t16=not need_x, res_rows=rows)
     else:
         out = ops.gemm_ln_producer(hg, w2, b2, s if x32 is None else x32, need_x=need_x)
     return out.x if rows32 else out
@@ -303,6 +307,7 @@
         return out_residual(a, w, b, x)
 
     def self_block(self, x, norm, cu, max_len, qkv=None):
+        assert qkv is not None or not (isinstance(x, ops.LnStream) and x.rows is not None), "a row-mapped stream comes with its projection"
         a = self.attend(x, norm, None, cu, max_len) if qkv is None else self.attend_qkv(qkv[0], cu, max_len, rows=qkv[1])
         return self.out_proj_residual(a, x)
 
@@ -422,10 +427,12 @@
             return qkv
         stream = None
         if trunk_f16_active():
-            x16 = ops.gather_rows_bf16(torch.cat([sa.x16, sb.x16], dim=0), idx2)
-            t16 = ops.gather_rows_bf16(torch.cat([ops.trunk16_of(sa.x), ops.trunk16_of(sb.x, raise_alert=rows_b_used is None)],
-                                                 dim=0), idx2)
-            stream = ops.LnStream(None, x16, None, sa.scale, t16)
+            x16 = torch.cat([sa.x16, sb.x16], dim=0)
+            t16 = torch.cat([ops.trunk16_of(sa.x), ops.trunk16_of(sb.x, raise_alert=rows_b_used is None)], dim=0)
+            if runtime.switches().residual_rows:
+                stream = ops.LnStream(None, x16, None, sa.scale, t16, rows=idx2)
+            else:
+                stream = ops.LnStream(None, ops.gather_rows_bf16(x16, idx2), None, sa.scale, ops.gather_rows_bf16(t16, idx2))
         return qkv, stream
 
     def forward_packed(self, src, cu_src, max_src, context=None, cu_ctx=None, max_ctx=None, context_kv=None,
diff --git a/variantformer_amd/seq2reg/model.py b/variantformer_amd/seq2reg/model.py
--- a/variantformer_amd/seq2reg/model.py
+++ b/variantformer_amd/seq2reg/model.py
@@ -14,6 +14,7 @@
 
 LAYER0_QKV_TABLE_MAX_BYTES = 1 << 30
 _LAYER0_SLOTS = {torch.bfloat16: "_vf_layer0_qkv_bf16", torch.float16: "_vf_layer0_qkv_fp16"}
+_LAYER0_ROWS_SLOT = "_vf_layer0_rows"
 
 
 def positionalencoding1d(d_model: int, length: int) -> torch.Tensor:
@@ -103,6 +104,24 @@
             return l0.MHA.project_qkv(s, l0.norm1, family="seq2reg")
         return weights.derived(self, _LAYER0_SLOTS[ops.cdt()], prm, build, key_L), key_L
 
+    def _layer0_input_tables(self, device):
+        pos = self._pos_table(device)
+        V = self.token_embedding.weight.shape[0]
+        key_L = pos.shape[0] if pos is not None else 1
+        prm = [self.token_embedding.weight, pos]
+        def build():
+            ids = torch.arange(V, device=device, dtype=torch.int64).view(V, 1).expand(V, key_L).contiguous()
+            pad = torch.zeros((V, key_L), dtype=torch.uint8, device=device)
+            cu = (torch.arange(V + 1, device=device, dtype=torch.int32) * key_L).contiguous()
+            alert = ops._alert_flag(device)
+            before = alert.clone()
+            alert.zero_()
+            s = ops.embed_stream(ids, pad, cu, self.token_embedding.weight, pos, V * key_L)
+            raised = int(alert.item())
+            alert.copy_(before)
+            return None if raised else (s.x16, s.t16, s.scale)
+        return weights.derived(self, _LAYER0_ROWS_SLOT, prm, build, key_L, ops.ln_fold_abs_limit())
+
     def _layer0_qkv_table_bytes(self) -> int:
         key_L = self.position_encoding.shape[0] if self.pos_encoding_type == "sinusoidal" else 1
         V, d = self.token_embedding.weight.shape
@@ -119,7 +138,16 @@
         with ops.scope("seq2reg"):
             cu = ops.mask_to_cu_seqlens(pad)
             l0 = self.transformer_encoder[0]
-            if (trunk_f16_active() and ln_fold_enabled(l0.norm1.weight.numel(), l0.linear_geglu_2.in_features)
+            V = self.token_embedding.weight.shape[0]
+            lookup0 = (not self.use_context and runtime.switches().layer0_qkv_table and
+                       ln_fold_enabled(l0.norm1.weight.numel(), l0.linear_geglu_2.in_features) and
+                       self.token_embedding.weight.shape[1] <= 2048 and self._layer0_qkv_table_bytes() <= LAYER0_QKV_TABLE_MAX_BYTES)
+            keys0 = ops.token_keys(ids, pad, cu, n_tokens, V, self._pos_table(ids.device).shape[0]
+                                   if self.pos_encoding_type == "sinusoidal" else 1) if lookup0 else None
+            rows0 = self._layer0_input_tables(ids.device) if lookup0 and trunk_f16_active() and runtime.switches().residual_rows else None
+            if rows0 is not None:
+                x = ops.LnStream(None, rows0[0], None, rows0[2], rows0[1], rows=keys0)
+            elif (trunk_f16_active() and ln_fold_enabled(l0.norm1.weight.numel(), l0.linear_geglu_2.in_features)
                     and self.token_embedding.weight.shape[1] <= 2048):
                 x = ops.embed_stream(ids, pad, cu, self.token_embedding.weight, self._pos_table(ids.device), n_tokens)
             else:
@@ -140,12 +168,9 @@
                 pool_in_layer = (self.seq_pool == "mean" and runtime.switches().pool_before_down_projection and lg2.in_features % 8 == 0 and
                                  lg2.out_features % 8 == 0 and max(lg2.in_features, lg2.out_features) <= 2048)
                 qkv0 = None
-                V = self.token_embedding.weight.shape[0]
-                if (runtime.switches().layer0_qkv_table and ln_fold_enabled(l0.norm1.weight.numel(), l0.linear_geglu_2.in_features) and
-                        self.token_embedding.weight.shape[1] <= 2048 and
-                        self._layer0_qkv_table_bytes() <= LAYER0_QKV_TABLE_MAX_BYTES):
+                if lookup0:
                     tab, key_L = self._layer0_qkv_table(ids.device)
-                    qkv0 = (tab, ops.token_keys(ids, pad, cu, n_tokens, V, key_L))
+                    qkv0 = (tab, keys0)
                 for li, layer in enumerate(self.transformer_encoder):
                     x = layer.forward_packed(x, cu, Lmax, last=li + 1 == n_layers, keep_x=not trunk16_enabled(),
                                              pool_mean=pool_in_layer and li + 1 == n_layers, qkv=qkv0 if li == 0 else None)
```
